# RinceWND/extPOM

Hardware: AMD Instinct MI355X
Metric: 3D cell-updates/sec on internal mode (one internal step = the 3-D baroclinic step and its isplit 2-D external substeps; whole-step wall time) (higher is better)
Workload: dtype f64

## Files before the change

### extpom_amd/csrc/k_adv.hip

```cpp
#include "pomgpu_internal.hpp"

#define dt_(i, j) F2(dt, i, j)
#define dx_(i, j) F2(dx, i, j)
#define dy_(i, j) F2(dy, i, j)
#define h_(i, j) F2(h, i, j)
#define u_(i, j, k) F3(u, i, j, k)
#define v_(i, j, k) F3(v, i, j, k)
#define ub_(i, j, k) F3(ub, i, j, k)
#define vb_(i, j, k) F3(vb, i, j, k)
#define w_(i, j, k) F3(w, i, j, k)
#define aam_(i, j, k) F3(aam, i, j, k)

#define MARCH3(call)                                                                  \
  const int g_ = (int)(blockIdx.x * blockDim.x + threadIdx.x);    \
  const int L_ = g_ >> 6, xcd_ = L_ & 7, m_ = L_ >> 3;                                \
  const int bpl_ = P.g_bpl, nbx_ = P.g_nbx;                                           \
  const int p_ = m_ % bpl_, t_ = m_ / bpl_;                                           \
  const int k = t_ % P.kb + 1;                                                        \
  const int band_ = (t_ / P.kb) * 8 + xcd_;                                           \
  const int i = (p_ % nbx_) * 64 + (g_ & 63) + 1;                                     \
  const int j = band_ * P.g_rb + (p_ / nbx_) * 4 + (int)threadIdx.y + 1;              \
  if (i > P.iml || j > P.jml) return;                                                 \
  call;
__device__ __forceinline__ void c_advct_a(const KP &P, const int i, const int j, const int k);
// ... 290 lines not shown
  MARCH3(c_smol(P, i, j, k, ff))
}
__device__ __forceinline__ void c_smol(const KP &P, const int i, const int j, const int k, const double *ff) {
  if (i > P.im || j > P.jm) return;
  const double value_min = 1.e-9, epsilon = 1.0e-14;
  double *xm = P.s3[0], *ym = P.s3[1], *zw = P.s3[2];
  const double fc = G3(ff, i, j, k);
  if (k <= P.kbm1 && j >= 2 && j <= P.jmm1 && i >= 2) {
    const double fw = G3(ff, i - 1, j, k);
    double r = 0.;
    if (!(fc < value_min || fw < value_min)) {
      const double m = G3(xm, i, j, k);
      const double udx = fabs(m);
      const double u2dt = P.dti2 * m * m * 2. / (F2(aru, i, j) * (dt_(i - 1, j) + dt_(i, j)));
      const double mol = (fc - fw) / (fw + fc + epsilon);
      r = (udx - u2dt) * mol * P.sw;
      if (fabs(udx) < fabs(u2dt)) r = 0.;
    }
    G3(xm, i, j, k) = r;
  }
  if (k <= P.kbm1 && j >= 2 && i >= 2 && i <= P.imm1) {
    const double fs = G3(ff, i, j - 1, k);
    double r = 0.;
    if (!(fc < value_min || fs < value_min)) {
      const double m = G3(ym, i, j, k);
      const double vdy = fabs(m);
      const double v2dt = P.dti2 * m * m * 2. / (F2(arv, i, j) * (dt_(i, j - 1) + dt_(i, j)));
      const double mol = (fc - fs) / (fs + fc + epsilon);
      r = (vdy - v2dt) * mol * P.sw;
      if (fabs(vdy) < fabs(v2dt)) r = 0.;
    }
    G3(ym, i, j, k) = r;
  }
  if (k >= 2 && k <= P.kbm1 && i >= 2 && i <= P.imm1 && j >= 2 && j <= P.jmm1) {
    const double fu = G3(ff, i, j, k - 1);
    double r = 0.;
    if (!(fc < value_min || fu < value_min)) {
      const double m = G3(zw, i, j, k);
      const double wdz = fabs(m);
      const double w2dt = P.dti2 * m * m / (F1(dzz, k - 1) * dt_(i, j));
      const double mol = (fu - fc) / (fc + fu + epsilon);
      r = (wdz - w2dt) * mol * P.sw;
      if (fabs(wdz) < fabs(w2dt)) r = 0.;
    }
    G3(zw, i, j, k) = r;
  }
}
__device__ __forceinline__ void c_copy3(const KP &P, const int i, const int j, const int k, double *dst, const double *src);
__global__ void k_copy3(KP P, double *dst, const double *src) {
  MARCH3(c_copy3(P, i, j, k, dst, src))
}
__device__ __forceinline__ void c_copy3(const KP &P, const int i, const int j, const int k, double *dst, const double *src) {
  G3(dst, i, j, k) = G3(src, i, j, k);
}
__device__ __forceinline__ double advt2_xdiff(const KP &P, const double *fb, const double *fc, int i, int j, int k) {
  const double am = 0.5 * (aam_(i, j, k) + aam_(i - 1, j, k));
  return -am * (h_(i, j) + h_(i - 1, j)) * P.tprni *
         ((G3(fb, i, j, k) - G3(fc, i, j, k)) - (G3(fb, i - 1, j, k) - G3(fc, i - 1, j, k))) * F2(dum, i, j) *
         (dy_(i, j) + dy_(i - 1, j)) * 0.5 / (dx_(i, j) + dx_(i - 1, j));
}
__device__ __forceinline__ double advt2_ydiff(const KP &P, const double *fb, const double *fc, int i, int j, int k) {
  const double am = 0.5 * (aam_(i, j, k) + aam_(i, j - 1, k));
  return -am * (h_(i, j) + h_(i, j - 1)) * P.tprni *
         ((G3(fb, i, j, k) - G3(fc, i, j, k)) - (G3(fb, i, j - 1, k) - G3(fc, i, j - 1, k))) * F2(dvm, i, j) *
         (dx_(i, j) + dx_(i, j - 1)) * 0.5 / (dy_(i, j) + dy_(i, j - 1));
}
__device__ __forceinline__ void c_advt2_diff(const KP &P, const int i, const int j, const int k, const double *fb, const double *fc, double *ff);
__global__ void k_advt2_diff(KP P, const double *fb, const double *fc, double *ff) {
  MARCH3(c_advt2_diff(P, i, j, k, fb, fc, ff))
}
__device__ __forceinline__ void c_advt2_diff(const KP &P, const int i, const int j, const int k, const double *fb, const double *fc, double *ff) {
  if (k > P.kbm1 || i < 2 || i > P.imm1 || j < 2 || j > P.jmm1) return;
  G3(ff, i, j, k) = G3(ff, i, j, k) -
                    P.dti2 * (advt2_xdiff(P, fb, fc, i + 1, j, k) - advt2_xdiff(P, fb, fc, i, j, k) +
                              advt2_ydiff(P, fb, fc, i, j + 1, k) - advt2_ydiff(P, fb, fc, i, j, k)) /
                        ((h_(i, j) + F2(etf, i, j)) * F2(art, i, j));
}

__device__ __forceinline__ double dens_point(const KP &P, double si, double ti, int i, int j, int k);
template <int TAU> __device__ __forceinline__ void c_ts_update(const KP &P, const int i, const int j, const int k, double fold, double fnew, int rt, int store_rst, double tau_b, double tau_f, const unsigned long long *rtf);
template <int TAU> __global__ void k_ts_update(KP P, double fold, double fnew, int rt, int store_rst, double tau_b, double tau_f, const unsigned long long *rtf) {
  MARCH3(c_ts_update<TAU>(P, i, j, k, fold, fnew, rt, store_rst, tau_b, tau_f, rtf))
}
__global__ void k_ts_update_same(KP P, double fold, double fnew, int rt, int store_rst, const unsigned long long *rtf) {
  MARCH3(c_ts_update<2>(P, i, j, k, fold, fnew, rt, store_rst, 0., 0., rtf))
}
template <int TAU> __device__ __forceinline__ void c_ts_update(const KP &P, const int i, const int j, const int k, double fold, double fnew, int rt, int store_rst, double tau_b, double tau_f, const unsigned long long *rtf) {
  const bool act = (i <= P.im && j <= P.jm), lev = (k <= P.kbm1);
  const pomgpu_ct m = F2(fsm, i, j);
  pomgpu_ct uf = F3(uf, i, j, k), vf = F3(vf, i, j, k);
  if (lev && act) {
    uf = uf * m;
    vf = vf * m;
  }
  pomgpu_ct tb = F3(tb, i, j, k), sb = F3(sb, i, j, k);
  bool rtc = rt != 0;
  if (rtc && rtf && lev) rtc = ((rtf[RT_WORD(P, i, j, k)] >> RT_BIT(i)) & 1ull) != 0;
  if (rtc) {
    const pomgpu_ct tc = F3(tclim, i, j, k), sc = F3(sclim, i, j, k);
    tb = (tb - tc) + tc;
    sb = (sb - sc) + sc;
  }
  const pomgpu_ct t0 = F3(t, i, j, k), s0 = F3(s, i, j, k);
  pomgpu_ct tbn = t0 + CT(.5) * CT(P.smoth) * (uf + tb - CT(2.) * t0);
  pomgpu_ct sbn = s0 + CT(.5) * CT(P.smoth) * (vf + sb - CT(2.) * s0);
  pomgpu_ct tn = uf, sn = vf;
// ... 297 lines not shown
  }
  F3(wr, i, j, k) = v;
}

struct LevR { double w_n, u_c, u_e, v_c, v_n; };
__device__ __forceinline__ LevR realvertvl_load(const KP &P, int a, int b, int k) {
  LevR L;
  L.w_n = w_(a, b, k + 1); L.u_c = u_(a, b, k); L.u_e = u_(a + 1, b, k); L.v_c = v_(a, b, k); L.v_n = v_(a, b + 1, k);
  return L;
}
__global__ void __launch_bounds__(256) k_realvertvl_col(KP P, int etf_is_et) {
  const int i = TID_I, j = TID_J;
  if (i > P.iml || j > P.jml) return;
  const bool act = (i <= P.im && j <= P.jm);
  const int a = (P.W && i == 1) ? 2 : ((P.E && i == P.im) ? P.imm1 : i);
  const int b = (P.S && j == 1) ? 2 : ((P.N && j == P.jm) ? P.jmm1 : j);
  const int kb = P.kb, kbm1 = P.kbm1;
  if (!(act && a >= 2 && a <= P.imm1 && b >= 2 && b <= P.jmm1)) {
    for (int k = 1; k <= kb; k++) F3(wr, i, j, k) = 0.;
    return;
  }
  const double dt_c = dt_(a, b), dt_e = dt_(a + 1, b), dt_w = dt_(a - 1, b), dt_n = dt_(a, b + 1), dt_s = dt_(a, b - 1);
  const double et_c = F2(et, a, b), et_e = F2(et, a + 1, b), et_w = F2(et, a - 1, b), et_n = F2(et, a, b + 1), et_s = F2(et, a, b - 1);
  const double dxr = K2(R2DXSX, a + 1, b), dxl = K2(R2DXSX, a, b), dyt = K2(R2DYSY, a, b + 1), dyb = K2(R2DYSY, a, b);
  const double detf = (etf_is_et ? et_c : F2(etf, a, b)) - F2(etb, a, b);
  const double m = F2(fsm, i, j);
  double w_k = w_(a, b, 1);
  LevR c = realvertvl_load(P, a, b, 1), nxt = c;
  for (int k = 1; k <= kbm1; k++) {
    PACE_BARRIER();
    if (k + 1 <= kbm1) nxt = realvertvl_load(P, a, b, k + 1);
    const double zzk = F1(zz, k);
#define TPS(dtv, etv) (zzk * (dtv) + (etv))
    const double tc = TPS(dt_c, et_c);
    double v = 0.5 * (w_k + c.w_n) +
               0.5 * (c.u_e * (TPS(dt_e, et_e) - tc) * dxr + c.u_c * (tc - TPS(dt_w, et_w)) * dxl +
                      c.v_n * (TPS(dt_n, et_n) - tc) * dyt + c.v_c * (tc - TPS(dt_s, et_s)) * dyb) +
               (1.0 + zzk) * detf / P.dti2;
#undef TPS
    F3(wr, i, j, k) = m * v;
    w_k = c.w_n;
    c = nxt;
  }
  F3(wr, i, j, kb) = 0.;
}

#define LD2(ptr, ii, jj, kk) (*(const double2 *)&(ptr)[IX3(ii, jj, kk)])
#define A3(name) (P.b3 + (size_t)P3_##name * P.a3)
__device__ __forceinline__ double aam_point(const KP &P, double dx, double dy, double u_c, double u_e, double u_n, double u_ne, double u_s,
                                            double u_se, double v_c, double v_n, double v_e, double v_ne, double v_w, double v_nw) {
  return P.horcon * dx * dy *
         sqrt(sq((u_e - u_c) / dx) + sq((v_n - v_c) / dy) +
              .5 * sq(.25 * (u_n + u_ne - u_s - u_se) / dy + .25 * (v_e + v_ne - v_w - v_nw) / dx));
}
__device__ __forceinline__ double aam_point_r(const KP &P, const InvD &dx, const InvD &dy, double u_c, double u_e, double u_n, double u_ne, double u_s,
                                              double u_se, double v_c, double v_n, double v_e, double v_ne, double v_w, double v_nw) {
  return P.horcon * dx.b * dy.b *
         sqrt(sq(divi(u_e - u_c, dx)) + sq(divi(v_n - v_c, dy)) +
              .5 * sq(divi(.25 * (u_n + u_ne - u_s - u_se), dy) + divi(.25 * (v_e + v_ne - v_w - v_nw), dx)));
}
#ifndef AAM_KCH
#define AAM_KCH 7
#endif
struct AamLev { double2 u_s, u_0, u_n, v_0, v_n; };
__global__ void __launch_bounds__(256) k_aam_pair(KP P) {
  const int g_ = (int)(blockIdx.x * blockDim.x + threadIdx.x);
  const int L_ = g_ >> 6, xcd_ = L_ & 7, m_ = L_ >> 3;
  const int nbx_ = (P.iml / 2 + 61) / 62, bpl_ = nbx_ * (P.g_rb / 4);
  const int nch_ = (P.kbm1 + AAM_KCH - 1) / AAM_KCH;
  const int p_ = m_ % bpl_, t_ = m_ / bpl_;
  const int k0 = (t_ % nch_) * AAM_KCH + 1;
  const int band_ = (t_ / nch_) * 8 + xcd_;
  const int lane = g_ & 63;
  const int ia0 = 2 * ((p_ % nbx_) * 62 + lane - 1) + 1;
  const int j = band_ * P.g_rb + (p_ / nbx_) * 4 + (int)threadIdx.y + 1;
  if (k0 > P.kbm1 || j < 2 || j > P.jmm1) return;
  const int k1 = k0 + AAM_KCH - 1 < P.kbm1 ? k0 + AAM_KCH - 1 : P.kbm1;
  const bool out = (lane >= 1 && lane <= 62 && ia0 <= P.iml);
#ifdef POMGPU_EMU
  if (!out) return;
#endif
  const int ia = ia0 < 1 ? 1 : (ia0 > P.iml - 1 ? P.iml - 1 : ia0), ib = ia + 1;
  const int iw = ia > 1 ? ia - 1 : 1, ie = ib < P.iml ? ib + 1 : P.iml;
  const double2 dx = *(const double2 *)&F2(dx, ia, j), dy = *(const double2 *)&F2(dy, ia, j);
#ifndef AAM_PLAIN_DIV
  const double2 rdx = *(const double2 *)&K2(RDX, ia, j), rdy = *(const double2 *)&K2(RDY, ia, j);
  const InvD dxa = {dx.x, rdx.x}, dya = {dy.x, rdy.x}, dxb = {dx.y, rdx.y}, dyb = {dy.y, rdy.y};
#endif
  auto lev = [&](int k) {
    AamLev L;
    L.u_s = LD2(A3(u), ia, j - 1, k); L.u_0 = LD2(A3(u), ia, j, k); L.u_n = LD2(A3(u), ia, j + 1, k);
    L.v_0 = LD2(A3(v), ia, j, k); L.v_n = LD2(A3(v), ia, j + 1, k);
    return L;
  };
  AamLev cur = lev(k0);
  for (int k = k0; k <= k1; k++) {
    const AamLev nxt = lev(k < k1 ? k + 1 : k1);
    const double2 u_s = cur.u_s, u_0 = cur.u_0, u_n = cur.u_n, v_0 = cur.v_0, v_n = cur.v_n;
    const double uE_s = halo_e(u_s.x, [&] { return u_(ie, j - 1, k); }), uE_0 = halo_e(u_0.x, [&] { return u_(ie, j, k); }),
                 uE_n = halo_e(u_n.x, [&] { return u_(ie, j + 1, k); });
    const double vE_0 = halo_e(v_0.x, [&] { return v_(ie, j, k); }), vE_n = halo_e(v_n.x, [&] { return v_(ie, j + 1, k); });
    const double vW_0 = halo_w(v_0.y, [&] { return v_(iw, j, k); }), vW_n = halo_w(v_n.y, [&] { return v_(iw, j + 1, k); });
#ifndef AAM_PLAIN_DIV
    const double aa = aam_point_r(P, dxa, dya, u_0.x, u_0.y, u_n.x, u_n.y, u_s.x, u_s.y, v_0.x, v_n.x, v_0.y, v_n.y, vW_0, vW_n);
    const double ab = aam_point_r(P, dxb, dyb, u_0.y, uE_0, u_n.y, uE_n, u_s.y, uE_s, v_0.y, v_n.y, vE_0, vE_n, v_0.x, v_n.x);
#else
    const double aa = aam_point(P, dx.x, dy.x, u_0.x, u_0.y, u_n.x, u_n.y, u_s.x, u_s.y, v_0.x, v_n.x, v_0.y, v_n.y, vW_0, vW_n);
    const double ab = aam_point(P, dx.y, dy.y, u_0.y, uE_0, u_n.y, uE_n, u_s.y, uE_s, v_0.y, v_n.y, vE_0, vE_n, v_0.x, v_n.x);
#endif
    if (out && ia0 >= 2 && ia0 <= P.imm1) F3(aam, ia0, j, k) = aa;
    if (out && ia0 + 1 <= P.imm1) F3(aam, ia0 + 1, j, k) = ab;
    cur = nxt;
  }
}
#undef LD2
#undef A3


void launch_advct_a(pomgpu_ctx *c) { LAUNCH(c, k_advct_a, gridm(c->P), blk2(), c->P); }
void launch_advct_b(pomgpu_ctx *c) { LAUNCH(c, k_advct_b, gridm(c->P), blk2(), c->P); }
void launch_advct_c(pomgpu_ctx *c) { LAUNCH(c, k_advct_c, gridm(c->P), blk2(), c->P); }
void launch_aam(pomgpu_ctx *c) {
  const KP &P = c->P;
#ifdef POMGPU_STORE_F32
  const bool pair_ok = false;
#else
  const bool pair_ok = true;
#endif
  if (pair_ok && P.iml % 2 == 0 && !SW(c, NO_PAIR)) {
    const long nbands = (P.jml + P.g_rb - 1) / P.g_rb, rounds = (nbands + 7) / 8;
    const long bpl = (long)((P.iml / 2 + 61) / 62) * (P.g_rb / 4);
    const long nch = (P.kbm1 + AAM_KCH - 1) / AAM_KCH;
    LAUNCHN(c, "k_aam_pair", k_aam_pair, dim3((unsigned)(8 * rounds * nch * bpl), 1, 1), blk2(), c->P);
  } else {
    LAUNCH(c, k_aam, gridm(c->P), blk2(), c->P);
  }
}
void launch_roundtrip(pomgpu_ctx *c, double *a, const double *b, int fix_kb) { LAUNCH(c, k_roundtrip, gridm(c->P), blk2(), c->P, a, b, fix_kb); }
void launch_roundtrip_level(pomgpu_ctx *c, double *a, const double *b, int k) { LAUNCH(c, k_roundtrip_level, grid2(c->P), blk2(), c->P, a, b, k); }
void launch_advq_flux(pomgpu_ctx *c, const double *q, const double *qb, double *xf, double *yf) {
  LAUNCH(c, k_advq_flux, gridm(c->P), blk2(), c->P, q, qb, xf, yf);
}
void launch_advq_step(pomgpu_ctx *c, const double *q, const double *qb, double *qf, const double *xf, const double *yf, int zero_else) {
  LAUNCH(c, k_advq_step, gridm(c->P), blk2(), c->P, q, qb, qf, xf, yf, zero_else);
}
void launch_q_filter(pomgpu_ctx *c, int mask) { LAUNCH(c, k_q_filter, gridm(c->P), blk2(), c->P, mask); }
void launch_q_filter_rim(pomgpu_ctx *c) {
  const KP &P = c->P;
  const int len = P.im > P.jm ? P.im : P.jm;
  LAUNCH(c, k_q_filter_rim, dim3((len + 63) / 64, 8, P.kb), dim3(64, 1, 1), c->P);
}
void launch_mask_q(pomgpu_ctx *c) { LAUNCH(c, k_mask_q, gridm(c->P), blk2(), c->P); }
void launch_advt1(pomgpu_ctx *c, double *fb, double *f, const double *fclim, double *ff) {
  LAUNCH(c, k_advt1, gridm(c->P), blk2(), c->P, (const double *)fb, (const double *)f, fclim, ff);
  LAUNCH(c, k_copy_kb, grid2(c->P), blk2(), c->P, f, (double *)NULL);
}
void launch_copy_kb(pomgpu_ctx *c, double *f, double *g) { LAUNCH(c, k_copy_kb, grid2(c->P), blk2(), c->P, f, g); }
void launch_advt2_mass(pomgpu_ctx *c) { LAUNCH(c, k_advt2_mass, gridm(c->P), blk2(), c->P); }
void launch_advt2_step(pomgpu_ctx *c, const double *fbmem, const double *f, const double *eta, double *ff, int itera) {
  LAUNCH(c, k_advt2_step, gridm(c->P), blk2(), c->P, fbmem, f, eta, ff, itera);
}
void launch_mask3(pomgpu_ctx *c, double *a, const double *m2) { LAUNCH(c, k_mask3, gridm(c->P), blk2(), c->P, a, m2); }
void launch_smol(pomgpu_ctx *c, const double *ff) { LAUNCH(c, k_smol, gridm(c->P), blk2(), c->P, ff); }
void launch_copy3(pomgpu_ctx *c, double *dst, const double *src) { LAUNCH(c, k_copy3, gridm(c->P), blk2(), c->P, dst, src); }
void launch_advt2_diff(pomgpu_ctx *c, const double *fb, const double *fc, double *ff) { LAUNCH(c, k_advt2_diff, gridm(c->P), blk2(), c->P, fb, fc, ff); }
void launch_ts_update(pomgpu_ctx *c, double fold, double fnew, int rt, int store_rst, int rt_flags) {
  const unsigned long long *rtf = (rt && rt_flags) ? c->rt_words : NULL;
  if (rtf && c->prof_on) {
    const int s = pomgpu_prof_slot(c, "ts_rt_flags");
    if (s >= 0) (c->parent ? c->parent : c)->prof[s].launches++;
  }
  if (c->tau_known[0] && c->tau_known[1] && !c->tau_handed && !SW(c, TAU_ARRAYS))
    LAUNCHN(c, "k_ts_update", (k_ts_update<1>), gridm(c->P), blk2(), c->P, fold, fnew, rt, store_rst, c->tau_val[0], c->tau_val[1], rtf);
  else if (c->tau_same && !c->tau_handed && !SW(c, TAU_ARRAYS))
    LAUNCH(c, k_ts_update_same, gridm(c->P), blk2(), c->P, fold, fnew, rt, store_rst, rtf);
  else
    LAUNCHN(c, "k_ts_update", (k_ts_update<0>), gridm(c->P), blk2(), c->P, fold, fnew, rt, store_rst, 0., 0., rtf);
}
void launch_restore_fields(pomgpu_ctx *c, double fold, double fnew) { LAUNCH(c, k_restore_fields, gridm(c->P), blk2(), c->P, fold, fnew); }
void launch_mask_ts(pomgpu_ctx *c) { LAUNCH(c, k_mask_ts, gridm(c->P), blk2(), c->P); }
void launch_tr_update(pomgpu_ctx *c, const TrUpd *u, int nf, int rt) {
  if (nf == 2) {
    TrUpds<2> A; A.u[0] = u[0]; A.u[1] = u[1];
    LAUNCHN(c, "k_tr_update2", (k_tr_update<2>), gridm(c->P), blk2(), c->P, A, rt);
  } else {
    TrUpds<1> A; A.u[0] = u[0];
    LAUNCHN(c, "k_tr_update", (k_tr_update<1>), gridm(c->P), blk2(), c->P, A, rt);
  }
}
void launch_tr_source(pomgpu_ctx *c, double *ff, const double *fb, const double *fc, const double *q, double lam) {
  LAUNCH(c, k_tr_source, gridm(c->P), blk2(), c->P, ff, fb, fc, q, lam);
}
void launch_mask_uv(pomgpu_ctx *c) { LAUNCH(c, k_mask_uv, gridm(c->P), blk2(), c->P); }
void launch_mask_w(pomgpu_ctx *c) { LAUNCH(c, k_mask_w, gridm(c->P), blk2(), c->P); }
void launch_restore(pomgpu_ctx *c, double fold, double fnew) { LAUNCH(c, k_restore, gridm(c->P), blk2(), c->P, fold, fnew); }
void launch_restore_shift(pomgpu_ctx *c) { LAUNCH(c, k_restore_shift, gridm(c->P), blk2(), c->P); }
void launch_restore_load(pomgpu_ctx *c, const double *tr, const double *sr, double tau, const double *taur, int fill_tau) { LAUNCH(c, k_restore_load, gridm(c->P), blk2(), c->P, tr, sr, tau, taur, fill_tau); }
void launch_probe_gpow15(pomgpu_ctx *c, long n, const double *x, double *out) { LAUNCH(c, k_probe_gpow15, dim3((unsigned)((n + 255) / 256), 1, 1), dim3(256, 1, 1), n, x, out); }
void launch_dens(pomgpu_ctx *c, const double *si, const double *ti, double *rhoo) { LAUNCH(c, k_dens, gridm(c->P), blk2(), c->P, si, ti, rhoo); }
void launch_realvertvl(pomgpu_ctx *c, int etf_is_et) {
  if (SW(c, REALVERTVL_CELLS)) LAUNCH(c, k_realvertvl, gridm(c->P), blk2(), c->P, etf_is_et);
  else LAUNCHN(c, "k_realvertvl_col", k_realvertvl_col, grid2(c->P), blk2(), c->P, etf_is_et);
}
```

### extpom_amd/csrc/k_tile.hip

```cpp
#include "pomgpu_internal.hpp"


__global__ void k_coef_static(KP P) {
  const int i = TID_I, j = TID_J;
  if (i > P.iml || j > P.jml) return;
  const int iw = i > 1 ? i - 1 : 1, js = j > 1 ? j - 1 : 1;
  P.m8[IX2(i, j)] = (unsigned char)((F2(fsm, i, j) != 0. ? 1 : 0) | (F2(dum, i, j) != 0. ? 2 : 0) | (F2(dvm, i, j) != 0. ? 4 : 0));
  K2(HSX, i, j) = F2(h, i, j) + F2(h, iw, j);
  K2(HSY, i, j) = F2(h, i, j) + F2(h, i, js);
  K2(DYSX, i, j) = F2(dy, i, j) + F2(dy, iw, j);
  K2(DXSX, i, j) = F2(dx, i, j) + F2(dx, iw, j);
  K2(DXSY, i, j) = F2(dx, i, j) + F2(dx, i, js);
  K2(DYSY, i, j) = F2(dy, i, j) + F2(dy, i, js);
  K2(DX4, i, j) = F2(dx, i, j) + F2(dx, iw, j) + F2(dx, i, js) + F2(dx, iw, js);
  K2(DY4, i, j) = F2(dy, i, j) + F2(dy, iw, j) + F2(dy, i, js) + F2(dy, iw, js);
  const int ie = i < P.iml ? i + 1 : P.iml, jn = j < P.jml ? j + 1 : P.jml;
  K2(CVA, i, j) = F2(dy, ie, j) - F2(dy, iw, j);
  K2(CVB, i, j) = F2(dx, i, jn) - F2(dx, i, js);
  K2(R2DXSX, i, j) = 2.0 / (F2(dx, i, j) + F2(dx, iw, j));
  K2(R2DYSY, i, j) = 2.0 / (F2(dy, i, j) + F2(dy, i, js));
  K2(RDX, i, j) = 1.0 / F2(dx, i, j);
  K2(RDY, i, j) = 1.0 / F2(dy, i, j);
  if (j == 1)
    for (int n = i - 1; n < POM_NBLK1D * P.kb; n += P.iml) P.r1[n] = 1.0 / P.b1[n];
// ... 24 lines not shown
    K2(VCOR, i, j) = (j >= 2 && j <= P.jm && i <= P.im) ? cv : mark;
  }
}

__device__ __forceinline__ pomgpu_ct upw_(pomgpu_ct m, pomgpu_ct lo, pomgpu_ct hi) {
  return CT(0.5) * ((m + fabs(m)) * lo + (m - fabs(m)) * hi);
}
struct FaceT { pomgpu_ct adv, dif; };
struct TFields { const double *fb[2], *f[2], *fcl[2]; double *ff[2]; unsigned long long *rtf; };
template <int NF> struct LevT { pomgpu_ct c[2 * NF + 2], o[2], h[ROWSHARE_SLOTS(2 * NF + 2)]; };
template <int NS> struct NbrT { pomgpu_ct s[NS], n[NS]; };
struct CoefT { pomgpu_ct cm, hs, msk, ds_num; InvDc den; };
__device__ __forceinline__ CoefT coef_x(const KP &P, int i, int j) {
  CoefT c; c.cm = K2(CMX, i, j); c.hs = K2(HSX, i, j); c.msk = F2(dum, i, j); c.ds_num = K2(DYSX, i, j); c.den = inv_of(CT(K2(DXSX, i, j))); return c;
}
__device__ __forceinline__ CoefT coef_y(const KP &P, int i, int j) {
  CoefT c; c.cm = K2(CMY, i, j); c.hs = K2(HSY, i, j); c.msk = F2(dvm, i, j); c.ds_num = K2(DXSY, i, j); c.den = inv_of(CT(K2(DYSY, i, j))); return c;
}
__device__ __forceinline__ FaceT advt2_face(const pomgpu_ct tprni, const CoefT &c, pomgpu_ct vel, pomgpu_ct fb_hi, pomgpu_ct fb_lo, pomgpu_ct fc_hi,
                                            pomgpu_ct fc_lo, pomgpu_ct am_hi, pomgpu_ct am_lo) {
  FaceT f;
  f.adv = upw_(c.cm * vel, fb_lo, fb_hi);
  const pomgpu_ct am = CT(0.5) * (am_hi + am_lo);
  f.dif = divi(-am * c.hs * tprni * ((fb_hi - fc_hi) - (fb_lo - fc_lo)) * c.msk * c.ds_num * CT(0.5), c.den);
  return f;
}
#if COL_WX != 1
#error "the row-sharing column kernels keep one wavefront per workgroup row (COL_WX == 1)"
#endif
template <int NF, bool UM = false, bool RTF = false>
__global__ void __launch_bounds__(64 * LDS_ROWS) k_advt2_col(KP P, TFields A) {
  constexpr int NS = 2 * NF + 2, NH = ROWSHARE_SLOTS(NS), AM = 2 * NF, VV = 2 * NF + 1;
  HALO_XCD_DECODE_R(LDS_ROWS)
  const int r = WAVE_UNIFORM((int)threadIdx.y), j0w = j - r;
  const bool jrow = j <= P.jml;
  const int jc = jrow ? j : P.jml;
  const bool icol = jrow && (lane >= 1 && lane <= 62 && i0 <= P.iml);
#ifdef POMGPU_EMU
  if (!icol) return;
#endif
  const int i = i0 < 1 ? 1 : (i0 > P.iml ? P.iml : i0);
  const int iw = i > 1 ? i - 1 : 1, ie = i < P.iml ? i + 1 : P.iml;
  const int js = jc > 1 ? jc - 1 : 1, jn = jc < P.jml ? jc + 1 : P.jml;
  const bool in = icol && (i >= 2 && i <= P.imm1 && jc >= 2 && jc <= P.jmm1);
  const pomgpu_ct fsm = F2(fsm, i, jc);
  const CoefT cw = coef_x(P, i, jc), cs = coef_y(P, i, jc), cn = coef_y(P, i, jn);
  const pomgpu_ct art = F2(art, i, jc), hea = K2(HEA, i, jc);
  const InvDc hfa = inv_of(CT(K2(HFA, i, jc)));
  const pomgpu_ct tprni = P.tprni, dti2 = P.dti2;
  BufA bs[NS], bo[2], bff[NF], bh[NH];
  const double *ps[NS];
#pragma unroll
  for (int f = 0; f < NF; f++) { ps[f] = A.fb[f]; ps[NF + f] = A.fcl[f]; bff[f] = BUF3(A.ff[f]); }
  ps[AM] = A3(aam); ps[VV] = A3(v); bo[0] = BUF3(A3(u)); bo[1] = BUF3(A3(w));
#pragma unroll
  for (int x = 0; x < NS; x++) bs[x] = BUF3(ps[x]);
  const RowShare<NS> S = rowshare_setup<NS>(P, r, j, j0w, i);
#pragma unroll
  for (int q = 0; q < NH; q++) bh[q] = BUF3(rowshare_pick<NS>(ps, S.hop[q]));
  const UvmC mu = UM ? uvm_of<0>(P, i, jc) : uvm_none(), mv = UM ? uvm_of<1>(P, i, jc) : uvm_none();
  UvmC mh[NH];
#pragma unroll
  for (int q = 0; q < NH; q++) mh[q] = UM ? rowshare_uvm<1, NS, LDS_ROWS>(P, S, q, VV, j0w, i) : uvm_none();
  const unsigned oc = BOFF2(i, jc), lvb = LVB;
  const unsigned ost = in ? oc : BOFF_NONE;
  const int rt_nbx = RT_NBX(P);
  const BufA brtf = buf2_of((const double *)A.rtf, RTF ? (size_t)P.kbm1 * P.jml * rt_nbx : 0);
  const unsigned ortf = (RTF && jrow && lane == 0) ? (unsigned)((jc - 1) * rt_nbx + (i0 - lane) / 62) * 8u : BOFF_NONE, lvrtf = (unsigned)(P.jml * rt_nbx) * 8u;
#ifndef POMGPU_EMU
  __shared__ pomgpu_ct slab[2][NS][ROWSHARE_ROWS][64];
#else
  const unsigned os = BOFF2(i, js), on = BOFF2(i, jn);
#endif
  auto load = [&](LevT<NF> &L, unsigned lv) {
#pragma unroll
    for (int x = 0; x < NS; x++) L.c[x] = bldc(bs[x], oc, lv);
    L.o[0] = bldc(bo[0], oc, lv); L.o[1] = bldc(bo[1], oc, lv);
#pragma unroll
    for (int q = 0; q < NH; q++) L.h[q] = bldc(bh[q], S.hoff[q], lv);
  };
  pomgpu_ct f1[NF];
#pragma unroll
  for (int f = 0; f < NF; f++) f1[f] = G3(A.f[f], i, jc, 1);
  const int kbm1 = P.kbm1;
  pomgpu_ct p_adv[NF], p_dif[NF], p_fb[NF], p_zu[NF];
#pragma unroll
  for (int f = 0; f < NF; f++) p_adv[f] = p_dif[f] = p_fb[f] = p_zu[f] = 0.;
  auto step = [&](const int L, const int par, const LevT<NF> &cur, LevT<NF> &nxt) {
    load(nxt, (unsigned)(L < kbm1 ? L : kbm1 - 1) * lvb);
    NbrT<NS> nb;
    const pomgpu_ct v_c = uvm_fix(cur.c[VV], mv);
#ifndef POMGPU_EMU
#pragma unroll
    for (int x = 0; x < NS; x++) slab[par][x][r + 1][lane] = x == VV ? v_c : cur.c[x];
#pragma unroll
    for (int q = 0; q < NH; q++) slab[par][S.hop[q]][S.hrow[q]][lane] = uvm_fix(cur.h[q], mh[q]);
    __syncthreads();
#pragma unroll
    for (int x = 0; x < NS; x++) { nb.s[x] = slab[par][x][S.ss][lane]; nb.n[x] = slab[par][x][S.sn][lane]; }
#else
    const unsigned lvc = (unsigned)((L <= kbm1 ? L : kbm1) - 1) * lvb;
#pragma unroll
    for (int x = 0; x < NS; x++) { nb.s[x] = bldc(bs[x], os, lvc); nb.n[x] = bldc(bs[x], on, lvc); }
    nb.s[VV] = uvm_fix(nb.s[VV], uvm_of<1>(P, i, js)); nb.n[VV] = uvm_fix(nb.n[VV], uvm_of<1>(P, i, jn));
#endif
    const pomgpu_ct am_c = cur.c[AM], u_c = uvm_fix(cur.o[0], mu), w_c = cur.o[1];
    const pomgpu_ct am_w = halo_w(am_c, [&] { return F3(aam, iw, jc, L); });
    InvDc dzk; dzk.b = dzk.y = 0.;
    if (L >= 2) { dzk.b = F1(dz, L - 1); dzk.y = R1(dz, L - 1); }
    if constexpr (RTF) {
      bool ch = false;
#pragma unroll
      for (int f = 0; f < NF; f++) ch = ch || rt_changes(cur.c[f], cur.c[NF + f]);
      const unsigned lvw = (unsigned)WAVE_UNIFORM(L - 1) * lvrtf;
#ifndef POMGPU_EMU
      bst2u(brtf, L <= kbm1 ? ortf : BOFF_NONE, lvw, __ballot(icol && ch));
#else
      if (L <= kbm1) {
        unsigned long long &wd = A.rtf[RT_WORD(P, i, jc, L)];
        wd = (lane == 1 ? 0ull : wd) | ((unsigned long long)ch << lane);
      }
      (void)brtf; (void)ortf; (void)lvw;
#endif
    }
#pragma unroll
    for (int f = 0; f < NF; f++) {
      const pomgpu_ct fb_c = cur.c[f], fc_c = cur.c[NF + f];
      pomgpu_ct zu = 0.;
      pomgpu_ct s_adv = 0., s_dif = 0.;
      if (L <= kbm1) {
        const pomgpu_ct fb_w = halo_w(fb_c, [&] { return G3(A.fb[f], iw, jc, L); });
        const pomgpu_ct fc_w = halo_w(fc_c, [&] { return G3(A.fcl[f], iw, jc, L); });
        const FaceT xw = advt2_face(tprni, cw, u_c, fb_c, fb_w, fc_c, fc_w, am_c, am_w);
        auto east = [&] {
          return advt2_face(tprni, coef_x(P, ie, jc), uvm_ld<0>(P, ie, jc, L), G3(A.fb[f], ie, jc, L), fb_c, G3(A.fcl[f], ie, jc, L), fc_c,
                            F3(aam, ie, jc, L), am_c);
        };
        FaceT xe;
        xe.adv = halo_e(xw.adv, [&] { return east().adv; });
        xe.dif = halo_e(xw.dif, [&] { return east().dif; });
        const FaceT ys = advt2_face(tprni, cs, v_c, fb_c, nb.s[f], fc_c, nb.s[NF + f], am_c, nb.s[AM]);
        const FaceT yn = advt2_face(tprni, cn, nb.n[VV], nb.n[f], fb_c, nb.n[NF + f], fc_c, nb.n[AM], am_c);
        s_adv = xe.adv - xw.adv + yn.adv - ys.adv;
        s_dif = xe.dif - xw.dif + yn.dif - ys.dif;
        zu = (L == 1) ? w_c * f1[f] * art : upw_(w_c, fb_c, p_fb[f]) * art;
      }
      {
        pomgpu_ct rr = p_adv[f] + divi(p_zu[f] - zu, dzk);
        rr = divi(p_fb[f] * hea - dti2 * rr, hfa);
        rr = rr * fsm;
        rr = rr - divi(dti2 * p_dif[f], hfa);
        bstc(bff[f], (L >= 2 && L <= kbm1 + 1) ? ost : BOFF_NONE, (unsigned)(L >= 2 ? L - 2 : 0) * lvb, rr);
      }
      p_adv[f] = s_adv; p_dif[f] = s_dif; p_fb[f] = fb_c; p_zu[f] = zu;
    }
  };
  LevT<NF> ra, rb;
  load(ra, 0u);
  rb = ra;
  for (int L = 1; L <= kbm1 + 1; L += 2) {
    step(L, 1, ra, rb);
    step(L + 1, 0, rb, ra);
  }
  if (icol) {
    for (int k = in ? P.kb : 1; k <= P.kb; k++) {
#pragma unroll
      for (int f = 0; f < NF; f++) G3(A.ff[f], i, jc, k) = CT(G3(A.ff[f], i, jc, k)) * fsm;
    }
  }
}

struct QFields { const double *q[2], *qb[2]; double *qf[2]; };
template <int NF, int NO = 2> struct LevQa { pomgpu_ct c[2 * NF + 2], o[NO], h[ROWSHARE_SLOTS(2 * NF + 2)]; };
struct CoefQ { pomgpu_ct dts, hs, msk, ds_num; InvDc den; };
__device__ __forceinline__ CoefQ coefq_x(const KP &P, int i, int j) {
  CoefQ c; c.dts = K2(DTSX, i, j); c.hs = K2(HSX, i, j); c.msk = F2(dum, i, j); c.den = inv_of(CT(K2(DXSX, i, j))); c.ds_num = K2(DYSX, i, j); return c;
}
__device__ __forceinline__ CoefQ coefq_y(const KP &P, int i, int j) {
  CoefQ c; c.dts = K2(DTSY, i, j); c.hs = K2(HSY, i, j); c.msk = F2(dvm, i, j); c.den = inv_of(CT(K2(DYSY, i, j))); c.ds_num = K2(DXSY, i, j); return c;
}
__device__ __forceinline__ pomgpu_ct advq_face(const CoefQ &c, pomgpu_ct q_hi, pomgpu_ct q_lo, pomgpu_ct vel_k, pomgpu_ct vel_km1, pomgpu_ct am_hi_k,
                                               pomgpu_ct am_lo_k, pomgpu_ct am_hi_m, pomgpu_ct am_lo_m, pomgpu_ct qb_hi, pomgpu_ct qb_lo) {
  pomgpu_ct x = CT(.125) * (q_hi + q_lo) * c.dts * (vel_k + vel_km1);
  x = x - divi(CT(.25) * (am_hi_k + am_lo_k + am_hi_m + am_lo_m) * c.hs * (qb_hi - qb_lo) * c.msk, c.den);
  return CT(.5) * c.ds_num * x;
}
template <int NF, bool WF = false, bool UM = false>
__global__ void __launch_bounds__(64 * LDS_ROWS) k_advq_col(KP P, QFields A, int zero_else) {
  constexpr int NS = 2 * NF + 2, NH = ROWSHARE_SLOTS(NS), AM = 2 * NF, VV = 2 * NF + 1;
  typedef LevQa<NF, WF ? 1 : 2> Lev;
  HALO_XCD_DECODE_R(LDS_ROWS)
  const int r = WAVE_UNIFORM((int)threadIdx.y), j0w = j - r;
  const bool jrow = j <= P.jml;
  const int jc = jrow ? j : P.jml;
  const bool icol = jrow && (lane >= 1 && lane <= 62 && i0 <= P.iml);
#ifdef POMGPU_EMU
  if (!icol) return;
#endif
  const int i = i0 < 1 ? 1 : (i0 > P.iml ? P.iml : i0);
  const int iw = i > 1 ? i - 1 : 1, ie = i < P.iml ? i + 1 : P.iml;
  const int js = jc > 1 ? jc - 1 : 1, jn = jc < P.jml ? jc + 1 : P.jml;
  const bool in = icol && (i >= 2 && i <= P.imm1 && jc >= 2 && jc <= P.jmm1);
  const CoefQ cw = coefq_x(P, i, jc), cs = coefq_y(P, i, jc), cn = coefq_y(P, i, jn);
  const pomgpu_ct art = F2(art, i, jc), hea = K2(HEA, i, jc);
  const InvDc hfa = inv_of(CT(K2(HFA, i, jc)));
  const int kb = P.kb, kbm1 = P.kbm1;
  BufA bs[NS], bo[2], bqf[NF], bh[NH];
  const double *ps[NS];
#pragma unroll
  for (int f = 0; f < NF; f++) { ps[f] = A.q[f]; ps[NF + f] = A.qb[f]; bqf[f] = BUF3(A.qf[f]); }
  ps[AM] = A3(aam); ps[VV] = A3(v); bo[0] = BUF3(A3(u)); bo[1] = BUF3(A3(w));
#pragma unroll
  for (int x = 0; x < NS; x++) bs[x] = BUF3(ps[x]);
  const RowShare<NS> S = rowshare_setup<NS>(P, r, j, j0w, i);
#pragma unroll
  for (int q = 0; q < NH; q++) bh[q] = BUF3(rowshare_pick<NS>(ps, S.hop[q]));
  const UvmC mu = UM ? uvm_of<0>(P, i, jc) : uvm_none(), mv = UM ? uvm_of<1>(P, i, jc) : uvm_none();
  UvmC mh[NH];
#pragma unroll
  for (int q = 0; q < NH; q++) mh[q] = UM ? rowshare_uvm<1, NS, LDS_ROWS>(P, S, q, VV, j0w, i) : uvm_none();
  const unsigned oc = BOFF2(i, jc), lvb = LVB;
  const unsigned ost = in ? oc : ((zero_else && icol) ? oc : BOFF_NONE);
  const unsigned ostw = in ? oc : BOFF_NONE;
#ifndef POMGPU_EMU
  __shared__ pomgpu_ct slab[2][NS][ROWSHARE_ROWS][64];
#else
  const unsigned os = BOFF2(i, js), on = BOFF2(i, jn);
#endif
  double vv_cw = 0., vv_ce = 0., vv_cs = 0., vv_cn = 0., vv_det = 0., vv_m = 0., wk = 0.;
  InvD vv_area; vv_area.b = vv_area.y = 0.;
  if constexpr (WF) {
    vv_m = F2(fsm, i, jc);
    const double dyc = F2(dy, i, jc), dtc = F2(dt, i, jc), dxc = F2(dx, i, jc);
    const double dyw = halo_w(dyc, [&] { return F2(dy, iw, jc); }), dtw = halo_w(dtc, [&] { return F2(dt, iw, jc); });
    const double dye = halo_e(dyc, [&] { return F2(dy, ie, jc); }), dte = halo_e(dtc, [&] { return F2(dt, ie, jc); });
    vv_cw = .25 * (dyc + dyw) * (dtc + dtw);
    vv_ce = .25 * (dye + dyc) * (dte + dtc);
    vv_cs = .25 * (dxc + F2(dx, i, js)) * (dtc + F2(dt, i, js));
    vv_cn = .25 * (F2(dx, i, jn) + dxc) * (F2(dt, i, jn) + dtc);
    vv_area = inv_of(dxc * dyc);
    vv_det = (F2(etf, i, jc) - F2(etb, i, jc)) / P.dti2;
    wk = 0.5 * (F2(vfluxb, i, jc) + F2(vfluxf, i, jc));
  }
  auto load = [&](Lev &L, int k) {
    const unsigned lv = (unsigned)WAVE_UNIFORM(k - 1) * lvb;
#pragma unroll
    for (int x = 0; x < NS; x++) L.c[x] = bldc(bs[x], oc, lv);
    L.o[0] = bldc(bo[0], oc, lv);
    if constexpr (!WF) L.o[1] = bldc(bo[1], oc, lv);
#pragma unroll
    for (int q = 0; q < NH; q++) L.h[q] = bldc(bh[q], S.hoff[q], lv);
  };
  pomgpu_ct u_m = 0., v_m = 0., vn_m = 0., am_m = 0., ams_m = 0., amn_m = 0.;
  pomgpu_ct am_w_prv = 0.;
  pomgpu_ct ue_m = 0.;
  pomgpu_ct wq_pp[NF], wq_p[NF];
  pomgpu_ct xe_p[NF], xw_p[NF], yn_p[NF], ys_p[NF], qb_p[NF];
#pragma unroll
  for (int f = 0; f < NF; f++) wq_pp[f] = wq_p[f] = xe_p[f] = xw_p[f] = yn_p[f] = ys_p[f] = qb_p[f] = 0.;
  auto step = [&](const int L, const int par, const Lev &cur, Lev &nxt) {
    load(nxt, L + 1 <= kb ? L + 1 : kb);
    NbrT<NS> nb;
    const bool lcor = L <= kbm1;
    const pomgpu_ct v_c = uvm_fix(cur.c[VV], mv, lcor), u_c = uvm_fix(cur.o[0], mu, lcor);
#ifndef POMGPU_EMU
#pragma unroll
    for (int x = 0; x < NS; x++) slab[par][x][r + 1][lane] = x == VV ? v_c : cur.c[x];
#pragma unroll
    for (int q = 0; q < NH; q++) slab[par][S.hop[q]][S.hrow[q]][lane] = uvm_fix(cur.h[q], mh[q], lcor);
    __syncthreads();
#pragma unroll
    for (int x = 0; x < NS; x++) { nb.s[x] = slab[par][x][S.ss][lane]; nb.n[x] = slab[par][x][S.sn][lane]; }
#else
    const unsigned lvc = (unsigned)((L <= kb ? L : kb) - 1) * lvb;
#pragma unroll
    for (int x = 0; x < NS; x++) { nb.s[x] = bldc(bs[x], os, lvc); nb.n[x] = bldc(bs[x], on, lvc); }
    nb.s[VV] = uvm_fix(nb.s[VV], uvm_of<1>(P, i, js), lcor); nb.n[VV] = uvm_fix(nb.n[VV], uvm_of<1>(P, i, jn), lcor);
#endif
    const pomgpu_ct am_c = cur.c[AM];
    const pomgpu_ct am_s = nb.s[AM], am_n = nb.n[AM], v_n = nb.n[VV];
    const pomgpu_ct am_w = halo_w(am_c, [&] { return F3(aam, iw, jc, L); });
    pomgpu_ct w_c, ue_c = 0.;
    if constexpr (WF) {
      ue_c = halo_e(u_c, [&] { return uvm_ld<0>(P, ie, jc, L); });
      const double wn = wk + F1(dz, L >= 2 ? L - 1 : 1) *
                             (divi(vv_ce * (double)ue_m - vv_cw * (double)u_m + vv_cn * (double)vn_m - vv_cs * (double)v_m, vv_area) + vv_det);
      wk = L >= 2 ? wn : wk;
      const double wst = L <= kbm1 ? wk * vv_m : wk;
      bst(bo[1], ostw, (unsigned)WAVE_UNIFORM(L - 1) * lvb, wst);
      w_c = CT((pomgpu_st)wst);
    } else {
      w_c = cur.o[1];
    }
    const int k = L - 1;
    InvDc dz2; dz2.b = dz2.y = 0.;
    if (k >= 2 && k <= kbm1) { dz2.b = CT(F1(dz, k)) + CT(F1(dz, k - 1)); dz2.y = CT(1.0) / dz2.b; }
#pragma unroll
    for (int f = 0; f < NF; f++) {
      const pomgpu_ct q_c = cur.c[f], qb_c = cur.c[NF + f];
      pomgpu_ct xe_c = 0., xw_c = 0., yn_c = 0., ys_c = 0.;
      if (L >= 2 && L <= kbm1) {
        const pomgpu_ct q_w = halo_w(q_c, [&] { return G3(A.q[f], iw, jc, L); });
        const pomgpu_ct qb_w = halo_w(qb_c, [&] { return G3(A.qb[f], iw, jc, L); });
        const pomgpu_ct xw = advq_face(cw, q_c, q_w, u_c, u_m, am_c, am_w, am_m, am_w_prv, qb_c, qb_w);
        xw_c = xw;
        xe_c = halo_e(xw, [&] {
          return advq_face(coefq_x(P, ie, jc), G3(A.q[f], ie, jc, L), q_c, uvm_ld<0>(P, ie, jc, L), uvm_ld<0>(P, ie, jc, L - 1), F3(aam, ie, jc, L), am_c,
                           F3(aam, ie, jc, L - 1), am_m, G3(A.qb[f], ie, jc, L), qb_c);
        });
        ys_c = advq_face(cs, q_c, nb.s[f], v_c, v_m, am_c, am_s, am_m, ams_m, qb_c, nb.s[NF + f]);
        yn_c = advq_face(cn, nb.n[f], q_c, v_n, vn_m, am_n, am_c, amn_m, am_m, nb.n[NF + f], qb_c);
      }
      const pomgpu_ct wq_c = w_c * q_c;
      {
        pomgpu_ct rr = 0.;
        if (in && k >= 2 && k <= kbm1) {
          rr = divi((wq_pp[f] - wq_c) * art, dz2) + xe_p[f] - xw_p[f] + yn_p[f] - ys_p[f];
          rr = divi(hea * qb_p[f] - CT(P.dti2) * rr, hfa);
        }
        const bool lev_in = (k >= 2 && k <= kbm1);
        const unsigned o = (k >= 1) ? (lev_in ? ost : ((zero_else && icol) ? oc : BOFF_NONE)) : BOFF_NONE;
        bstc(bqf[f], o, (unsigned)WAVE_UNIFORM(k >= 1 ? k - 1 : 0) * lvb, rr);
      }
      wq_pp[f] = wq_p[f]; wq_p[f] = wq_c; qb_p[f] = qb_c;
      xe_p[f] = xe_c; xw_p[f] = xw_c; yn_p[f] = yn_c; ys_p[f] = ys_c;
    }
    am_w_prv = am_w;
    if constexpr (WF) ue_m = ue_c;
    u_m = u_c; v_m = v_c; vn_m = v_n; am_m = am_c; ams_m = am_s; amn_m = am_n;
  };
  Lev ra, rb;
  load(ra, 1);
  rb = ra;
  for (int L = 1; L <= kb; L += 2) {
    step(L, 1, ra, rb);
    if (L + 1 <= kb) step(L + 1, 0, rb, ra);
  }
  if (icol && zero_else) {
#pragma unroll
    for (int f = 0; f < NF; f++) G3(A.qf[f], i, jc, kb) = 0.;
  }
  if constexpr (WF) {
    if (icol && !in && i0 <= P.im && jc <= P.jm)
      for (int k = 1; k <= kbm1; k++) F3(w, i, jc, k) = F3(w, i, jc, k) * vv_m;
  }
}

__device__ double advct_xf_mem(const KP &P, int i, int j, int k) {
  if (i < 2 || i > P.imm1) return 0.;
  double xf = .125 * (K2(DTSX, i + 1, j) * F3(u, i + 1, j, k) + K2(DTSX, i, j) * F3(u, i, j, k)) * (F3(u, i + 1, j, k) + F3(u, i, j, k));
  xf = xf - F2(dt, i, j) * F3(aam, i, j, k) * 2. * (F3(ub, i + 1, j, k) - F3(ub, i, j, k)) / F2(dx, i, j);
  return F2(dy, i, j) * xf;
}
__device__ double advct_curv_mem(const KP &P, int i, int j, int k) {
  if (i < 2 || i > P.imm1 || j < 2 || j > P.jmm1) return 0.;
  return .25 * ((F3(v, i, j + 1, k) + F3(v, i, j, k)) * K2(CVA, i, j) - (F3(u, i + 1, j, k) + F3(u, i, j, k)) * K2(CVB, i, j)) / F2(art, i, j);
}
__device__ double advct_xg_mem(const KP &P, int i, int j, int k) {
  double xg = .125 * (K2(DTSX, i, j) * F3(u, i, j, k) + K2(DTSX, i, j - 1) * F3(u, i, j - 1, k)) * (F3(v, i, j, k) + F3(v, i - 1, j, k));
  const double dtaam = .25 * K2(DT4, i, j) * (F3(aam, i, j, k) + F3(aam, i - 1, j, k) + F3(aam, i, j - 1, k) + F3(aam, i - 1, j - 1, k));
  const double dy4 = K2(DY4, i, j);
  xg = xg - dtaam * ((F3(ub, i, j, k) - F3(ub, i, j - 1, k)) / dy4 + (F3(vb, i, j, k) - F3(vb, i - 1, j, k)) / K2(DX4, i, j));
  return .25 * dy4 * xg;
}
__device__ double advct_yf_mem(const KP &P, int i, int j, int k) {
  double yf = .125 * (K2(DTSY, i, j) * F3(v, i, j, k) + K2(DTSY, i - 1, j) * F3(v, i - 1, j, k)) * (F3(u, i, j, k) + F3(u, i, j - 1, k));
  const double dtaam = .25 * K2(DT4, i, j) * (F3(aam, i, j, k) + F3(aam, i - 1, j, k) + F3(aam, i, j - 1, k) + F3(aam, i - 1, j - 1, k));
  const double dx4 = K2(DX4, i, j);
  yf = yf - dtaam * ((F3(ub, i, j, k) - F3(ub, i, j - 1, k)) / K2(DY4, i, j) + (F3(vb, i, j, k) - F3(vb, i - 1, j, k)) / dx4);
  return .25 * dx4 * yf;
}
__device__ double advct_yg_mem(const KP &P, int i, int j, int k) {
  double yg = .125 * (K2(DTSY, i, j + 1) * F3(v, i, j + 1, k) + K2(DTSY, i, j) * F3(v, i, j, k)) * (F3(v, i, j + 1, k) + F3(v, i, j, k));
  yg = yg - F2(dt, i, j) * F3(aam, i, j, k) * 2. * (F3(vb, i, j + 1, k) - F3(vb, i, j, k)) / F2(dy, i, j);
  return F2(dx, i, j) * yg;
}
__global__ void k_advct_edge(KP P, double *to_e, double *to_n) {
  const int t = TID_I, k = (int)blockIdx.y + 1;
  if (k > P.kbm1) return;
  if (to_e && t <= P.jm) {
    const size_t o = (size_t)(k - 1) * P.jm + (size_t)(t - 1);
    to_e[o] = advct_curv_mem(P, P.imm1, t, k);
    to_e[(size_t)P.kbm1 * P.jm + o] = t >= 2 ? advct_xf_mem(P, P.imm1, t, k) : 0.;
  }
  if (to_n && t <= P.im) {
    const size_t o = (size_t)(k - 1) * P.im + (size_t)(t - 1);
    to_n[o] = advct_curv_mem(P, t, P.jmm1, k);
    to_n[(size_t)P.kbm1 * P.im + o] = t >= 2 ? advct_yg_mem(P, t, P.jmm1, k) : 0.;
  }
}
__global__ void k_advct_fix(KP P, const double *from_w, const double *from_s) {
  const int t = TID_I, k = (int)blockIdx.y + 1;
  if (k > P.kbm1) return;
  if (from_w && t >= 2 && t <= P.jmm1) {
    const int j = t;
    const size_t o = (size_t)(k - 1) * P.jm + (size_t)(j - 1);
    const double cv_w = from_w[o], xf_w = from_w[(size_t)P.kbm1 * P.jm + o];
    const double xf = advct_xf_mem(P, 2, j, k), yf_n = advct_yf_mem(P, 2, j + 1, k), yf_c = advct_yf_mem(P, 2, j, k);
    const double cv = advct_curv_mem(P, 2, j, k);
    const double ctx = cv * F2(dt, 2, j) * (F3(v, 2, j + 1, k) + F3(v, 2, j, k));
    const double ctx_w = cv_w * F2(dt, 1, j) * (F3(v, 1, j + 1, k) + F3(v, 1, j, k));
    double ax = xf - xf_w + yf_n - yf_c;
    ax = ax - F2(aru, 2, j) * .25 * (ctx + ctx_w);
    F3(advx, 2, j, k) = ax;
  }
  if (from_s && t >= 2 && t <= P.imm1) {
    const int i = t;
    const size_t o = (size_t)(k - 1) * P.im + (size_t)(i - 1);
    const double cv_s = from_s[o], yg_s = from_s[(size_t)P.kbm1 * P.im + o];
    const double xg_e = advct_xg_mem(P, i + 1, 2, k), xg = advct_xg_mem(P, i, 2, k), yg_c = advct_yg_mem(P, i, 2, k);
    const double cv = advct_curv_mem(P, i, 2, k);
    double ay = xg_e - xg + yg_c - yg_s;
    ay = ay + F2(arv, i, 2) * .25 * (cv * F2(dt, i, 2) * (F3(u, i + 1, 2, k) + F3(u, i, 2, k)) +
                                     cv_s * F2(dt, i, 1) * (F3(u, i + 1, 1, k) + F3(u, i, 1, k)));
    F3(advy, i, 2, k) = ay;
  }
}
template <int ROWS> struct LevCaT { pomgpu_ct c[5], h[(2 * 5 + ROWS - 1) / ROWS]; };
template <int ROWS>
__global__ void __launch_bounds__(64 * ROWS) k_advct_col(KP P, int sum2d) {
  constexpr int NS = 5, NH = (2 * NS + ROWS - 1) / ROWS, U = 0, V = 1, UB = 2, VB = 3, AM = 4;
  typedef LevCaT<ROWS> LevCa;
  HALO_XCD_DECODE_R(ROWS)
#ifdef POMGPU_WGTIME
  const unsigned long long wgt0 = wall_clock64();
#endif
  const int r = WAVE_UNIFORM((int)threadIdx.y), j0w = j - r;
  const bool jvalid = j <= P.jml;
  const int jc = jvalid ? j : P.jml;
  const bool out = jvalid && (lane >= 1 && lane <= 62 && i0 <= P.iml);
#ifdef POMGPU_EMU
  if (!out) return;
#endif
  const int i = i0 < 1 ? 1 : (i0 > P.iml ? P.iml : i0);
  const int iw = i > 1 ? i - 1 : 1, ie = i < P.iml ? i + 1 : P.iml;
  const int js = jc > 1 ? jc - 1 : 1, jn = jc < P.jml ? jc + 1 : P.jml;
  const bool jrow = (jc >= 2 && jc <= P.jmm1);
  const bool iin = (i0 >= 2 && i0 <= P.imm1);
  const bool in = out && iin && jrow;
  const int kb = P.kb, kbm1 = P.kbm1;
  double ax2 = 0., ay2 = 0.;
#if POMGPU_UVM_ONLOAD
  double su2 = 0., sv2 = 0.;
#endif
  const pomgpu_ct dtsx_c = K2(DTSX, i, jc), dtsx_s = K2(DTSX, i, js);
  const pomgpu_ct dtsx_e = halo_e(dtsx_c, [&] { return K2(DTSX, ie, jc); });
  const pomgpu_ct dtsy_c = K2(DTSY, i, jc), dtsy_n = K2(DTSY, i, jn), dtsy_s = K2(DTSY, i, js);
  const pomgpu_ct dtsy_w = halo_w(dtsy_c, [&] { return K2(DTSY, iw, jc); });
  const pomgpu_ct dtsy_nw = halo_w(dtsy_n, [&] { return K2(DTSY, iw, jn); });
  const pomgpu_ct dt4_c = K2(DT4, i, jc), dt4_n = K2(DT4, i, jn);
  const pomgpu_ct dx4_c = K2(DX4, i, jc), dx4_n = K2(DX4, i, jn);
  const InvDc dy4_c = inv_of(CT(K2(DY4, i, jc))), dy4_n = inv_of(CT(K2(DY4, i, jn))), idx4_c = inv_of(dx4_c), idx4_n = inv_of(dx4_n);
  const pomgpu_ct dt_c = F2(dt, i, jc), dy_c = F2(dy, i, jc), dx_c = F2(dx, i, jc);
  const pomgpu_ct dt_s = F2(dt, i, js), dx_s = F2(dx, i, js);
  const InvDc idx_c = inv_of(dx_c), idy_c = inv_of(dy_c), idy_s = inv_of(CT(F2(dy, i, js)));
  const pomgpu_ct cva_c = K2(CVA, i, jc), cvb_c = K2(CVB, i, jc);
  const pomgpu_ct cva_s = K2(CVA, i, js), cvb_s = K2(CVB, i, js);
  const InvDc art_c = inv_of(CT(F2(art, i, jc))), art_s = inv_of(CT(F2(art, i, js)));
  const pomgpu_ct aru = F2(aru, i, jc), arv = F2(arv, i, jc);
  const bool srow = (jc - 1 >= 2);
  const bool curvx = (i0 >= (P.W ? 3 : 2)), curvy = (jc >= (P.S ? 3 : 2));
  BufA bs[NS], bh[NH];
  const double *ps[NS] = {A3(u), A3(v), A3(ub), A3(vb), A3(aam)};
#pragma unroll
  for (int x = 0; x < NS; x++) bs[x] = BUF3(ps[x]);
  const BufA bax = BUF3(A3(advx)), bay = BUF3(A3(advy));
  const RowShare<NS, ROWS> S = rowshare_setup<NS, ROWS>(P, r, j, j0w, i);
#pragma unroll
  for (int q = 0; q < NH; q++) bh[q] = BUF3(rowshare_pick<NS>(ps, S.hop[q]));
  const unsigned oc = BOFF2(i, jc), lvb = LVB;
  const unsigned ost = (out && jrow) ? oc : BOFF_NONE;
#ifndef POMGPU_EMU
  __shared__ pomgpu_ct slab[2][NS][ROWS + 3][64];
#else
  const unsigned os = BOFF2(i, js), on = BOFF2(i, jn);
#endif
  auto load = [&](LevCa &L, int k) {
    const unsigned lv = (unsigned)WAVE_UNIFORM(k - 1) * lvb;
#pragma unroll
    for (int x = 0; x < NS; x++) L.c[x] = bldc(bs[x], oc, lv);
#pragma unroll
    for (int q = 0; q < NH; q++) L.h[q] = bldc(bh[q], S.hoff[q], lv);
  };
  auto step = [&](const int k, const int par, const LevCa &cur, LevCa &nxt) {
    load(nxt, k + 1 <= kbm1 ? k + 1 : kbm1);
    NbrT<NS> nb;
#ifndef POMGPU_EMU
#pragma unroll
    for (int x = 0; x < NS; x++) slab[par][x][r + 1][lane] = cur.c[x];
#pragma unroll
    for (int q = 0; q < NH; q++) slab[par][S.hop[q]][S.hrow[q]][lane] = cur.h[q];
    __syncthreads();
#pragma unroll
    for (int x = 0; x < NS; x++) { nb.s[x] = slab[par][x][S.ss][lane]; nb.n[x] = slab[par][x][S.sn][lane]; }
#else
    const unsigned lvc = (unsigned)(k - 1) * lvb;
#pragma unroll
    for (int x = 0; x < NS; x++) { nb.s[x] = bldc(bs[x], os, lvc); nb.n[x] = bldc(bs[x], on, lvc); }
#endif
    const pomgpu_ct u_c = cur.c[U], v_c = cur.c[V], ub_c = cur.c[UB], vb_c = cur.c[VB], am_c = cur.c[AM];
    const pomgpu_ct u_s = nb.s[U], v_s = nb.s[V], ub_s = nb.s[UB], vb_s = nb.s[VB], am_s = nb.s[AM];
    const pomgpu_ct u_n = nb.n[U], v_n = nb.n[V], ub_n = nb.n[UB], vb_n = nb.n[VB], am_n = nb.n[AM];
    const pomgpu_ct u_e = halo_e(u_c, [&] { return F3(u, ie, jc, k); });
    const pomgpu_ct u_se = halo_e(u_s, [&] { return F3(u, ie, js, k); });
    const pomgpu_ct ub_e = halo_e(ub_c, [&] { return F3(ub, ie, jc, k); });
    const pomgpu_ct v_w = halo_w(v_c, [&] { return F3(v, iw, jc, k); });
    const pomgpu_ct v_nw = halo_w(v_n, [&] { return F3(v, iw, jn, k); });
    const pomgpu_ct vb_w = halo_w(vb_c, [&] { return F3(vb, iw, jc, k); });
    const pomgpu_ct vb_nw = halo_w(vb_n, [&] { return F3(vb, iw, jn, k); });
    const pomgpu_ct am_w = halo_w(am_c, [&] { return F3(aam, iw, jc, k); });
    const pomgpu_ct am_sw = halo_w(am_s, [&] { return F3(aam, iw, js, k); });
    const pomgpu_ct am_nw = halo_w(am_n, [&] { return F3(aam, iw, jn, k); });
    pomgpu_ct xf = 0., cv = 0.;
    if (iin) {
      xf = CT(.125) * (dtsx_e * u_e + dtsx_c * u_c) * (u_e + u_c);
      xf = xf - divi(dt_c * am_c * CT(2.) * (ub_e - ub_c), idx_c);
      xf = dy_c * xf;
      cv = divi(CT(.25) * ((v_n + v_c) * cva_c - (u_e + u_c) * cvb_c), art_c);
    }
    const pomgpu_ct ctx = cv * dt_c * (v_n + v_c);
    const pomgpu_ct xf_w = halo_w(xf, [&] { return advct_xf_mem(P, i - 1, jc, k); });
    const pomgpu_ct ctx_w = halo_w(ctx, [&] {
      return advct_curv_mem(P, i - 1, jc, k) * F2(dt, i - 1, jc) * (F3(v, i - 1, jc + 1, k) + F3(v, i - 1, jc, k));
    });
    const pomgpu_ct dtaam = CT(.25) * dt4_c * (am_c + am_w + am_s + am_sw);
    const pomgpu_ct br = divi(ub_c - ub_s, dy4_c) + divi(vb_c - vb_w, idx4_c);
    pomgpu_ct yf_c = CT(.125) * (dtsy_c * v_c + dtsy_w * v_w) * (u_c + u_s);
    yf_c = yf_c - dtaam * br;
    yf_c = CT(.25) * dx4_c * yf_c;
    pomgpu_ct xg = CT(.125) * (dtsx_c * u_c + dtsx_s * u_s) * (v_c + v_w);
    xg = xg - dtaam * br;
    xg = CT(.25) * dy4_c.b * xg;
    const pomgpu_ct xg_e = halo_e(xg, [&] { return advct_xg_mem(P, i + 1, jc, k); });
    const pomgpu_ct dtaam_n = CT(.25) * dt4_n * (am_n + am_nw + am_c + am_w);
    pomgpu_ct yf_n = CT(.125) * (dtsy_n * v_n + dtsy_nw * v_nw) * (u_n + u_c);
    yf_n = yf_n - dtaam_n * (divi(ub_n - ub_c, dy4_n) + divi(vb_n - vb_nw, idx4_n));
    yf_n = CT(.25) * dx4_n * yf_n;
    pomgpu_ct yg_c = CT(.125) * (dtsy_n * v_n + dtsy_c * v_c) * (v_n + v_c);
    yg_c = yg_c - divi(dt_c * am_c * CT(2.) * (vb_n - vb_c), idy_c);
    yg_c = dx_c * yg_c;
    pomgpu_ct yg_s = 0., cv_s = 0.;
    if (srow) {
      yg_s = CT(.125) * (dtsy_c * v_c + dtsy_s * v_s) * (v_c + v_s);
      yg_s = yg_s - divi(dt_s * am_s * CT(2.) * (vb_c - vb_s), idy_s);
      yg_s = dx_s * yg_s;
      if (iin) cv_s = divi(CT(.25) * ((v_c + v_s) * cva_s - (u_se + u_s) * cvb_s), art_s);
    }
    pomgpu_ct ax = 0., ay = 0.;
    if (in) {
      ax = xf - xf_w + yf_n - yf_c;
      if (curvx) ax = ax - aru * CT(.25) * (ctx + ctx_w);
      ay = xg_e - xg + yg_c - yg_s;
      if (curvy) ay = ay + arv * CT(.25) * (cv * dt_c * (u_e + u_c) + cv_s * dt_s * (u_se + u_s));
    }
    const unsigned lv = (unsigned)WAVE_UNIFORM(k - 1) * lvb;
    bstc(bax, ost, lv, ax);
    bstc(bay, ost, lv, ay);
    const double dzk = F1(dz, k);
    ax2 = ax2 + ax * dzk;
    ay2 = ay2 + ay * dzk;
#if POMGPU_UVM_ONLOAD
    su2 = su2 + (double)u_c * dzk;
    sv2 = sv2 + (double)v_c * dzk;
#endif
  };
  LevCa ra, rb;
#ifdef POMGPU_EMU
  if (jrow) {
#endif
  load(ra, 1);
  rb = ra;
  for (int k = 1; k <= kbm1; k += 2) {
    step(k, 1, ra, rb);
    if (k + 1 <= kbm1) step(k + 1, 0, rb, ra);
  }
#ifdef POMGPU_EMU
  }
#if POMGPU_UVM_ONLOAD
  else {
    for (int k = 1; k <= kbm1; k++) { su2 = su2 + (double)F3(u, i, jc, k) * F1(dz, k); sv2 = sv2 + (double)F3(v, i, jc, k) * F1(dz, k); }
  }
#endif
#endif
#if POMGPU_UVM_ONLOAD
  if (out && (sum2d & 2)) { K2(USUM, i, jc) = su2; K2(VSUM, i, jc) = sv2; }
#endif
  if (out) {
    if (jrow) {
      F3(advx, i, jc, kb) = 0.; F3(advy, i, jc, kb) = 0.;
    } else {
      for (int k = 1; k <= kb; k++) { F3(advx, i, jc, k) = 0.; F3(advy, i, jc, k) = 0.; }
    }
    if (sum2d & 1) { F2(adx2d, i, jc) = jrow ? ax2 : 0.; F2(ady2d, i, jc) = jrow ? ay2 : 0.; }
  }
#ifdef POMGPU_WGTIME
  __syncthreads();
  if (threadIdx.y == 0 && lane == 0) {
    double *rec = (double *)(P.b3 + (size_t)P3_wr * P.a3) + 4 * (size_t)L__;
    rec[0] = (double)wgt0; rec[1] = (double)wall_clock64();
    rec[2] = (double)__builtin_amdgcn_s_getreg((31 << 11) | 4);
    rec[3] = (double)__builtin_amdgcn_s_getreg((31 << 11) | 20);
  }
#endif
}

struct LevUV { pomgpu_ct c[3], h[ROWSHARE_SLOTS(3)], ub, vb, advx, advy, drhox, drhoy; };
template <bool UM>
__global__ void __launch_bounds__(64 * LDS_ROWS) k_advuv_col(KP P) {
  constexpr int NS = 3, NH = ROWSHARE_SLOTS(NS), W = 0, U = 1, V = 2;
  HALO_XCD_DECODE_R(LDS_ROWS)
  const int r = WAVE_UNIFORM((int)threadIdx.y), j0w = j - r;
  const bool jvalid = j <= P.jm;
  const int jc = j <= P.jml ? j : P.jml;
  const bool out = jvalid && (lane >= 1 && lane <= 62 && i0 <= P.im);
#ifdef POMGPU_EMU
  if (!out) return;
#endif
  const int i = i0 < 1 ? 1 : (i0 > P.iml ? P.iml : i0);
  const int iw = i > 1 ? i - 1 : 1, ie = i < P.iml ? i + 1 : P.iml;
  const int js = jc > 1 ? jc - 1 : 1, jn = jc < P.jml ? jc + 1 : P.jml;
  const bool in = out && (i >= 2 && i <= P.imm1 && jc >= 2 && jc <= P.jmm1);
  const int kb = P.kb, kbm1 = P.kbm1;
#define C2_(name, i, j) CT(F2(name, i, j))
  const pomgpu_ct aru = F2(aru, i, jc), arv = F2(arv, i, jc), dti2 = P.dti2;
  const pomgpu_ct dt_c = F2(dt, i, jc), dt_w = F2(dt, iw, jc), dt_s = F2(dt, i, js);
  const pomgpu_ct cd_c = C2_(cor, i, jc) * dt_c, cd_s = C2_(cor, i, js) * dt_s;
  const pomgpu_ct hcu = CT(P.grav) * CT(.125) * (dt_c + dt_w) *
                        (C2_(egf, i, jc) - C2_(egf, iw, jc) + C2_(egb, i, jc) - C2_(egb, iw, jc) + (C2_(e_atmos, i, jc) - C2_(e_atmos, iw, jc)) * CT(2.)) *
                        (C2_(dy, i, jc) + C2_(dy, iw, jc));
  const pomgpu_ct hcv = CT(P.grav) * CT(.125) * (dt_c + dt_s) *
                        (C2_(egf, i, jc) - C2_(egf, i, js) + C2_(egb, i, jc) - C2_(egb, i, js) + (C2_(e_atmos, i, jc) - C2_(e_atmos, i, js)) * CT(2.)) *
                        (C2_(dx, i, jc) + C2_(dx, i, js));
  const pomgpu_ct hb = C2_(h, i, jc) + C2_(etb, i, jc), hf = C2_(h, i, jc) + C2_(etf, i, jc);
  const pomgpu_ct sau = (hb + C2_(h, iw, jc) + C2_(etb, iw, jc)) * aru;
  const pomgpu_ct sav = (hb + C2_(h, i, js) + C2_(etb, i, js)) * arv;
  const InvDc sdu = inv_of((hf + C2_(h, iw, jc) + C2_(etf, iw, jc)) * aru), sdv = inv_of((hf + C2_(h, i, js) + C2_(etf, i, js)) * arv);
#undef C2_
  BufA bs[NS], bh[NH];
  const double *ps[NS] = {A3(w), A3(u), A3(v)};
#pragma unroll
  for (int x = 0; x < NS; x++) bs[x] = BUF3(ps[x]);
  const BufA bub = BUF3(A3(ub)), bvb = BUF3(A3(vb)), bax = BUF3(A3(advx)), bay = BUF3(A3(advy)), bdx = BUF3(A3(drhox)), bdy = BUF3(A3(drhoy)),
             buf = BUF3(A3(uf)), bvf = BUF3(A3(vf));
  const RowShare<NS> S = rowshare_setup<NS>(P, r, j, j0w, i);
#pragma unroll
  for (int q = 0; q < NH; q++) bh[q] = BUF3(rowshare_pick<NS>(ps, S.hop[q]));
// ... 57 lines not shown
    pomgpu_ct fu_n = 0., fv_n = 0.;
    if (k + 1 <= kbm1) {
      if (i >= 2) fu_n = CT(.25) * (w_c + w_w) * (u_c + u_k);
      if (jc >= 2) fv_n = CT(.25) * (w_c + w_s) * (v_c + v_k);
    }
    pomgpu_ct ru = fu_k, rv = fv_k;
    if (in) {
      InvDc dzk; dzk.b = F1(dz, k); dzk.y = R1(dz, k);
      ru = divi(sau * c.ub - CT(2.) * dti2 * (c.advx + divi((fu_k - fu_n) * aru, dzk) - aru * CT(.25) * (tc + tw) + hcu + c.drhox), sdu);
      rv = divi(sav * c.vb -
                    CT(2.) * dti2 * (c.advy + divi((fv_k - fv_n) * arv, dzk) + arv * CT(.25) * (cd_c * (u_e + u_k) + cd_s * (u_se + u_s)) + hcv + c.drhoy),
                sdv);
    }
    const unsigned lv = (unsigned)WAVE_UNIFORM(k - 1) * lvb;
    bstc(buf, ost, lv, ru);
    bstc(bvf, ost, lv, rv);
    fu_k = fu_n; fv_k = fv_n;
    u_k = u_c; v_k = v_c;
  };
  LevUV ra, rb;
  load(ra, 1);
  rb = ra;
  for (int k = 1; k <= kbm1; k += 6) {
    step(k, 1, ra, rb);
    if (k + 1 <= kbm1) step(k + 1, 2, rb, ra);
    if (k + 2 <= kbm1) step(k + 2, 0, ra, rb);
    if (k + 3 <= kbm1) step(k + 3, 1, rb, ra);
    if (k + 4 <= kbm1) step(k + 4, 2, ra, rb);
    if (k + 5 <= kbm1) step(k + 5, 0, rb, ra);
  }
  if (out) { F3(uf, i, jc, kb) = 0.; F3(vf, i, jc, kb) = 0.; }
}

void launch_coef_static(pomgpu_ctx *c) { LAUNCH(c, k_coef_static, grid2(c->P), blk2(), c->P); }
void launch_coef_dt(pomgpu_ctx *c) { LAUNCH(c, k_coef_dt, grid2(c->P), blk2(), c->P); }
void launch_coef_eta(pomgpu_ctx *c, int uvm) { LAUNCH(c, k_coef_eta, grid2(c->P), blk2(), c->P, uvm); }
void launch_advq_col(pomgpu_ctx *c, const double *q, const double *qb, double *qf, int zero_else) {
  QFields A; A.q[0] = A.q[1] = q; A.qb[0] = A.qb[1] = qb; A.qf[0] = A.qf[1] = qf;
  LAUNCHN(c, "k_advq_col", (k_advq_col<1>), grid1_halo_r(c->P, LDS_ROWS), blk_col_r(LDS_ROWS), c->P, A, zero_else);
}
void launch_advq2_col(pomgpu_ctx *c, const double *q, const double *qb, double *qf, const double *ql, const double *qlb, double *qlf, int zero_else) {
  QFields A; A.q[0] = q; A.qb[0] = qb; A.qf[0] = qf; A.q[1] = ql; A.qb[1] = qlb; A.qf[1] = qlf;
  LAUNCHN(c, "k_advq2_col", (k_advq_col<2>), grid1_halo_r(c->P, LDS_ROWS), blk_col_r(LDS_ROWS), c->P, A, zero_else);
}
#if POMGPU_W_FUSE
void launch_advq2w_col(pomgpu_ctx *c, const double *q, const double *qb, double *qf, const double *ql, const double *qlb, double *qlf, int zero_else) {
  QFields A; A.q[0] = q; A.qb[0] = qb; A.qf[0] = qf; A.q[1] = ql; A.qb[1] = qlb; A.qf[1] = qlf;
#if POMGPU_UVM_ONLOAD
  if (c->P.uvm) { LAUNCHN(c, "k_advq2_col", (k_advq_col<2, true, true>), grid1_halo_r(c->P, LDS_ROWS), blk_col_r(LDS_ROWS), c->P, A, zero_else); return; }
#endif
  LAUNCHN(c, "k_advq2_col", (k_advq_col<2, true>), grid1_halo_r(c->P, LDS_ROWS), blk_col_r(LDS_ROWS), c->P, A, zero_else);
}
#endif
void launch_advct_col(pomgpu_ctx *c, int sum2d) {
  const bool rows4 = SW(c, ADVCT_ROWS4) || (!SW(c, ADVCT_ROWS8) && c->P.jml <= 400 && c->exch);
  sum2d = (sum2d ? 1 : 0) | (POMGPU_UVM_ONLOAD && !c->exch && !c->tp.on && !c->wide.on && !(c->flags & POMGPU_CTX_2D) ? 2 : 0);
  if (rows4) LAUNCHN(c, "k_advct_col", (k_advct_col<4>), grid1_halo_r(c->P, 4), blk_col_r(4), c->P, sum2d);
  else LAUNCHN(c, "k_advct_col", (k_advct_col<LDS_ROWS>), grid1_halo_r(c->P, LDS_ROWS), blk_col_r(LDS_ROWS), c->P, sum2d);
}
__global__ void k_advct_fix2d(KP P, int west, int south) {
  const int t = TID_I;
  if (west && t >= 2 && t <= P.jmm1) {
    double a = 0.;
#pragma unroll 8
    for (int k = 1; k <= P.kbm1; k++) a = a + F3(advx, 2, t, k) * F1(dz, k);
    F2(adx2d, 2, t) = a;
  }
  if (south && t >= 2 && t <= P.imm1) {
    double a = 0.;
#pragma unroll 8
    for (int k = 1; k <= P.kbm1; k++) a = a + F3(advy, t, 2, k) * F1(dz, k);
    F2(ady2d, t, 2) = a;
  }
}
void launch_advct_fix2d(pomgpu_ctx *c, int west, int south) {
  const KP &P = c->P;
  const int len = P.im > P.jm ? P.im : P.jm;
  LAUNCH(c, k_advct_fix2d, dim3((len + 63) / 64, 1, 1), dim3(64, 1, 1), c->P, west, south);
}
void launch_advct_edge(pomgpu_ctx *c, double *to_e, double *to_n) {
  const KP &P = c->P;
  const int len = P.im > P.jm ? P.im : P.jm;
  LAUNCH(c, k_advct_edge, dim3((len + 63) / 64, P.kbm1, 1), dim3(64, 1, 1), c->P, to_e, to_n);
}
void launch_advct_fix(pomgpu_ctx *c, const double *from_w, const double *from_s) {
  const KP &P = c->P;
  const int len = P.im > P.jm ? P.im : P.jm;
  LAUNCH(c, k_advct_fix, dim3((len + 63) / 64, P.kbm1, 1), dim3(64, 1, 1), c->P, from_w, from_s);
}
void launch_advuv_col(pomgpu_ctx *c) {
#if POMGPU_UVM_ONLOAD
  if (c->P.uvm) { LAUNCHN(c, "k_advuv_col", (k_advuv_col<true>), grid1_halo_r(c->P, LDS_ROWS), blk_col_r(LDS_ROWS), c->P); return; }
#endif
  LAUNCHN(c, "k_advuv_col", (k_advuv_col<false>), grid1_halo_r(c->P, LDS_ROWS), blk_col_r(LDS_ROWS), c->P);
}
void launch_advt2_rows(pomgpu_ctx *c, const double *fb, const double *f, const double *fc, double *ff) {
  {
    TFields A; A.fb[0] = A.fb[1] = fb; A.f[0] = A.f[1] = f; A.fcl[0] = A.fcl[1] = fc; A.ff[0] = A.ff[1] = ff; A.rtf = NULL;
#if POMGPU_UVM_ONLOAD
    if (c->P.uvm) { LAUNCHN(c, "k_advt2_col", (k_advt2_col<1, true>), grid1_halo_r(c->P, LDS_ROWS), blk_col_r(LDS_ROWS), c->P, A); return; }
#endif
    LAUNCHN(c, "k_advt2_col", (k_advt2_col<1>), grid1_halo_r(c->P, LDS_ROWS), blk_col_r(LDS_ROWS), c->P, A);
  }
}
void launch_advt2x2_col(pomgpu_ctx *c, const double *tb, const double *t, const double *tc, double *tf, const double *sb, const double *s_,
                        const double *sc, double *sf, unsigned long long *rtf) {
  TFields A; A.fb[0] = tb; A.f[0] = t; A.fcl[0] = tc; A.ff[0] = tf; A.fb[1] = sb; A.f[1] = s_; A.fcl[1] = sc; A.ff[1] = sf; A.rtf = rtf;
  if (rtf) {
#if POMGPU_UVM_ONLOAD
    if (c->P.uvm) { LAUNCHN(c, "k_advt2x2_col", (k_advt2_col<2, true, true>), grid1_halo_r(c->P, LDS_ROWS), blk_col_r(LDS_ROWS), c->P, A); return; }
#endif
// ... 9 lines not shown
```

### extpom_amd/csrc/pomgpu_api.hip

```cpp
#include <math.h>
#include <stdarg.h>
#include <stdio.h>
#include <stdlib.h>
#include <string.h>
#include <vector>
#include "pomgpu.h"
#include "pomgpu_internal.hpp"

struct ProfPair { int slot; hipEvent_t a, b; };
struct ProfState { std::vector<ProfPair> pending; std::vector<ProfPair> free_; char filter[64]; };
static ProfState *PS(pomgpu_ctx *c) { return (ProfState *)c->prof_state; }

#define SLOT2(c, n) ((c)->P.b2 + (size_t)(n) * (c)->P.n2)
#define SLOT3(c, n) ((c)->P.b3 + (size_t)(n) * (c)->P.a3)
#define D2(c, name) SLOT2(c, P2_##name)
#define D3(c, name) SLOT3(c, P3_##name)
#define LEV3(c, p, lev) ((double *)((pomgpu_st *)(p) + (size_t)(lev) * (c)->P.n2))

int pomgpu_fail(pomgpu_ctx *c, int code, const char *fmt, ...) {
  if (c && c->parent) c = c->parent;
  if (c) {
    va_list ap;
    va_start(ap, fmt);
    vsnprintf(c->err, sizeof c->err, fmt, ap);
// ... 175 lines not shown
}

static const int X2_SLOT[POMGPU_NGEN] = {P2_ua, P2_va, P2_d, P2_el, P2_elb, P2_uab, P2_vab};
static void ext_buffers(pomgpu_ctx *c) {
  KP &P = c->P;
  for (int n = 0; n < POMGPU_NGEN; n++) P.x2[n] = P.y2[n] = c->ext_parity ? c->alt2[n] : P.b2 + (size_t)X2_SLOT[n] * P.n2;
}
static void rho_materialize(pomgpu_ctx *c) {
  if (!c->rho_rt_pending || (c->flags & POMGPU_CTX_2D)) return;
  c->rho_rt_pending = c->rho_rt_cols = 0;
  launch_roundtrip(c, SLOT3(c, P3_rho), SLOT3(c, P3_rmean), 2);
}
static void side_join(pomgpu_ctx *c);
static void side_begin(pomgpu_ctx *c);
static void side_end(pomgpu_ctx *c, hipEvent_t ev);
static int rim_side(pomgpu_ctx *c);
static void early_invalidate(pomgpu_ctx *c);
void pomgpu_wr_materialize(pomgpu_ctx *c) {
  if (!c->wr_pending) return;
  c->wr_pending = 0;
  (void)hipSetDevice(c->device);
  if (!(c->flags & POMGPU_CTX_2D)) launch_realvertvl(c, 1);
}
static bool wr_on_demand(const pomgpu_ctx *c) {
  return !c->exch && !c->tp.on && !c->wide.on && !c->parent && !(c->flags & POMGPU_CTX_2D) && !c->wr_eager && !SW(c, WR_NODEFER);
}
static bool uv_fused(const pomgpu_ctx *c) {
  const KP &P = c->P;
  return !c->exch && !c->tp.on && !c->wide.on && !c->parent && !(c->flags & POMGPU_CTX_2D) && !c->wr_eager && pomgpu_reg_kb(c) &&
         P.im >= 8 && P.jm >= 8 && !SW(c, UV_NOFUSE);
}
static bool w_fused(const pomgpu_ctx *c) {
  return POMGPU_W_FUSE && !c->exch && !c->tp.on && !c->wide.on && !(c->flags & POMGPU_CTX_2D) && !SW(c, ADVQ_SINGLE) && !SW(c, ADVQ_EXCHANGE) &&
         !SW(c, VERTVL_CELLS) && !SW(c, W_NOFUSE);
}
static bool uvm_onload(const pomgpu_ctx *c) {
  const pom_blkcon &k = c->con;
  return POMGPU_UVM_ONLOAD && w_fused(c) && uv_fused(c) && c->uvm_valid && !SW(c, UVMEAN_PASS) &&
         (k.mode == 4 || (k.nadv == 2 && c->P.nitera == 1 && !SW(c, ADVT2_SINGLE))) &&
         (!c->ntr || (k.nadv == 2 && c->P.nitera == 1));
}
static bool rt_one_tile(const pomgpu_ctx *c) { return !c->exch && !c->tp.on && !c->wide.on && !c->parent && !(c->flags & POMGPU_CTX_2D) && !c->wr_eager; }
static bool ld_on_demand(const pomgpu_ctx *c) {
  return !c->exch && !c->tp.on && !c->wide.on && !c->parent && !(c->flags & POMGPU_CTX_2D) && !c->wr_eager && !SW(c, LD_EAGER);
}
static bool next_step_fetches_record(const pomgpu_ctx *c) {
  if (!c->frc_on && !c->lat_on && !c->wat_on) return false;
  const pom_blkcon &k = c->con;
  const int isrf = (int)(.125 * 86400. / k.dti), ibc = (int)((double)(1.f / 24.f) * 86400. / k.dti), iwater = (int)(86400. / k.dti);
  const int next = k.iint + 1 + k.cont_bry;
  return (c->frc_on && (isrf < 1 || next % isrf == 0)) || (c->lat_on && (ibc < 1 || next % ibc == 0)) ||
         (c->wat_on && (iwater < 1 || (k.iint + 1) % iwater == 0));
}
static void uvf_materialize(pomgpu_ctx *c) {
  if (!c->uvf_pending) return;
  c->uvf_pending = 0;
  launch_uvf_copy(c);
}
static void restore_materialize(pomgpu_ctx *c) {
  c->uvm_valid = 0;
  side_join(c);
  rho_materialize(c);
  pomgpu_wr_materialize(c);
  uvf_materialize(c);
  if (!c->rst_pending) return;
  c->rst_pending = 0;
  launch_restore_fields(c, c->rst_fold, c->rst_fnew);
}
static void ext_flush_deferred(pomgpu_ctx *c);
static void ext_canonical(pomgpu_ctx *c) {
  ext_flush_deferred(c);
  if (!c->ext_parity) return;
  KP &P = c->P;
  for (int n = 0; n < POMGPU_NGEN; n++) launch_copy2(c, P.b2 + (size_t)X2_SLOT[n] * P.n2, c->alt2[n]);
  c->ext_parity = 0;
  ext_buffers(c);
}
static int ctx_create(pomgpu_ctx **out, const pomgpu_dims *d, int device, void *stream, int flags);
extern "C" int pomgpu_create(pomgpu_ctx **out, const pomgpu_dims *d, int device, void *stream) {
  return ctx_create(out, d, device, stream, 0);
}
static int ctx_create(pomgpu_ctx **out, const pomgpu_dims *d, int device, void *stream, int flags) {
  if (!out || !d) return POMGPU_EINVAL;
  *out = NULL;
  if (d->kb < 4 || d->kb > POMGPU_KBMAX || d->im < 5 || d->jm < 5 || d->im > d->im_local || d->jm > d->jm_local) {
    fprintf(stderr, "pomgpu_create: unsupported extents im=%d jm=%d kb=%d (need im,jm>=5, 4<=kb<=%d)\n", d->im, d->jm,
            d->kb, POMGPU_KBMAX);
    return POMGPU_EINVAL;
  }
  if ((size_t)d->im_local * d->jm_local * d->kb * sizeof(double) >= ((size_t)1 << 32)) {
    fprintf(stderr, "pomgpu_create: a 3-D array of this tile has %zu bytes; the column kernels address a level with 32-bit offsets "
                    "(< 4 GiB per array): split the domain into more tiles\n", (size_t)d->im_local * d->jm_local * d->kb * sizeof(double));
    return POMGPU_EINVAL;
  }
  int ndev = 0;
  if (hipGetDeviceCount(&ndev) != hipSuccess || ndev <= 0 || device < 0 || device >= ndev) {
    fprintf(stderr, "pomgpu_create: no usable HIP device (count=%d, asked %d); the hot path has no CPU fallback\n", ndev,
            device);
    return POMGPU_ENODEV;
  }
  pomgpu_ctx *c = (pomgpu_ctx *)calloc(1, sizeof(pomgpu_ctx));
  if (!c) return POMGPU_ENOMEM;
  c->device = device;
  c->flags = flags;
  c->lbry_sides = POMGPU_SIDE_EAST | POMGPU_SIDE_SOUTH;
  if (hipSetDevice(device) != hipSuccess) { free(c); return POMGPU_EHIP; }
  KP &P = c->P;
  P.im = d->im; P.jm = d->jm; P.kb = d->kb; P.imm1 = d->im - 1; P.jmm1 = d->jm - 1; P.kbm1 = d->kb - 1; P.kbm2 = d->kb - 2;
  P.iml = d->im_local; P.jml = d->jm_local;
  P.W = d->n_west == -1; P.E = d->n_east == -1; P.S = d->n_south == -1; P.N = d->n_north == -1;
  P.n2 = (size_t)P.iml * P.jml; P.n3 = P.n2 * P.kb;
  pomgpu_switches_read(c->sw);
  {
    const long pages = SW(c, PAD3) ? SWV(c, PAD3) : 0;
    P.a3 = P.n3 + (pages > 0 ? (size_t)pages * 512 : 0);
  }
  set_band_geometry(P, c->sw);
// ... 11 lines not shown
  else {
    if (hipStreamCreateWithFlags(&c->stream, hipStreamNonBlocking) != hipSuccess) { free(c); return POMGPU_EHIP; }
    c->own_stream = true;
  }
  c->cur = c->stream;
  c->prof_state = new ProfState();
  PS(c)->filter[0] = 0;
  bool ok = true;
  auto alloc = [&](double **p, size_t n) {
    if (!ok) return;
    if (hipMalloc((void **)p, n * sizeof(double)) != hipSuccess) { ok = false; *p = NULL; return; }
    if (hipMemsetAsync(*p, 0, n * sizeof(double), c->stream) != hipSuccess) ok = false;
  };
  alloc(&P.b1, (size_t)POM_NBLK1D * P.kb);
  alloc(&P.r1, (size_t)POM_NBLK1D * P.kb);
  alloc(&P.b2, (size_t)POM_NBLK2D * P.n2);
  const bool only2d = (flags & POMGPU_CTX_2D) != 0;
  if (!only2d) alloc(&P.b3, (size_t)POM_NBLK3D * P.a3);
  alloc(&P.bd, nbd);
  for (int n = 0; n < POMGPU_NSCR3 && !only2d; n++) alloc(&P.s3[n], P.n3);
  for (int n = 0; n < POMGPU_NSCR2; n++) alloc(&P.s2[n], P.n2);
  for (int n = 0; n < 2 && !only2d; n++) alloc(&c->uvb_bot[n], P.n2);
  if (!only2d) {
    double *m = NULL; alloc(&m, (size_t)(P.kb > 1 ? P.kb - 1 : 1) * P.jml * RT_NBX(P)); c->rt_words = (unsigned long long *)m;
    m = NULL; alloc(&m, (P.n2 + 1) / 2); c->rt_cols = (unsigned *)m;
  }
  for (int n = 0; n < POMGPU_NCOEF2; n++) alloc(&P.c2[n], P.n2);
  alloc(&c->alt2[0], (size_t)POMGPU_NGEN * P.n2);
  for (int n = 1; n < POMGPU_NGEN && ok; n++) c->alt2[n] = c->alt2[0] + (size_t)n * P.n2;
  { double *m = NULL; alloc(&m, (P.n2 + 7) / 8 + 1); P.m8 = (unsigned char *)m; }
  for (int n = 0; n < 2; n++) {
    const size_t len = (size_t)(P.kb + 1) * (n == 0 ? P.jml : P.iml);
    alloc(&c->ord_send[n], len);
    alloc(&c->ord_recv[n], len);
  }
  if (ok) { P.g4[2] = c->ord_recv[0]; P.g4[0] = c->ord_recv[0] + P.jml; P.g4[3] = c->ord_recv[1]; P.g4[1] = c->ord_recv[1] + P.iml; }
  alloc(&c->d_vel, 4);
  alloc(&c->d_stats, 8);
  if (ok && hipMalloc((void **)&c->d_err, sizeof(int)) != hipSuccess) ok = false;
  if (ok && hipMalloc((void **)&c->d_areas, sizeof(int)) != hipSuccess) ok = false;
  if (ok && hipMemsetAsync(c->d_areas, 0, sizeof(int), c->stream) != hipSuccess) ok = false;
  if (ok && hipMemsetAsync(c->d_err, 0, sizeof(int), c->stream) != hipSuccess) ok = false;
  if (SW(c, DEBUG_ALLOC))
    fprintf(stderr, "pomgpu_create: b1 %p r1 %p b2 %p b3 %p bd %p s3[0] %p s3[4] %p s2[0] %p c2[0] %p\n", (void *)P.b1, (void *)P.r1, (void *)P.b2,
            (void *)P.b3, (void *)P.bd, (void *)P.s3[0], (void *)P.s3[4], (void *)P.s2[0], (void *)P.c2[0]);
  if (!ok) {
    fprintf(stderr, "pomgpu_create: device allocation failed (%zu MB per 3-D array)\n", P.n3 * 8 >> 20);
    pomgpu_destroy(c);
    return POMGPU_ENOMEM;
  }
  c->ext_parity = 0;
  c->rst_pending = 0;
  ext_buffers(c);
  (void)hipStreamSynchronize(c->stream);
  *out = c;
  return POMGPU_OK;
}

static void wide_free(pomgpu_ctx *c);
extern "C" void pomgpu_destroy(pomgpu_ctx *c) {
  if (!c) return;
  (void)hipSetDevice(c->device);
  if (c->stream) (void)hipStreamSynchronize(c->stream);
  if (c->side) (void)hipStreamSynchronize(c->side);
  if (pomgpu_io_wait(c) != POMGPU_OK)
    fprintf(stderr, "pomgpu_destroy: the output / restart file still being written could not be completed -- call pomgpu_io_wait (or pomgpu_sync) "
                    "before pomgpu_destroy to get its status\n");
  wide_free(c);
  pomgpu_tp_free(c);
  pomgpu_ff_free(c);
  KP &P = c->P;
  (void)hipFree(P.r1);
  if (c->tune_block) {
    (void)hipFree(c->tune_block);
    c->tune_block = NULL; P.b3 = NULL;
    for (int n = 0; n < POMGPU_NSCR3; n++) P.s3[n] = NULL;
  }
  (void)hipFree(P.b1); (void)hipFree(P.b2); (void)hipFree(P.b3); (void)hipFree(P.bd);
  for (int n = 0; n < POMGPU_NSCR3; n++) (void)hipFree(P.s3[n]);
  for (int n = 0; n < POMGPU_NSCR2; n++) (void)hipFree(P.s2[n]);
  (void)hipFree(c->uvb_bot[0]); (void)hipFree(c->uvb_bot[1]);
  (void)hipFree(c->rt_words); (void)hipFree(c->rt_cols);
  for (int n = 0; n < POMGPU_NCOEF2; n++) (void)hipFree(P.c2[n]);
  (void)hipFree(c->alt2[0]); (void)hipFree(c->alt3[0]);
  (void)hipFree(P.m8);
  for (int n = 0; n < 2; n++) { (void)hipFree(c->ord_send[n]); (void)hipFree(c->ord_recv[n]); }
  for (int n = 0; n <= POMGPU_MAXREC; n++) { (void)hipFree(c->rec_t[n]); (void)hipFree(c->rec_s[n]); (void)hipFree(c->rec_tau[n]); }
  (void)hipFree(c->d_vel); (void)hipFree(c->d_err); (void)hipFree(c->d_areas); (void)hipFree(c->d_stats); (void)hipFree(c->ext_bar);
  for (int k = 0; k < 3; k++) for (int sl = 0; sl < 4; sl++) { (void)hipFree(c->frc_dev[k][sl][0]); (void)hipFree(c->frc_dev[k][sl][1]); }
  for (int sl = 0; sl < 4; sl++) { (void)hipFree(c->lat_dev[sl]); (void)hipFree(c->wat_dev[sl]); }
  (void)hipFree(c->mean_acc);
  tracers_free(c);
  ProfState *ps = PS(c);
  if (ps) {
    for (auto &p : ps->pending) { (void)hipEventDestroy(p.a); (void)hipEventDestroy(p.b); }
    for (auto &p : ps->free_) { (void)hipEventDestroy(p.a); (void)hipEventDestroy(p.b); }
    delete ps;
  }
  if (c->side) {
    (void)hipEventDestroy(c->ev_fork); (void)hipEventDestroy(c->ev_early);
    for (auto &e : c->side_ev) (void)hipEventDestroy(e.ev);
    (void)hipStreamDestroy(c->side);
  }
  if (c->own_stream && c->stream) (void)hipStreamDestroy(c->stream);
  free(c);
}

extern "C" int pomgpu_debug_switch(pomgpu_ctx *c, const char *name, const char *value) {
  if (!c || !name) return POMGPU_EINVAL;
  if (strncmp(name, "POMGPU_", 7) == 0) name += 7;
  for (int n = 0; n < SW__count; n++)
    if (strcmp(POMGPU_SW_NAMES[n], name) == 0) {
      pomgpu_ctx *two[2] = {c, c->wide.x};
      for (pomgpu_ctx *t : two)
        if (t) { t->sw.on[n] = value ? 1 : 0; t->sw.val[n] = value ? atol(value) : 0; }
      return POMGPU_OK;
    }
  return fail(c, POMGPU_EINVAL, "debug_switch: no switch named %s", name);
}
extern "C" const char *pomgpu_last_error(const pomgpu_ctx *c) { return c ? c->err : "null context"; }
extern "C" void *pomgpu_stream(pomgpu_ctx *c) { return c ? (void *)c->stream : NULL; }
extern "C" void *pomgpu_current_stream(pomgpu_ctx *c) { return c ? (void *)c->cur : NULL; }

static int pull_err(pomgpu_ctx *c) {
  if (c->launch_err) return POMGPU_EHIP;
  int e = 0;
  HIPCHK(c, hipMemcpyAsync(&e, c->d_err, sizeof(int), hipMemcpyDeviceToHost, c->stream));
  HIPCHK(c, hipStreamSynchronize(c->stream));
  if (e) c->con.error_status = 1;
  if (e & POMGPU_DERR_BARRIER) {
    pomgpu_ctx *two[2] = {c, c->wide.x};
    for (pomgpu_ctx *t : two)
      if (t && t->ext_bar) {
        (void)hipMemsetAsync(t->ext_bar, 0, 2 * sizeof(unsigned), c->stream);
        t->ext_bar_base = 0;
        t->ext_loop_off = 1;
      }
  }
  return POMGPU_OK;
}
extern "C" int pomgpu_sync(pomgpu_ctx *c) {
  if (!c) return POMGPU_EINVAL;
  side_join(c);
  HIPCHK(c, hipStreamSynchronize(c->stream));
  { const int rio = pomgpu_io_wait(c); if (rio) return rio; }
  return c->launch_err ? POMGPU_EHIP : POMGPU_OK;
}

extern "C" int pomgpu_set_con(pomgpu_ctx *c, const pom_blkcon *con, int lramp) {
  if (!c || !con) return POMGPU_EINVAL;
  if (c->wr_pending && con->dti2 != c->P.dti2) pomgpu_wr_materialize(c);
  c->con = *con;
  c->lramp = lramp;
  sync_scalars(c);
  return POMGPU_OK;
}
extern "C" int pomgpu_get_con(pomgpu_ctx *c, pom_blkcon *con) {
  if (!c || !con) return POMGPU_EINVAL;
  int rc = pull_err(c);
  if (rc) return rc;
  *con = c->con;
  return POMGPU_OK;
}
static int check_masks(pomgpu_ctx *c, const double *blk2d) {
  const int slots[3] = {P2_fsm, P2_dum, P2_dvm};
  for (int s = 0; s < 3; s++) {
    const double *m = blk2d + (size_t)slots[s] * c->P.n2;
    for (size_t n = 0; n < c->P.n2; n++)
// ... 178 lines not shown
  if (!c || !dev || !nz || (dir != 0 && dir != 1)) return POMGPU_EINVAL;
  return launch_halo_unpack(c, dev, nz, count, dir, from_lo, from_hi) ? fail(c, POMGPU_EINVAL, "halo_unpack: bad array list") : POMGPU_OK;
}
extern "C" int pomgpu_halo_pack8(pomgpu_ctx *c, double *const *dev, const int *nz, int count, double *const *to) {
  if (!c || !dev || !nz || !to) return POMGPU_EINVAL;
  return launch_halo_pack8(c, dev, nz, count, to) ? fail(c, POMGPU_EINVAL, "halo_pack8: bad array list") : POMGPU_OK;
}
extern "C" int pomgpu_halo_unpack8(pomgpu_ctx *c, double *const *dev, const int *nz, int count, const double *const *from) {
  if (!c || !dev || !nz || !from) return POMGPU_EINVAL;
  return launch_halo_unpack8(c, dev, nz, count, from) ? fail(c, POMGPU_EINVAL, "halo_unpack8: bad array list") : POMGPU_OK;
}

static double *dev3(pomgpu_ctx *c, const double *host) {
  if (!c->host3 || !host) return NULL;
  const ptrdiff_t off = host - c->host3;
  if (off < 0 || (size_t)off >= (size_t)POM_NBLK3D * c->P.n3 || (size_t)off % c->P.n3) return NULL;
  if ((size_t)off / c->P.n3 == P3_taurstrb) pomgpu_tau_touched(c, 0);
  if ((size_t)off / c->P.n3 == P3_taurstrf) pomgpu_tau_touched(c, 1);
  return SLOT3(c, (size_t)off / c->P.n3);
}
static double *dev2(pomgpu_ctx *c, const double *host) {
  if (!c->host2 || !host) return NULL;
  const ptrdiff_t off = host - c->host2;
  if (off < 0 || (size_t)off >= (size_t)POM_NBLK2D * c->P.n2 || (size_t)off % c->P.n2) return NULL;
  return c->P.b2 + off;
}

static void xch(pomgpu_ctx *c, int count, ...) {
  if (!c->exch) return;
  double *ptr[8];
  int nz[8];
  va_list ap;
  va_start(ap, count);
  for (int n = 0; n < count; n++) { ptr[n] = va_arg(ap, double *); nz[n] = va_arg(ap, int); }
  va_end(ap);
  c->exch(c->exch_user, ptr, nz, count);
}

static void seq_advave(pomgpu_ctx *c) {
  KP &P = c->P;
  if (!c->exch && P.mode != 2) { launch_advave_fused(c); return; }
  launch_advave_a(c);
  xch(c, 2, P.s2[0], 1, P.s2[1], 1);
  launch_advave_b(c);
  xch(c, 3, D2(c, advua), 1, D2(c, fluxua), 1, D2(c, fluxva), 1);
  launch_advave_c(c);
  xch(c, 1, D2(c, advva), 1);
  if (P.mode == 2) {
    launch_advave_m2a(c);
    xch(c, 1, P.s2[2], 1);
    launch_advave_m2b(c);
  }
}
static void seq_advct(pomgpu_ctx *c, int sum2d = 0, int defer_xch = 0) {
  KP &P = c->P;
  if (!c->exch) {
    launch_advct_col(c, sum2d);
    c->uvm_valid = POMGPU_UVM_ONLOAD && !c->tp.on && !c->wide.on && !(c->flags & POMGPU_CTX_2D);
    return;
  }
  if (c->tp.on && !SW(c, ADVCT_SPLIT)) {
    pomgpu_transport &T = c->tp;
    const size_t ne = 2 * (size_t)P.kbm1 * P.jm, nn = 2 * (size_t)P.kbm1 * P.im;
    const size_t sc[8] = {0, T.nbr[1] >= 0 ? ne : 0, 0, T.nbr[3] >= 0 ? nn : 0, 0, 0, 0, 0};
    const size_t rc[8] = {T.nbr[0] >= 0 ? ne : 0, 0, T.nbr[2] >= 0 ? nn : 0, 0, 0, 0, 0, 0};
    const bool side = rim_side(c);
    double *const *snd = side ? T.send2 : T.send, *const *rcv = side ? T.recv2 : T.recv;
    if (side) side_begin(c);
    launch_advct_edge(c, T.nbr[1] >= 0 ? snd[1] : NULL, T.nbr[3] >= 0 ? snd[3] : NULL);
    const int rcm = side ? pomgpu_tp_move_side(c, sc, rc) : pomgpu_tp_move(c, sc, rc);
    if (side) side_end(c, c->side_ev[SIDE_R1].ev);
    if (rcm) return;
    launch_advct_col(c, sum2d);
    if (side) (void)hipStreamWaitEvent(c->stream, c->side_ev[SIDE_R1].ev, 0);
    launch_advct_fix(c, T.nbr[0] >= 0 ? rcv[0] : NULL, T.nbr[2] >= 0 ? rcv[2] : NULL);
    if (sum2d) launch_advct_fix2d(c, T.nbr[0] >= 0, T.nbr[2] >= 0);
    if (!defer_xch) xch(c, 2, D3(c, advx), P.kb, D3(c, advy), P.kb);
    return;
  }
  launch_advct_a(c);
  xch(c, 2, P.s3[0], P.kbm1, P.s3[1], P.kbm1);
  launch_advct_b(c);
  xch(c, 2, D3(c, advx), P.kb, P.s3[4], P.kbm1);
  launch_advct_c(c);
  xch(c, 1, D3(c, advy), P.kb);
}
static void seq_rho_roundtrip(pomgpu_ctx *c, int defer_rt, int cols = 0) {
  if (defer_rt) {
    launch_roundtrip_level(c, D3(c, rho), D3(c, rmean), c->P.kb);
    c->rho_rt_pending = 1;
    c->rho_rt_cols = cols;
  } else {
    launch_roundtrip(c, D3(c, rho), D3(c, rmean), 0);
  }
}
static void seq_baropg(pomgpu_ctx *c, int sum2d = 0, int defer_rt = 0) {
  const int cols = launch_baropg(c, sum2d, (defer_rt && rt_one_tile(c)) ? c->rt_cols : NULL);
  seq_rho_roundtrip(c, defer_rt, cols);
}
static void seq_baropg_mcc(pomgpu_ctx *c, int sum2d = 0, int defer_rt = 0) {
  KP &P = c->P;
  if (c->order) {
    launch_order_pack(c, c->ord_send[0], c->ord_send[1]);
    c->order(c->order_user, c->ord_send[0], (P.kb + 1) * P.jml, c->ord_send[1], (P.kb + 1) * P.iml, c->ord_recv[0], c->ord_recv[1]);
  }
  launch_baropg_mcc(c, sum2d);
  seq_rho_roundtrip(c, defer_rt);
}
static void seq_advq(pomgpu_ctx *c, double *qb, double *q, double *qf, int pair, int zero_else) {
  KP &P = c->P;
// ... 173 lines not shown
  if (hipStreamCreateWithFlags(&c->side, hipStreamNonBlocking) != hipSuccess) { c->side = NULL; return 0; }
  bool ok = hipEventCreateWithFlags(&c->ev_fork, hipEventDisableTiming) == hipSuccess && hipEventCreateWithFlags(&c->ev_early, hipEventDisableTiming) == hipSuccess;
  for (auto &e : c->side_ev) ok = ok && hipEventCreateWithFlags(&e.ev, hipEventDisableTiming) == hipSuccess;
  if (!ok) {
    (void)hipStreamDestroy(c->side);
    c->side = NULL;
    return 0;
  }
#ifdef POMGPU_EMU
  emu_stream_defer(c->side);
#endif
  return 1;
}
#define NEED_RAW(c) if (!(c)) return POMGPU_EINVAL; if ((c)->broken) return POMGPU_EHIP; (void)hipSetDevice((c)->device)
static void wide_flush(pomgpu_ctx *c);
#define NEED_HOT(c) NEED_RAW(c); ext_canonical(c); wide_flush(c)
#define NEED(c) NEED_HOT(c); side_join(c); restore_materialize(c)

int pomgpu_materialize(pomgpu_ctx *c) {
  NEED(c);
  return POMGPU_OK;
}
void pomgpu_mirrors_written(pomgpu_ctx *c) {
  c->uvm_valid = 0;
  c->rho_rt_cols = 0;
  c->wide.static_done = 0;
  early_invalidate(c);
  refresh_coefs(c);
}
void pomgpu_cold_tail(pomgpu_ctx *c, void (*update_initial)(pomgpu_ctx *), void (*sums)(pomgpu_ctx *)) {
  launch_dens(c, D3(c, sclim), D3(c, tclim), D3(c, rmean));
  launch_dens(c, D3(c, sb), D3(c, tb), D3(c, rho));
  update_initial(c);
  if (c->con.npg == 2) seq_baropg_mcc(c); else seq_baropg(c);
  sums(c);
  pomgpu_tau_touched(c, 0); pomgpu_tau_touched(c, 1);
  pomgpu_mirrors_written(c);
}
extern "C" int pomgpu_get_time(pomgpu_ctx *c) {
  NEED_HOT(c);
  pom_blkcon &k = c->con;
  k.time = k.dti * (double)(float)k.iint / 86400. + k.time0;
  if (k.iint >= k.iswtch) k.iprint = (int)lround(k.prtd2 * 24. * 3600. / k.dti);
  if (c->lramp) { k.ramp = k.time / k.period; if (k.ramp > 1.) k.ramp = 1.; }
  else k.ramp = 1.;
  sync_scalars(c);
  return POMGPU_OK;
}
static int lateral_viscosity(pomgpu_ctx *c, int sum2d, int defer_rt = 0) {
  NEED_HOT(c);
  side_wait(c, SIDE_RTS);
  rho_materialize(c);
  KP &P = c->P;
  if (P.mode != 2) {
    const bool lib_x = c->tp.on && c->exch && !SW(c, ADVCT_SPLIT);
    auto pressure_gradient = [&]() {
      if (P.npg == 1) seq_baropg(c, sum2d, defer_rt);
      else if (P.npg == 2) seq_baropg_mcc(c, sum2d, defer_rt);
      else {
        fprintf(stderr, "\nError: invalid value for npg\n");
        c->con.error_status = 1;
      }
    };
    const bool pg_first = c->side_ev[SIDE_R8].pending != 0;
    if (pg_first) pressure_gradient();
    side_wait(c, SIDE_R8);
    seq_advct(c, sum2d, lib_x);
    if (!pg_first) pressure_gradient();
    launch_aam(c);
    if (lib_x && sum2d && rim_side(c)) {
      double *arr[3] = {D3(c, advx), D3(c, advy), D3(c, aam)};
      const int nz[3] = {P.kb, P.kb, P.kbm1};
      side_begin(c);
      const int rc2 = round8(c, 1, arr, nz, 3);
      if (!rc2) launch_vint(c, 1, -1);
      side_post(c, SIDE_R2);
      if (rc2) return rc2;
    }
    else if (lib_x) xch(c, 3, D3(c, advx), P.kb, D3(c, advy), P.kb, D3(c, aam), P.kbm1);
    else xch(c, 1, D3(c, aam), P.kbm1);
  }
  return POMGPU_OK;
}
static int wide_early_start(pomgpu_ctx *c);
extern "C" int pomgpu_lateral_viscosity(pomgpu_ctx *c) {
  NEED_HOT(c);
  const int rc = wide_early_start(c);
  const pom_blkcon &k0 = c->con;
  const int defer_rt = k0.mode == 3 && (k0.iint != 1 || k0.time0 != 0.) && !SW(c, RHO_ROUNDTRIP);
  return rc ? rc : lateral_viscosity(c, 0, defer_rt);
}
static int wide_begin(pomgpu_ctx *c);
static int mode_interaction(pomgpu_ctx *c, int sums_done) {
  NEED_HOT(c);
  if (c->wide.on) {
    if (c->P.mode != 2) launch_vint(c, sums_done, sums_done && c->side_ev[SIDE_R2].pending ? 1 : 0);
    return wide_begin(c);
  }
  if (c->P.mode != 2) {
    launch_vint(c, sums_done);
    seq_advave(c);
  }
  launch_modeint_tail(c);
  xch(c, 2, D2(c, utf), 1, D2(c, vtf), 1);
  return POMGPU_OK;
}
static KP row_window(const KP &P, int lo, int hi) {
  KP Q = P;
  const size_t sh = (size_t)lo * P.iml;
  Q.b2 += sh;
  for (int n = 0; n < POMGPU_NSCR2; n++) if (Q.s2[n]) Q.s2[n] += sh;
  for (int n = 0; n < POMGPU_NCOEF2; n++) if (Q.c2[n]) Q.c2[n] += sh;
  for (int n = 0; n < POMGPU_NGEN; n++) { Q.x2[n] += sh; Q.y2[n] += sh; }
  if (Q.m8) Q.m8 += sh;
  int s = 0;
#define BD_(name, shape) Q.bdoff[s++] += BDW_##shape;
#define BDW_J ((size_t)lo)
#define BDW_I 0
#define BDW_JK 0
#define BDW_IK 0
  POM_BDRY(BD_)
#undef BD_
  Q.jm = P.jm - lo - hi; Q.jmm1 = Q.jm - 1; Q.jml = Q.jm;
  return Q;
}
static int mode_external(pomgpu_ctx *c, int store_f) {
  NEED_RAW(c);
  if (c->wide.on && c->wide.pending) {
    pomgpu_ctx *x = c->wide.x;
    x->con.iext = c->con.iext;
    const int last = c->con.iext == c->con.isplit;
    const int rc = mode_external(x, store_f || last);
    if (last) wide_flush(c);
    return rc;
  }
  KP &P = c->P;
  P.iext = c->con.iext;
  if (!c->exch && !SW(c, EXT_SPLIT)) {
    const int fuse_adv = c->con.ispadv == 1 && P.mode != 2 && !SW(c, ADVAVE_SEPARATE);
    if (!fuse_adv && c->con.ispadv > 0 && c->con.iext % c->con.ispadv == 0) seq_advave(c);
    KP Q = P;
    for (int n = 0; n < POMGPU_NGEN; n++) Q.y2[n] = c->ext_parity ? P.b2 + (size_t)X2_SLOT[n] * P.n2 : c->alt2[n];
    if (fuse_adv && !c->areas_checked) { launch_check_areas(c); c->areas_checked = 1; }
    if (c->parent && !SW(c, WIDE_FULL)) {
      const pomgpu_wide &Wd = c->parent->wide;
      int cut = P.iext - 1 < Wd.w - 5 ? P.iext - 1 : Wd.w - 5;
      if (cut < 0) cut = 0;
      const int lo = Wd.oy > 0 ? cut : 0, hi = P.jm - c->parent->P.jm - Wd.oy > 0 ? cut : 0;
      if (lo + hi > 0 && P.jm - lo - hi >= 16) Q = row_window(Q, lo, hi);
    }
    launch_ext_step(c, Q, store_f || P.iext == P.isplit, fuse_adv);
    c->ext_parity ^= 1;
    ext_buffers(c);
    return POMGPU_OK;
  }
// ... 416 lines not shown
    else if (one_pass) {
      launch_advt2_rows(c, a.trb, a.tr, a.clim, a.trf);
      if (!lib_x) xch(c, 1, a.trf, P.kbm1);
      launch_copy_kb(c, a.trb);
    } else seq_advt2(c, a.trb, a.tr, a.clim, a.trf, true);
    n += 1;
  }
  for (int n = 0; n < ntr; n++) {
    const pomgpu_ctx::pomgpu_tracer &a = c->trc[n];
    if (a.q || a.lam != 0.) launch_tr_source(c, a.trf, a.trb, rt ? a.clim : NULL, a.q, a.lam);
  }
  {
    double *ptr[POMGPU_TRMAX];
    int nz[POMGPU_TRMAX];
    for (int n = 0; n < ntr; n++) { ptr[n] = c->trc[n].trf; nz[n] = P.kbm1; }
    xchv(c, ptr, nz, ntr);
  }
  side_wait(c, SIDE_RQ);
  for (int n = 0; n < ntr;) {
    const pomgpu_ctx::pomgpu_tracer &a = c->trc[n];
    const int nf = (pairs && n + 1 < ntr) ? 2 : 1;
    const pomgpu_ctx::pomgpu_tracer &b = c->trc[n + nf - 1];
    if (nf == 1 || !launch_proft2(c, a.trf, a.wsurf, a.surf, a.nbc, b.trf, b.wsurf, b.surf, b.nbc)) {
      launch_proft(c, a.trf, a.wsurf, a.surf, a.nbc);
      if (nf == 2) launch_proft(c, b.trf, b.wsurf, b.surf, b.nbc);
    }
    const TrEdge e[2] = {{a.trf, a.tr, a.bd[0], a.bd[1], a.bd[2], a.bd[3]}, {b.trf, b.tr, b.bd[0], b.bd[1], b.bd[2], b.bd[3]}};
    launch_tr_edges(c, e, nf);
    const TrUpd u[2] = {{a.trf, a.clim, a.tr, a.trb}, {b.trf, b.clim, b.tr, b.trb}};
    launch_tr_update(c, u, nf, rt);
    n += nf;
  }
  return POMGPU_OK;
}
static int wr_on_side(pomgpu_ctx *c, int with_kernel) {
  const KP &P = c->P;
  side_wait(c, SIDE_WR);
  side_begin(c);
  if (with_kernel) launch_realvertvl(c);
  double *arr[1] = {D3(c, wr)};
  const int nz[1] = {P.kbm1};
  const int rcw = round8(c, 1, arr, nz, 1);
  side_post(c, SIDE_WR);
  return rcw;
}
static int mode_internal(pomgpu_ctx *c, int defer_wr) {
  NEED_HOT(c);
  KP &P = c->P;
  const pom_blkcon &k = c->con;
  side_wait(c, SIDE_R2);
  side_wait(c, SIDE_R8);
  if ((k.iint != 1 || k.time0 != 0.) && k.mode != 2) {
    c->uvf_pending = 0;
    struct UvmScope { pomgpu_ctx *c; ~UvmScope() { c->P.uvm = 0; c->uvm_valid = 0; } } uvm_scope{c};
    P.uvm = uvm_onload(c) ? 1 : 0;
    if (!P.uvm) launch_int_uvmean(c);
    const bool wf = w_fused(c);
    if (!wf) launch_vertvl(c, 1);
    const bool lib_x = c->tp.on && c->exch;
    const bool rimr = lib_x && rim_side(c) && !SW(c, RIM_RESULTS_MAIN) && !SW(c, ADVQ_EXCHANGE) && !SW(c, PROD_FULL);
    if (rimr) {
      double *aw[1] = {D3(c, w)};
      const int nw[1] = {P.kb};
      const int rcw = rim_round(c, SIDE_RW, aw, nw, 1);
      if (rcw) return rcw;
    }
    else if (!lib_x) xch(c, 1, D3(c, w), P.kb);
    launch_coef_eta(c, P.uvm);
    if (!c->exch || !SW(c, ADVQ_EXCHANGE)) {
      if (SW(c, ADVQ_SINGLE)) {
        launch_advq_col(c, D3(c, q2), D3(c, q2b), D3(c, uf), 1);
        launch_advq_col(c, D3(c, q2l), D3(c, q2lb), D3(c, vf), 1);
#if POMGPU_W_FUSE
      } else if (wf) {
        launch_advq2w_col(c, D3(c, q2), D3(c, q2b), D3(c, uf), D3(c, q2l), D3(c, q2lb), D3(c, vf), 1);
#endif
      } else {
        launch_advq2_col(c, D3(c, q2), D3(c, q2b), D3(c, uf), D3(c, q2l), D3(c, q2lb), D3(c, vf), 1);
      }
    } else {
      double *x0 = P.s3[0], *y0 = P.s3[1], *x1 = P.s3[2], *y1 = P.s3[3];
      launch_advq_flux(c, D3(c, q2), D3(c, q2b), x0, y0);
      launch_advq_flux(c, D3(c, q2l), D3(c, q2lb), x1, y1);
      xch(c, 4, x0, P.kbm1, y0, P.kbm1, x1, P.kbm1, y1, P.kbm1);
      launch_advq_step(c, D3(c, q2), D3(c, q2b), D3(c, uf), x0, y0, 1);
      launch_advq_step(c, D3(c, q2l), D3(c, q2lb), D3(c, vf), x1, y1, 1);
    }
    const int qfuse = !SW(c, QFILTER_SPLIT);
    if (rimr) {
      launch_profq_bc(c);
      launch_profq(c, 1, qfuse, c->rho_rt_pending, P.S ? 1 : 2, P.N ? P.jm : P.jmm1);
    } else {
      seq_profq(c, qfuse, lib_x, !(defer_wr && ld_on_demand(c) && !next_step_fetches_record(c)));
      xch(c, 2, LEV3(c, D3(c, uf), 1), P.kbm2, LEV3(c, D3(c, vf), 1), P.kbm2);
    }
    launch_bcond6_edges(c);
    if (qfuse) launch_q_filter_rim(c);
    else launch_q_filter(c, 1);
    if (rimr) {
      double *aq[9] = {D3(c, q2), D3(c, q2b), D3(c, q2l), D3(c, q2lb), D3(c, km), D3(c, kh), D3(c, kq), D3(c, l), D3(c, dtef)};
      const int nq[9] = {P.kb, P.kb, P.kb, P.kb, P.kb, P.kb, P.kb, P.kb, P.kb};
      const int rcq = rim_round(c, SIDE_RQ, aq, nq, 9);
      if (rcq) return rcq;
    }
    side_wait(c, SIDE_RW);
    if (k.mode != 4) {
// ... 561 lines not shown
  }
  const int ph_ext = prof_phase_open(c);
  if (!ext_loop_all(c))
  for (int iext = 1; iext <= c->con.isplit; iext++) {
    if (ext_pair(c, iext)) { iext++; continue; }
    c->con.iext = iext;
    if ((rc = mode_external(c, 0))) return rc;
  }
  prof_phase_close(c, ph_ext, "phase_external");
  c->con.iext = c->con.isplit + 1;
  if ((rc = mode_internal(c, more_steps_follow))) return rc;
  if (c->mean_acc && (rc = mean_accumulate(c))) return rc;
  launch_check_velocity(c);
  prof_phase_close(c, ph_step, "phase_step");
  return POMGPU_OK;
}
extern "C" int pomgpu_run(pomgpu_ctx *c, int nsteps) {
  NEED_HOT(c);
  c->wr_deferred = 0;
  for (int n = 0; n < nsteps; n++) {
    c->con.iint += 1;
    int rc = advance(c, n + 1 < nsteps);
    if (rc) return rc;
  }
  return POMGPU_OK;
}

static int piece_move(pomgpu_ctx *c, double *dst, const double *src, size_t n) {
  if (dst == src || !n) return POMGPU_OK;
  const size_t shift = dst > src ? (size_t)(dst - src) : (size_t)(src - dst), chunk = shift < n ? shift : n;
  const size_t nch = (n + chunk - 1) / chunk;
  for (size_t q = 0; q < nch; q++) {
    const size_t m = dst > src ? nch - 1 - q : q;
    const size_t o = m * chunk, len = (o + chunk <= n ? chunk : n - o);
    HIPCHK(c, hipMemcpyAsync(dst + o, src + o, len * sizeof(double), hipMemcpyDeviceToDevice, c->stream));
  }
  return POMGPU_OK;
}
struct TuneLay { size_t f, a; };
static double *tune_piece(const pomgpu_ctx *c, const TuneLay &L, int i) {
  return c->tune_block + L.f + (i < POM_NBLK3D ? (size_t)i * L.a : (size_t)POM_NBLK3D * L.a + (size_t)(i - POM_NBLK3D) * c->P.n3);
}
static int tune_relayout(pomgpu_ctx *c, TuneLay to) {
  const int np = POM_NBLK3D + POMGPU_NSCR3;
  auto one_way = [&](const TuneLay &from, const TuneLay &dst_) -> int {
    const bool up = dst_.f >= from.f && dst_.a >= from.a;
    for (int q = 0; q < np; q++) {
      const int i = up ? np - 1 - q : q;
      const int rc = piece_move(c, tune_piece(c, dst_, i), tune_piece(c, from, i), c->P.n3);
      if (rc) return rc;
    }
    return POMGPU_OK;
  };
  const TuneLay cur = {c->tune_front, c->P.a3};
  int rc = POMGPU_OK;
  if ((to.f >= cur.f && to.a >= cur.a) || (to.f <= cur.f && to.a <= cur.a)) rc = one_way(cur, to);
  else {
    const TuneLay mid = {to.f > cur.f ? to.f : cur.f, to.a > cur.a ? to.a : cur.a};
    rc = one_way(cur, mid);
    if (!rc) rc = one_way(mid, to);
  }
  if (rc) return rc;
  KP &P = c->P;
  c->tune_front = to.f;
  P.a3 = to.a;
  P.b3 = c->tune_block + to.f;
  for (int n = 0; n < POMGPU_NSCR3; n++) P.s3[n] = P.b3 + (size_t)POM_NBLK3D * P.a3 + (size_t)n * P.n3;
  return POMGPU_OK;
}
extern "C" int pomgpu_tune_placement(pomgpu_ctx *c, int steps, int max_try, double *ms_out, long *front_mib_out, long *pad_mib_out, int *ntried, int *kept) {
  NEED(c);
  if (ntried) *ntried = 0;
  if (kept) *kept = 0;
  if (c->mean_acc)
    return fail(c, POMGPU_EINVAL, "tune_placement: the time-mean output is on and the trial steps would count -- tune first, switch the mean on afterwards");
  if (c->ntr)
    return fail(c, POMGPU_EINVAL, "tune_placement: passive tracers are registered and the trial steps would move them -- tune first, register tracers afterwards");
#ifdef POMGPU_EMU
  (void)steps; (void)max_try; (void)ms_out; (void)front_mib_out; (void)pad_mib_out;
  return POMGPU_OK;
#else
  KP &P = c->P;
  if ((c->flags & POMGPU_CTX_2D) || !P.b3 || steps < 1 || max_try < 1) return fail(c, POMGPU_EINVAL, "tune_placement: a context with 3-D arrays, steps >= 1, max_try >= 1");
  if (c->dev3_handed)
    return fail(c, POMGPU_EINVAL, "tune_placement: pomgpu_device_3d has handed out addresses of the 3-D arrays, which this call would leave dangling -- tune first, take addresses afterwards");
  if (P.n3 * sizeof(double) < ((size_t)64 << 20) && !SW(c, TUNE_FORCE)) return POMGPU_OK;
  const size_t unit = 2 * P.n3;
  size_t pad1 = P.n3 * sizeof(double) >= ((size_t)512 << 20) ? ((size_t)256 << 20) / sizeof(double) : (P.n3 / 4 + 8191) / 8192 * 8192;
  HIPCHK(c, hipStreamSynchronize(c->stream));
  if (c->side) HIPCHK(c, hipStreamSynchronize(c->side));
  if (!c->tune_block) {
    size_t fre = 0, tot = 0;
    HIPCHK(c, hipMemGetInfo(&fre, &tot));
    const size_t a0 = P.a3;
    size_t amax = a0 + pad1;
    auto need = [&](int kmax, size_t am) { return ((size_t)kmax * unit + (size_t)POM_NBLK3D * am + (size_t)POMGPU_NSCR3 * P.n3) * sizeof(double) + ((size_t)2 << 30); };
    int kmax = max_try > 12 ? 30 : 10;
    while (kmax > 0 && need(kmax, amax) > fre) kmax--;
    if (kmax < 1) { amax = a0; kmax = 10; while (kmax > 0 && need(kmax, amax) > fre) kmax--; }
    if (kmax < 1) return POMGPU_OK;
    double *blk = NULL;
    if (hipMalloc((void **)&blk, need(kmax, amax) - ((size_t)2 << 30)) != hipSuccess) { (void)hipGetLastError(); return POMGPU_OK; }
    for (int n = 0; n < POM_NBLK3D; n++)
      HIPCHK(c, hipMemcpyAsync(blk + (size_t)n * a0, P.b3 + (size_t)n * a0, P.n3 * sizeof(double), hipMemcpyDeviceToDevice, c->stream));
    for (int n = 0; n < POMGPU_NSCR3; n++)
      HIPCHK(c, hipMemcpyAsync(blk + (size_t)POM_NBLK3D * a0 + (size_t)n * P.n3, P.s3[n], P.n3 * sizeof(double), hipMemcpyDeviceToDevice, c->stream));
    HIPCHK(c, hipStreamSynchronize(c->stream));
    (void)hipFree(P.b3);
    for (int n = 0; n < POMGPU_NSCR3; n++) (void)hipFree(P.s3[n]);
    c->tune_block = blk;
    c->tune_front = 0;
    c->tune_kmax = kmax;
    c->tune_a0 = a0;
    c->tune_amax = amax;
    P.b3 = blk;
    for (int n = 0; n < POMGPU_NSCR3; n++) P.s3[n] = blk + (size_t)POM_NBLK3D * a0 + (size_t)n * P.n3;
  }
  static const int KS[20][2] = {{0, 0}, {3, 0}, {10, 0}, {0, 1}, {3, 1}, {10, 1}, {5, 0}, {5, 1}, {2, 0}, {1, 0}, {7, 0}, {4, 0}, {7, 1}, {2, 1}, {15, 0}, {20, 0}, {25, 0}, {30, 0}, {15, 1}, {20, 1}};
  hipEvent_t e0 = NULL, e1 = NULL;
  if (hipEventCreate(&e0) != hipSuccess || hipEventCreate(&e1) != hipSuccess) {
    if (e0) (void)hipEventDestroy(e0);
    return fail(c, POMGPU_EHIP, "tune_placement: hipEventCreate failed");
  }
  int n = 0, best = 0, rc = POMGPU_OK;
  TuneLay lay[20];
  double ms[20];
  for (int q = 0; q < 20 && n < max_try && !rc; q++) {
    if (KS[q][0] > c->tune_kmax || (KS[q][1] && c->tune_amax == c->tune_a0)) continue;
    lay[n].f = (size_t)KS[q][0] * unit;
    lay[n].a = KS[q][1] ? c->tune_amax : c->tune_a0;
    if ((rc = tune_relayout(c, lay[n]))) break;
    if ((rc = pomgpu_run(c, 1))) break;
    (void)hipEventRecord(e0, c->stream);
    if ((rc = pomgpu_run(c, steps))) break;
    side_join(c);
    (void)hipEventRecord(e1, c->stream);
    (void)hipEventSynchronize(e1);
    float t = 0.f;
    (void)hipEventElapsedTime(&t, e0, e1);
    ms[n] = (double)t / steps;
    if (ms[n] < ms[best]) best = n;
    n++;
  }
  (void)hipEventDestroy(e0); (void)hipEventDestroy(e1);
  if (!rc && n) rc = tune_relayout(c, lay[best]);
  if (!rc && hipStreamSynchronize(c->stream) != hipSuccess) rc = fail(c, POMGPU_EHIP, "tune_placement: hipStreamSynchronize failed");
  if (rc) {
    c->broken = 1;
    c->con.error_status = 1;
    return rc;
  }
  for (int q = 0; q < n; q++) {
    if (ms_out) ms_out[q] = ms[q];
    if (front_mib_out) front_mib_out[q] = (long)(lay[q].f * sizeof(double) >> 20);
    if (pad_mib_out) pad_mib_out[q] = (long)((lay[q].a - P.n3) * sizeof(double) >> 20);
  }
  if (ntried) *ntried = n;
  if (kept) *kept = best;
  return POMGPU_OK;
#endif
}

extern "C" int pomgpu_advave(pomgpu_ctx *c) { NEED(c); seq_advave(c); return POMGPU_OK; }
extern "C" int pomgpu_advct(pomgpu_ctx *c) { NEED(c); seq_advct(c); return POMGPU_OK; }
extern "C" int pomgpu_baropg(pomgpu_ctx *c) { NEED(c); seq_baropg(c); return POMGPU_OK; }
extern "C" int pomgpu_baropg_mcc(pomgpu_ctx *c) { NEED(c); seq_baropg_mcc(c); return POMGPU_OK; }
extern "C" int pomgpu_advq(pomgpu_ctx *c, const double *qb, const double *q, const double *qf) {
  NEED(c);
  double *a = dev3(c, qb), *b = dev3(c, q), *d = dev3(c, qf);
// ... 144 lines not shown
```

### extpom_amd/csrc/pomgpu_internal.hpp

```cpp
#pragma once
#include <hip/hip_runtime.h>
#include <stddef.h>
#include <stdlib.h>
#include "pom_layout.h"

#ifndef COL_ROWS
#define COL_ROWS 4
#endif
#ifndef COL_WX
#define COL_WX 1
#endif
#define POMGPU_NSCR3 8
#define POMGPU_NSCR2 8
#define POMGPU_NCOEF2 25
#define POMGPU_MAXREC 8
#define POMGPU_TRMAX 8
#define POMGPU_KBMAX 128
#define POMGPU_CTX_2D 1
#define POMGPU_DERR_VELOCITY 1
#define POMGPU_DERR_BARRIER 2
#define POMGPU_NGEN 7

struct KP {
  int im, jm, kb, imm1, jmm1, kbm1, kbm2, iml, jml;
  int W, E, S, N;
  size_t n2, n3;
  size_t a3;
  double *b1, *b2, *b3, *bd;
  double *r1;
  double *s3[POMGPU_NSCR3];
  double *s2[POMGPU_NSCR2];
  double *c2[POMGPU_NCOEF2];
  size_t bdoff[80];
  double alpha, dte, dti, dti2, dte2, grav, kappa, ramp, rfe, rfn, rfs, rfw, rhoref, sbias, small_,
         tbias, tprni, umol, horcon, ispi, isp2i, smoth, sw, time, vmaxl;
  int mode, ntp, nadv, nbct, nbcs, nitera, npg, isplit, iext, iint, iend;
  int g_rb, g_nbx, g_bpl;
  int g_lin;
  int g_strip;
  double const1_profq, cb_profq;
  double *x2[POMGPU_NGEN], *y2[POMGPU_NGEN];
  double *g4[4];
  unsigned char *m8;
  int uvm;
};
enum pomgpu_x2 { X2_ua, X2_va, X2_d, X2_el, X2_elb, X2_uab, X2_vab };

#ifdef POMGPU_STORE_F32
typedef float pomgpu_st;
#else
typedef double pomgpu_st;
#endif
#define POMGPU_ST_BYTES ((unsigned)sizeof(pomgpu_st))
#if defined(POMGPU_COMPUTE_F32) && !defined(POMGPU_STORE_F32)
#error "POMGPU_COMPUTE_F32 is the fp32-arithmetic variant of the fp32-storage build: it needs POMGPU_STORE_F32"
#endif
#ifdef POMGPU_COMPUTE_F32
typedef float pomgpu_ct;
#else
typedef double pomgpu_ct;
#endif
#define CT(x) ((pomgpu_ct)(x))
#ifdef POMGPU_COMPUTE_F32
#define POMGPU_W_FUSE 0
#else
#define POMGPU_W_FUSE 1
#endif
#ifdef POMGPU_COMPUTE_F32
#define POMGPU_UVM_ONLOAD 0
#else
#define POMGPU_UVM_ONLOAD 1
#endif
#ifdef POMGPU_STORE_F32
struct Ref3 {
  pomgpu_st *p;
  __device__ __forceinline__ operator double() const { return (double)*p; }
  __device__ __forceinline__ const Ref3 &operator=(double v) const { *p = (pomgpu_st)v; return *this; }
  __device__ __forceinline__ const Ref3 &operator=(const Ref3 &o) const { *p = *o.p; return *this; }
};
#define REF3(ptr, idx) (Ref3{(pomgpu_st *)(ptr) + (idx)})
#else
#define REF3(ptr, idx) ((ptr)[(idx)])
#endif

#define IX2(i, j) ((size_t)((j)-1) * (size_t)P.iml + (size_t)((i)-1))
#define IX3(i, j, k) ((size_t)((k)-1) * P.n2 + IX2(i, j))
#if !defined(POMGPU_EMU) && !defined(POMGPU_F1_GLOBAL)
typedef const double __attribute__((address_space(4))) *pomgpu_cptr;
#define F1(name, k) ((pomgpu_cptr)(size_t)P.b1)[(size_t)P1_##name * P.kb + ((k)-1)]
#define R1(name, k) ((pomgpu_cptr)(size_t)P.r1)[(size_t)P1_##name * P.kb + ((k)-1)]
#else
#define F1(name, k) P.b1[(size_t)P1_##name * P.kb + ((k)-1)]
#define R1(name, k) P.r1[(size_t)P1_##name * P.kb + ((k)-1)]
#endif
#define F2(name, i, j) P.b2[(size_t)P2_##name * P.n2 + IX2(i, j)]
#define F3(name, i, j, k) REF3(P.b3 + (size_t)P3_##name * P.a3, IX3(i, j, k))
#define A2(name) (P.b2 + (size_t)P2_##name * P.n2)
#define A3(name) (P.b3 + (size_t)P3_##name * P.a3)
#define G3(p, i, j, k) REF3(p, IX3(i, j, k))
#define G2(p, i, j) (p)[IX2(i, j)]

enum pom_bdry_slot_dev {
#define POMGPU_BD_(name, shape) PB_##name,
  POM_BDRY(POMGPU_BD_)
#undef POMGPU_BD_
  PB__count
};
#define BD1(name, a) P.bd[P.bdoff[PB_##name] + (size_t)((a)-1)]
#define BDJ(name, a, k) P.bd[P.bdoff[PB_##name] + (size_t)((k)-1) * P.jml + (size_t)((a)-1)]
#define BDI(name, a, k) P.bd[P.bdoff[PB_##name] + (size_t)((k)-1) * P.iml + (size_t)((a)-1)]

__device__ __forceinline__ double sq(double x) { return x * x; }

enum pomgpu_coef2 {
  C2_HSX, C2_HSY,
  C2_DYSX, C2_DXSX,
  C2_DXSY, C2_DYSY,
  C2_CMX, C2_CMY,
  C2_HEA, C2_HFA,
  C2_DTSX, C2_DTSY,
  C2_DT4,
  C2_DX4, C2_DY4,
  C2_CVA, C2_CVB,
  C2_R2DXSX, C2_R2DYSY,
// ... 224 lines not shown
    const int job = q * ROWS + r;
    const bool valid = job < 2 * NS;
    const int side = valid ? job / NS : 0;
    S.hop[q] = valid ? job % NS : 0;
    S.hrow[q] = valid ? (side ? ROWS + 1 : 0) : ROWS + 2;
    S.hoff[q] = valid ? BOFF2(i, side ? jnorth : jsouth) : BOFF_NONE;
  }
  return S;
}
template <int V, int NS, int ROWS> __device__ __forceinline__ UvmC rowshare_uvm(const KP &P, const RowShare<NS, ROWS> &S, int q, int op, int j0w, int i) {
  if (S.hop[q] != op || S.hrow[q] == ROWS + 2) return uvm_none();
  const int jsouth = j0w > 1 ? j0w - 1 : 1, jnorth = j0w + ROWS <= P.jml ? j0w + ROWS : P.jml;
  return uvm_of<V>(P, i, S.hrow[q] == 0 ? jsouth : jnorth);
}
template <int NS> __device__ __forceinline__ const double *rowshare_pick(const double *const (&b)[NS], int op) {
  const double *x = b[0];
#pragma unroll
  for (int o = 1; o < NS; o++)
    if (op == o) x = b[o];
#ifndef POMGPU_EMU
  const unsigned long long v = (unsigned long long)x;
  const unsigned lo = (unsigned)__builtin_amdgcn_readfirstlane((int)(unsigned)v), hi = (unsigned)__builtin_amdgcn_readfirstlane((int)(unsigned)(v >> 32));
  x = (const double *)(((unsigned long long)hi << 32) | lo);
#endif
  return x;
}

template <class T> struct InvDT { T b, y; };
typedef InvDT<double> InvD;
typedef InvDT<pomgpu_ct> InvDc;
__device__ __forceinline__ InvD inv_of(double b) { InvD d; d.b = b; d.y = 1.0 / b; return d; }
__device__ __forceinline__ InvDT<float> inv_of(float b) { InvDT<float> d; d.b = b; d.y = 1.0f / b; return d; }
#ifndef POMGPU_EMU
__device__ __forceinline__ double divi(double a, const InvD &d) {
  const double q0 = a * d.y;
  double r = __builtin_fma(-d.b, q0, a);
  double q = __builtin_fma(r, d.y, q0);
  r = __builtin_fma(-d.b, q, a);
  q = __builtin_fma(r, d.y, q);
  return a == 0. ? q0 : q;
}
__device__ __forceinline__ float divi(float a, const InvDT<float> &d) {
  const float q0 = a * d.y;
  float r = __builtin_fmaf(-d.b, q0, a);
  float q = __builtin_fmaf(r, d.y, q0);
  r = __builtin_fmaf(-d.b, q, a);
  q = __builtin_fmaf(r, d.y, q);
  return a == 0.f ? q0 : q;
}
#else
static inline double divi(double a, const InvD &d) { return a / d.b; }
static inline float divi(float a, const InvDT<float> &d) { return a / d.b; }
#endif
#define HALO_XCD_ORDER                                                                    \
  if (P.g_strip > 0) {                                                                    \
    const int st__ = P.g_strip, nfull__ = nbx__ / st__, wlast__ = nbx__ - nfull__ * st__; \
    int s__ = m__ / (rpx__ * st__);                                                       \
    if (s__ > nfull__) s__ = nfull__;                                                     \
    const int rem__ = m__ - s__ * rpx__ * st__, w__ = s__ < nfull__ ? st__ : (wlast__ > 0 ? wlast__ : 1); \
    byl__ = rem__ / w__; bxg__ = s__ * st__ + rem__ % w__;                                \
    if (bxg__ >= nbx__ || byl__ >= rpx__) return;                                         \
  } else {                                                                                \
    byl__ = m__ / nbx__; bxg__ = m__ % nbx__;                                             \
    if (byl__ >= rpx__) return;                                                           \
  }
#define HALO_XCD_DECODE HALO_XCD_DECODE_R(COL_ROWS)
#define HALO_XCD_DECODE_R(ROWS__)                                                         \
  const int g__ = (int)(blockIdx.x * blockDim.x + threadIdx.x);                           \
  const int L__ = g__ >> 6, nwx__ = (P.iml + 61) / 62, nbx__ = (nwx__ + COL_WX - 1) / COL_WX; \
  const int nby__ = (P.jml + ROWS__ - 1) / ROWS__;                                        \
  const int rpx__ = (nby__ + 7) / 8, m__ = L__ >> 3;                                      \
  int by__, bxg__;                                                                        \
  if (P.g_lin && 10 * nby__ < 72 * rpx__) {                                               \
    const int x__ = L__ & 7, T__ = nby__ * nbx__;                                         \
    const int c0__ = (int)(((long)x__ * T__) >> 3), c1__ = (int)(((long)(x__ + 1) * T__) >> 3); \
    const int t__ = c0__ + m__;                                                           \
    if (t__ >= c1__) return;                                                              \
    const int st__ = P.g_strip > 0 ? P.g_strip : nbx__, per__ = st__ * nby__, s__ = t__ / per__; \
    const int rem__ = t__ - s__ * per__, w__ = (s__ + 1) * st__ <= nbx__ ? st__ : nbx__ - s__ * st__; \
    by__ = rem__ / w__; bxg__ = s__ * st__ + rem__ % w__;                                 \
  } else {                                                                                \
    int byl__;                                                                            \
    HALO_XCD_ORDER                                                                        \
    by__ = (L__ & 7) * rpx__ + byl__;                                                     \
    if (by__ >= nby__) return;                                                            \
  }                                                                                       \
  const int lane = g__ & 63;                                                              \
  const int i0 = (bxg__ * COL_WX + (int)threadIdx.y % COL_WX) * 62 + lane;                \
  const int j = by__ * ROWS__ + (int)threadIdx.y / COL_WX + 1;
static inline dim3 grid1_halo_r(const KP &P, int rows) {
  const int nwx = (P.iml + 61) / 62, nbx = (nwx + COL_WX - 1) / COL_WX, nby = (P.jml + rows - 1) / rows, rpx = (nby + 7) / 8;
  if (P.g_lin && 10 * nby < 72 * rpx) return dim3((unsigned)(8 * ((nby * nbx + 7) / 8)), 1, 1);
  return dim3((unsigned)(8 * rpx * nbx), 1, 1);
}
static inline dim3 grid1_halo(const KP &P) { return grid1_halo_r(P, COL_ROWS); }
static inline dim3 blk_col_r(int rows) { return dim3(64, rows * COL_WX, 1); }
static inline dim3 blk_col() { return dim3(64, COL_ROWS * COL_WX, 1); }
#define HALO_COL (int)(((blockIdx.x * blockDim.x + threadIdx.x) >> 6) * 62 + ((blockIdx.x * blockDim.x + threadIdx.x) & 63))
static inline dim3 grid2_halo(const KP &P) { return dim3((P.iml + 61) / 62, (P.jml + 3) / 4, 1); }

#define TID_I (int)(blockIdx.x * blockDim.x + threadIdx.x + 1)
#define TID_J (int)(blockIdx.y * blockDim.y + threadIdx.y + 1)
#define TID_K (int)(blockIdx.z * blockDim.z + threadIdx.z + 1)

#define POMGPU_SWITCHES(X)                                                                                                    \
  X(THOMAS_SCRATCH) X(NO_PAIR) X(EXT_SPLIT) X(ADVAVE_SEPARATE) X(EXT_RIM_KERNEL) X(EXT_LOOP) X(EXT_NOMARCH) X(EXT_MARCH)      \
  X(EXT_ROWS) X(EXT_NOPAIR) X(EXT_PAIR) X(EXT_ROWS2) X(EXT_TWO_SETS) X(EXT_AREAS_LOAD) X(BAROPG_CELLS) X(VERTVL_CELLS)        \
  X(NO_LIN) X(ADVQ_SINGLE) X(ADVT2_SINGLE) X(REALVERTVL_CELLS) X(RHO_ROUNDTRIP) X(TAU_ARRAYS) X(PROFQ_ROWS8) X(PROFQ_ROWS2)    \
  X(PROFQ_NOPACE) X(COL_STRIP) X(BAND_BYTES) X(PAD3) X(IO_SYNC) X(ADVCT_SPLIT) X(ADVQ_EXCHANGE) X(PROD_FULL) X(QFILTER_SPLIT) \
  X(NO_OVERLAP) X(NO_SIDE_COMM) X(WR_MAIN) X(WIDE_W) X(WIDE_FULL) X(DEBUG_ALLOC) X(TEST_SPLIT_FAIL_RANK)  \
  X(WR_NODEFER) X(EXT_RING_FIRST) X(TUNE_FORCE) X(RIM_MAIN) X(RIM_RESULTS_MAIN) X(SUM2D_OFF) X(ADVCT_ROWS4) X(ADVCT_ROWS8) \
  X(IO_CHUNK_KB) X(UV_NOFUSE) X(W_NOFUSE) X(UVMEAN_PASS) X(PROFT_TWIN) X(LD_EAGER) X(TR_NOPAIR) X(RT_LOAD)
enum pomgpu_sw {
#define POMGPU_SW_(name) SW_##name,
  POMGPU_SWITCHES(POMGPU_SW_)
#undef POMGPU_SW_
  SW__count
};
struct pomgpu_switches {
  unsigned char on[SW__count];
  long val[SW__count];
};
static const char *const POMGPU_SW_NAMES[SW__count] = {
#define POMGPU_SW_(name) #name,
  POMGPU_SWITCHES(POMGPU_SW_)
#undef POMGPU_SW_
};
static inline void pomgpu_switches_read(pomgpu_switches &s) {
  for (int n = 0; n < SW__count; n++) {
    char var[64] = "POMGPU_";
    size_t k = 7;
    for (const char *q = POMGPU_SW_NAMES[n]; *q && k + 1 < sizeof var; q++) var[k++] = *q;
    var[k] = 0;
    const char *e = getenv(var);
    s.on[n] = e ? 1 : 0;
    s.val[n] = e ? atol(e) : 0;
  }
}
static inline unsigned pomgpu_switches_collective_digest(const pomgpu_switches &s) {
  static const int coll[] = {SW_ADVCT_SPLIT, SW_ADVQ_EXCHANGE, SW_PROD_FULL, SW_QFILTER_SPLIT, SW_NO_OVERLAP,
                             SW_NO_SIDE_COMM, SW_WR_MAIN, SW_WIDE_W, SW_WIDE_FULL, SW_EXT_SPLIT, SW_ADVAVE_SEPARATE, SW_WR_NODEFER, SW_RIM_MAIN, SW_ADVT2_SINGLE, SW_RIM_RESULTS_MAIN, SW_SUM2D_OFF};
  unsigned h = 2166136261u;
  for (size_t n = 0; n < sizeof coll / sizeof coll[0]; n++) {
    h = (h ^ (unsigned)(s.on[coll[n]] ? 1 + coll[n] : 0)) * 16777619u;
    h = (h ^ (unsigned)s.val[coll[n]]) * 16777619u;
  }
  return h & 0x3fffffffu;
}
#define SW(c, NAME) ((c)->sw.on[SW_##NAME] != 0)
#define SWV(c, NAME) ((c)->sw.val[SW_##NAME])
struct ProfEntry { const char *name; long launches; double ms; };
struct pomgpu_ctx;

static const int POMGPU_OPP[8] = {1, 0, 3, 2, 7, 6, 5, 4};
struct pomgpu_transport {
  int on;
  int nbr[8];
  void (*fn)(void *, const double *const *, const size_t *, double *const *, const size_t *);
  void *user;
  void *rccl;
  double *send[8], *recv[8];
  size_t cap[8];
  double *send2[8], *recv2[8];
  size_t cap2[8];
  int fn_ordered;
// ... 12 lines not shown
  size_t scount[8], rcount[8];
  RectTable early_pack, early_unpack, late_pack, late_unpack;
  size_t e_scount[8], e_rcount[8], l_scount[8], l_rcount[8];
  int split;
  int pending;
  int static_done;
};
enum side_round { SIDE_WR, SIDE_R1, SIDE_R2, SIDE_R8, SIDE_RW, SIDE_RQ, SIDE_RTS, SIDE__count };

struct pomgpu_ctx {
  KP P;
  pomgpu_switches sw;
  int device;
  hipStream_t stream;
  bool own_stream;
  hipStream_t cur, side;
  hipEvent_t ev_fork, ev_early;
  struct { hipEvent_t ev; int pending; } side_ev[SIDE__count];
  int early_started;
  double *tune_block;
  size_t tune_front;
  int tune_kmax;
  size_t tune_a0, tune_amax;
  int dev3_handed;
  int broken;
  int wr_deferred;
  pom_blkcon con;
  int lramp;
  double *rec_t[POMGPU_MAXREC + 1], *rec_s[POMGPU_MAXREC + 1];
  const double *host2, *host3;
  void (*exch)(void *, double *const *, const int *, int);
  void *exch_user;
  void (*order)(void *, const double *, int, const double *, int, double *, double *);
  void *order_user;
  double *ord_send[2], *ord_recv[2];
  double *alt2[POMGPU_NGEN];
  double *alt3[POMGPU_NGEN];
  int ext_parity;
  int ext_deferred;
  int tau_known[2];
  double tau_val[2];
  double *rec_tau[POMGPU_MAXREC + 1];
  long tau_id[2], tau_gen;
  int tau_same, rate_in_f, tau_handed;
  int rho_rt_pending;
  unsigned long long *rt_words;
  unsigned *rt_cols;
  int rho_rt_cols;
  int rst_pending;
  double rst_fold, rst_fnew;
  int wr_pending;
  int uvf_pending;
  int uvm_valid;
  double *uvb_bot[2];
  int wr_eager;
  double *d_vel;
  int *d_err;
  int *d_areas;
  int areas_checked;
  double *d_stats;
  double *frc_dev[3][4][2];
  int frc_n[3][4];
  double *lat_dev[4];
  int lat_n[4];
  int frc_on, lat_on;
  double *wat_dev[4];
  int wat_n[4];
  int wat_on;
  int sss_on;
  bool prof_on;
  ProfEntry prof[96];
  int nprof;
  void *prof_state;
  pomgpu_transport tp;
  pomgpu_wide wide;
  pomgpu_ctx *parent;
  int flags;
  unsigned *ext_bar;
  unsigned ext_bar_base;
  int ext_loop_off;
  void *io_job;
  int z_init, z_clim;
  int z_lbry;
  int lbry_sides;
  void *frc_files;
  int launch_err;
  double *mean_acc;
  size_t mean_off[9];
  int mean_count;
  int ntr;
  struct pomgpu_tracer { double *trb, *tr, *trf, *clim, *q, *wsurf, *surf, *bd[4]; int nbc; double lam; } trc[POMGPU_TRMAX];
  double *tr_zero3;
  double *trmean_acc;
  size_t trmean_stride;
  int trmean_count;
  double *d_trstats;
  char err[512];
};
static inline bool pomgpu_reg_kb(const pomgpu_ctx *c) { return c->P.kb >= 6 && c->P.kb <= 64 && !SW(c, THOMAS_SCRATCH); }

int pomgpu_prof_slot(pomgpu_ctx *c, const char *name);
void pomgpu_prof_pre(pomgpu_ctx *c);
void pomgpu_prof_post(pomgpu_ctx *c, int slot);
int pomgpu_fail(pomgpu_ctx *c, int code, const char *fmt, ...);
void pomgpu_launch_check(pomgpu_ctx *c, const char *name);

// ... 4 lines not shown
    hipLaunchKernelGGL(kern, grid, block, 0, (c)->cur, __VA_ARGS__);             \
    pomgpu_launch_check((c), #kern);                                             \
    if (_s >= 0) pomgpu_prof_post((c), _s);                                      \
  } while (0)

#define LAUNCHN(c, name, kern, grid, block, ...)                                 \
  do {                                                                           \
    int _s = (c)->prof_on ? pomgpu_prof_slot((c), name) : -1;                    \
    if (_s >= 0) pomgpu_prof_pre(c);                                             \
    hipLaunchKernelGGL(kern, grid, block, 0, (c)->cur, __VA_ARGS__);             \
    pomgpu_launch_check((c), name);                                              \
    if (_s >= 0) pomgpu_prof_post((c), _s);                                      \
  } while (0)

static inline dim3 blk2() { return dim3(64, 4, 1); }
static inline dim3 grid2(const KP &P) { return dim3((P.iml + 63) / 64, (P.jml + 3) / 4, 1); }
static inline dim3 grid3(const KP &P, int nz) { return dim3((P.iml + 63) / 64, (P.jml + 3) / 4, nz); }
static inline dim3 gridm(const KP &P) {
  const long nbands = (P.jml + P.g_rb - 1) / P.g_rb;
  const long rounds = (nbands + 7) / 8;
  return dim3((unsigned)(8 * rounds * P.kb * P.g_bpl), 1, 1);
}
static inline void set_band_geometry(KP &P, const pomgpu_switches &sw) {
  long budget = 3L << 20;
  const bool e = sw.on[SW_BAND_BYTES] != 0;
  if (e && sw.val[SW_BAND_BYTES] >= 1024) budget = sw.val[SW_BAND_BYTES];
  long rows = budget / ((long)P.iml * 8 * 24);
  rows = (rows / 4) * 4;
  if (rows < 4) rows = 4;
  if (rows > ((P.jml + 3) / 4) * 4) rows = ((P.jml + 3) / 4) * 4;
  P.g_rb = (int)rows;
  P.g_nbx = (P.iml + 63) / 64;
  P.g_bpl = P.g_nbx * (int)(rows / 4);
  const int nbx = ((P.iml + 61) / 62 + COL_WX - 1) / COL_WX;
  const int nstr = (nbx + 11) / 12;
  P.g_strip = nbx >= 20 ? (nbx + nstr - 1) / nstr : 0;
  if (sw.on[SW_COL_STRIP]) P.g_strip = (int)sw.val[SW_COL_STRIP];
  P.g_lin = sw.on[SW_NO_LIN] ? 0 : 1;
  if (!e) {
    long best = -1, bslots = 0;
    for (long r = 4; r <= rows; r += 4) {
      const long nb = (P.jml + r - 1) / r, slots = (nb + 7) / 8 * 8 * r;
      if (best < 0 || slots < bslots || (slots == bslots && r > best)) { best = r; bslots = slots; }
    }
    P.g_rb = (int)best;
    P.g_bpl = P.g_nbx * (int)(best / 4);
  }
}

void launch_advave_a(pomgpu_ctx *c);
void launch_advave_b(pomgpu_ctx *c);
void launch_advave_c(pomgpu_ctx *c);
void launch_advave_fused(pomgpu_ctx *c);
void launch_advct_col(pomgpu_ctx *c, int sum2d);
void launch_advct_edge(pomgpu_ctx *c, double *to_e, double *to_n);
void launch_advct_fix(pomgpu_ctx *c, const double *from_w, const double *from_s);
void launch_advct_fix2d(pomgpu_ctx *c, int west, int south);
void launch_advt2x2_col(pomgpu_ctx *c, const double *tb, const double *t, const double *tc, double *tf, const double *sb, const double *s_,
                        const double *sc, double *sf, unsigned long long *rtf = NULL);
void launch_advq2_col(pomgpu_ctx *c, const double *q, const double *qb, double *qf, const double *ql, const double *qlb, double *qlf, int zero_else);
#if POMGPU_W_FUSE
void launch_advq2w_col(pomgpu_ctx *c, const double *q, const double *qb, double *qf, const double *ql, const double *qlb, double *qlf, int zero_else);
#endif
void launch_advuv_col(pomgpu_ctx *c);
int launch_profuv_reg(pomgpu_ctx *c);
void launch_profuv_filter_reg(pomgpu_ctx *c, double *ubk, double *vbk);
void launch_uv_filter_rim(pomgpu_ctx *c);
void launch_uvf_copy(pomgpu_ctx *c);
void launch_advave_m2a(pomgpu_ctx *c);
void launch_advave_m2b(pomgpu_ctx *c);
void launch_vint(pomgpu_ctx *c, int only_aam, int ghost = 0);
void launch_modeint_tail(pomgpu_ctx *c);
void launch_ext_elf(pomgpu_ctx *c);
void launch_ext_uvaf(pomgpu_ctx *c, int interior);
void launch_ext_update(pomgpu_ctx *c);
void launch_ext_step(pomgpu_ctx *c, const KP &Q, int store_f, int fuse_adv);
void launch_check_areas(pomgpu_ctx *c);
int launch_ext_loop(pomgpu_ctx *c, const KP &Q, int first, int last);
int launch_ext_pair_ok(const pomgpu_switches &sw, const KP &Q);
int launch_ext_pair(pomgpu_ctx *c, const KP &Q, double *const *T, int store_f2);
void launch_copy2(pomgpu_ctx *c, double *dst, const double *src);
void launch_lat(pomgpu_ctx *c, int phase, const double *rec, double fold, double fnew);
void launch_frc_load(pomgpu_ctx *c, const double *ra, const double *rb, double *xf, double *yf);
void launch_frc_interp(pomgpu_ctx *c, double fold, double fnew, double *x, const double *xb, const double *xf, double *y, const double *yb,
                       const double *yf);
void launch_frc_load1(pomgpu_ctx *c, const double *ra, double *xf, double *xb);
void launch_frc_interp1(pomgpu_ctx *c, double fold, double fnew, double *x, const double *xb, const double *xf);
void launch_int_tail(pomgpu_ctx *c);
void launch_bcond1(pomgpu_ctx *c);
void launch_advct_a(pomgpu_ctx *c);
void launch_advct_b(pomgpu_ctx *c);
void launch_advct_c(pomgpu_ctx *c);
void launch_aam(pomgpu_ctx *c);
void launch_roundtrip(pomgpu_ctx *c, double *a, const double *b, int fix_kb);
void launch_roundtrip_level(pomgpu_ctx *c, double *a, const double *b, int k);
void launch_advq_flux(pomgpu_ctx *c, const double *q, const double *qb, double *xf, double *yf);
void launch_advq_step(pomgpu_ctx *c, const double *q, const double *qb, double *qf, const double *xf, const double *yf, int zero_else);
void launch_q_filter(pomgpu_ctx *c, int mask);
void launch_q_filter_rim(pomgpu_ctx *c);
void launch_mask_q(pomgpu_ctx *c);
void launch_advt1(pomgpu_ctx *c, double *fb, double *f, const double *fclim, double *ff);
void launch_copy_kb(pomgpu_ctx *c, double *f, double *g = NULL);
void launch_advt2_mass(pomgpu_ctx *c);
void launch_advt2_step(pomgpu_ctx *c, const double *fbmem, const double *f, const double *eta, double *ff, int itera);
void launch_mask3(pomgpu_ctx *c, double *a, const double *m2);
void launch_smol(pomgpu_ctx *c, const double *ff);
void launch_copy3(pomgpu_ctx *c, double *dst, const double *src);
void launch_advt2_diff(pomgpu_ctx *c, const double *fb, const double *fc, double *ff);
void launch_ts_update(pomgpu_ctx *c, double fold, double fnew, int rt, int store_rst, int rt_flags = 0);
void launch_restore_fields(pomgpu_ctx *c, double fold, double fnew);
void launch_mask_ts(pomgpu_ctx *c);
struct TrUpd { const double *ff, *fc; double *f, *fb; };
void launch_tr_update(pomgpu_ctx *c, const TrUpd *u, int nf, int rt);
void launch_mask_uv(pomgpu_ctx *c);
void launch_mask_w(pomgpu_ctx *c);
void launch_restore(pomgpu_ctx *c, double fold, double fnew);
void launch_restore_shift(pomgpu_ctx *c);
void launch_restore_load(pomgpu_ctx *c, const double *tr, const double *sr, double tau, const double *taur = NULL, int fill_tau = 1);
void launch_dens(pomgpu_ctx *c, const double *si, const double *ti, double *rhoo);
void launch_realvertvl(pomgpu_ctx *c, int etf_is_et = 0);
int launch_baropg(pomgpu_ctx *c, int sum2d, unsigned *rtcol = NULL);
void launch_baropg_mcc(pomgpu_ctx *c, int sum2d);
void launch_order_pack(pomgpu_ctx *c, double *send_e, double *send_n);
void launch_int_uvmean(pomgpu_ctx *c);
void launch_vertvl(pomgpu_ctx *c, int mask);
void launch_profq_bc(pomgpu_ctx *c);
void launch_profq_prod(pomgpu_ctx *c, int lines_only, int rho_rt = 0);
void launch_profq(pomgpu_ctx *c, int fuse_prod, int fuse_filter, int rho_rt = 0, int jfirst = 0, int jlast = -1, int store_ld = 1);
void launch_proft(pomgpu_ctx *c, double *f, const double *wfsurf, const double *fsurf, int nbc);
int launch_proft2(pomgpu_ctx *c, double *f0, const double *wfsurf0, const double *fsurf0, int nbc0, double *f1, const double *wfsurf1, const double *fsurf1, int nbc1);
void launch_advu_profu(pomgpu_ctx *c, int do_adv, int do_prof);
void launch_advv_profv(pomgpu_ctx *c, int do_adv, int do_prof);
void launch_uv_filter(pomgpu_ctx *c, int own = 0);
void launch_coef_static(pomgpu_ctx *c);
void launch_coef_dt(pomgpu_ctx *c);
void launch_coef_eta(pomgpu_ctx *c, int uvm = 0);
void launch_advt2_rows(pomgpu_ctx *c, const double *fb, const double *f, const double *fc, double *ff);
void launch_advq_col(pomgpu_ctx *c, const double *q, const double *qb, double *qf, int zero_else);
void launch_bcond4_edges(pomgpu_ctx *c);
void launch_bcond6_edges(pomgpu_ctx *c);
void launch_bcondorl3(pomgpu_ctx *c);
struct TrEdge { double *ff; const double *f, *be, *bw, *bn, *bs; };
void launch_tr_edges(pomgpu_ctx *c, const TrEdge *e, int nf);
void launch_tr_source(pomgpu_ctx *c, double *ff, const double *fb, const double *fc, const double *q, double lam);
int launch_halo_pack(pomgpu_ctx *c, double *const *dev, const int *nz, int count, int dir, double *to_lo, double *to_hi);
int launch_halo_pack8(pomgpu_ctx *c, double *const *dev, const int *nz, int count, double *const *to);
int launch_halo_unpack8(pomgpu_ctx *c, double *const *dev, const int *nz, int count, const double *const *from);
int launch_halo_unpack(pomgpu_ctx *c, double *const *dev, const int *nz, int count, int dir, const double *from_lo, const double *from_hi);
void launch_rect_jobs(pomgpu_ctx *c, const RectJob *jobs_dev, int njobs, int max_ni, int max_nj);
int pomgpu_tp_move(pomgpu_ctx *c, const size_t *scount, const size_t *rcount);
int pomgpu_tp_move_ptr(pomgpu_ctx *c, const double *const *send, const size_t *scount, double *const *recv, const size_t *rcount);
int pomgpu_tp_setup(pomgpu_ctx *c, const int *nbr8);
int pomgpu_tp_rccl(pomgpu_ctx *c, const void *id128, int rank, int nranks, const char *librccl_path);
void pomgpu_tp_free(pomgpu_ctx *c);
int pomgpu_tp_reserve(pomgpu_ctx *c, const size_t *need);
int pomgpu_tp_reserve2(pomgpu_ctx *c, const size_t *need);
void pomgpu_wr_materialize(pomgpu_ctx *c);
int pomgpu_materialize(pomgpu_ctx *c);
void pomgpu_mirrors_written(pomgpu_ctx *c);
void pomgpu_cold_tail(pomgpu_ctx *c, void (*update_initial)(pomgpu_ctx *), void (*sums)(pomgpu_ctx *));
// ... 29 lines not shown
```

Baseline: 4.969 billion.

## Fuse Smagorinsky aam computation and its vertical sum into advct column kernel

Computes the new horizontal viscosity aam inside the advct column kernel, which already holds u and v for each level. It also accumulates the depth-integrated aam2d there, which removes the separate launch_aam pass and lets vint skip recomputing the 2D sum. Because advct must keep reading the old aam while writing the new one, the code ping-pongs between the canonical aam slot and a newly allocated spare buffer. Consumers read through a P.aamc pointer, and an aam_canonical copy step restores the canonical layout wherever other paths need it. The cost is an extra full 3D allocation, more parity bookkeeping, and higher register pressure in the advct kernel.

```diff
diff --git a/extpom_amd/csrc/k_adv.hip b/extpom_amd/csrc/k_adv.hip
--- a/extpom_amd/csrc/k_adv.hip
+++ b/extpom_amd/csrc/k_adv.hip
@@ -366,6 +366,12 @@
 }
 __device__ __forceinline__ void c_copy3(const KP &P, const int i, const int j, const int k, double *dst, const double *src) {
   G3(dst, i, j, k) = G3(src, i, j, k);
+}
+__device__ __forceinline__ void c_aam_copy(const KP &P, const int i, const int j, const int k, double *dst, const double *src) {
+  if (k <= P.kbm1) G3(dst, i, j, k) = G3(src, i, j, k);
+}
+__global__ void k_aam_copy(KP P, double *dst, const double *src) {
+  MARCH3(c_aam_copy(P, i, j, k, dst, src))
 }
 __device__ __forceinline__ double advt2_xdiff(const KP &P, const double *fb, const double *fc, int i, int j, int k) {
   const double am = 0.5 * (aam_(i, j, k) + aam_(i - 1, j, k));
@@ -769,12 +775,6 @@
   return P.horcon * dx * dy *
          sqrt(sq((u_e - u_c) / dx) + sq((v_n - v_c) / dy) +
               .5 * sq(.25 * (u_n + u_ne - u_s - u_se) / dy + .25 * (v_e + v_ne - v_w - v_nw) / dx));
-}
-__device__ __forceinline__ double aam_point_r(const KP &P, const InvD &dx, const InvD &dy, double u_c, double u_e, double u_n, double u_ne, double u_s,
-                                              double u_se, double v_c, double v_n, double v_e, double v_ne, double v_w, double v_nw) {
-  return P.horcon * dx.b * dy.b *
-         sqrt(sq(divi(u_e - u_c, dx)) + sq(divi(v_n - v_c, dy)) +
-              .5 * sq(divi(.25 * (u_n + u_ne - u_s - u_se), dy) + divi(.25 * (v_e + v_ne - v_w - v_nw), dx)));
 }
 #ifndef AAM_KCH
 #define AAM_KCH 7
@@ -880,6 +880,7 @@
 void launch_mask3(pomgpu_ctx *c, double *a, const double *m2) { LAUNCH(c, k_mask3, gridm(c->P), blk2(), c->P, a, m2); }
 void launch_smol(pomgpu_ctx *c, const double *ff) { LAUNCH(c, k_smol, gridm(c->P), blk2(), c->P, ff); }
 void launch_copy3(pomgpu_ctx *c, double *dst, const double *src) { LAUNCH(c, k_copy3, gridm(c->P), blk2(), c->P, dst, src); }
+void launch_aam_copy(pomgpu_ctx *c, double *dst, const double *src) { LAUNCH(c, k_aam_copy, gridm(c->P), blk2(), c->P, dst, src); }
 void launch_advt2_diff(pomgpu_ctx *c, const double *fb, const double *fc, double *ff) { LAUNCH(c, k_advt2_diff, gridm(c->P), blk2(), c->P, fb, fc, ff); }
 void launch_ts_update(pomgpu_ctx *c, double fold, double fnew, int rt, int store_rst, int rt_flags) {
   const unsigned long long *rtf = (rt && rt_flags) ? c->rt_words : NULL;
diff --git a/extpom_amd/csrc/k_tile.hip b/extpom_amd/csrc/k_tile.hip
--- a/extpom_amd/csrc/k_tile.hip
+++ b/extpom_amd/csrc/k_tile.hip
@@ -100,7 +100,7 @@
   const double *ps[NS];
 #pragma unroll
   for (int f = 0; f < NF; f++) { ps[f] = A.fb[f]; ps[NF + f] = A.fcl[f]; bff[f] = BUF3(A.ff[f]); }
-  ps[AM] = A3(aam); ps[VV] = A3(v); bo[0] = BUF3(A3(u)); bo[1] = BUF3(A3(w));
+  ps[AM] = P.aamc; ps[VV] = A3(v); bo[0] = BUF3(A3(u)); bo[1] = BUF3(A3(w));
 #pragma unroll
   for (int x = 0; x < NS; x++) bs[x] = BUF3(ps[x]);
   const RowShare<NS> S = rowshare_setup<NS>(P, r, j, j0w, i);
@@ -153,7 +153,7 @@
     nb.s[VV] = uvm_fix(nb.s[VV], uvm_of<1>(P, i, js)); nb.n[VV] = uvm_fix(nb.n[VV], uvm_of<1>(P, i, jn));
 #endif
     const pomgpu_ct am_c = cur.c[AM], u_c = uvm_fix(cur.o[0], mu), w_c = cur.o[1];
-    const pomgpu_ct am_w = halo_w(am_c, [&] { return F3(aam, iw, jc, L); });
+    const pomgpu_ct am_w = halo_w(am_c, [&] { return G3(P.aamc, iw, jc, L); });
     InvDc dzk; dzk.b = dzk.y = 0.;
     if (L >= 2) { dzk.b = F1(dz, L - 1); dzk.y = R1(dz, L - 1); }
     if constexpr (RTF) {
@@ -182,7 +182,7 @@
         const FaceT xw = advt2_face(tprni, cw, u_c, fb_c, fb_w, fc_c, fc_w, am_c, am_w);
         auto east = [&] {
           return advt2_face(tprni, coef_x(P, ie, jc), uvm_ld<0>(P, ie, jc, L), G3(A.fb[f], ie, jc, L), fb_c, G3(A.fcl[f], ie, jc, L), fc_c,
-                            F3(aam, ie, jc, L), am_c);
+                            G3(P.aamc, ie, jc, L), am_c);
         };
         FaceT xe;
         xe.adv = halo_e(xw.adv, [&] { return east().adv; });
@@ -257,7 +257,7 @@
   const double *ps[NS];
 #pragma unroll
   for (int f = 0; f < NF; f++) { ps[f] = A.q[f]; ps[NF + f] = A.qb[f]; bqf[f] = BUF3(A.qf[f]); }
-  ps[AM] = A3(aam); ps[VV] = A3(v); bo[0] = BUF3(A3(u)); bo[1] = BUF3(A3(w));
+  ps[AM] = P.aamc; ps[VV] = A3(v); bo[0] = BUF3(A3(u)); bo[1] = BUF3(A3(w));
 #pragma unroll
   for (int x = 0; x < NS; x++) bs[x] = BUF3(ps[x]);
   const RowShare<NS> S = rowshare_setup<NS>(P, r, j, j0w, i);
@@ -327,7 +327,7 @@
 #endif
     const pomgpu_ct am_c = cur.c[AM];
     const pomgpu_ct am_s = nb.s[AM], am_n = nb.n[AM], v_n = nb.n[VV];
-    const pomgpu_ct am_w = halo_w(am_c, [&] { return F3(aam, iw, jc, L); });
+    const pomgpu_ct am_w = halo_w(am_c, [&] { return G3(P.aamc, iw, jc, L); });
     pomgpu_ct w_c, ue_c = 0.;
     if constexpr (WF) {
       ue_c = halo_e(u_c, [&] { return uvm_ld<0>(P, ie, jc, L); });
@@ -353,8 +353,8 @@
         const pomgpu_ct xw = advq_face(cw, q_c, q_w, u_c, u_m, am_c, am_w, am_m, am_w_prv, qb_c, qb_w);
         xw_c = xw;
         xe_c = halo_e(xw, [&] {
-          return advq_face(coefq_x(P, ie, jc), G3(A.q[f], ie, jc, L), q_c, uvm_ld<0>(P, ie, jc, L), uvm_ld<0>(P, ie, jc, L - 1), F3(aam, ie, jc, L), am_c,
-                           F3(aam, ie, jc, L - 1), am_m, G3(A.qb[f], ie, jc, L), qb_c);
+          return advq_face(coefq_x(P, ie, jc), G3(A.q[f], ie, jc, L), q_c, uvm_ld<0>(P, ie, jc, L), uvm_ld<0>(P, ie, jc, L - 1), G3(P.aamc, ie, jc, L), am_c,
+                           G3(P.aamc, ie, jc, L - 1), am_m, G3(A.qb[f], ie, jc, L), qb_c);
         });
         ys_c = advq_face(cs, q_c, nb.s[f], v_c, v_m, am_c, am_s, am_m, ams_m, qb_c, nb.s[NF + f]);
         yn_c = advq_face(cn, nb.n[f], q_c, v_n, vn_m, am_n, am_c, amn_m, am_m, nb.n[NF + f], qb_c);
@@ -394,33 +394,33 @@
   }
 }
 
-__device__ double advct_xf_mem(const KP &P, int i, int j, int k) {
+__device__ double advct_xf_mem(const KP &P, const double *am, int i, int j, int k) {
   if (i < 2 || i > P.imm1) return 0.;
   double xf = .125 * (K2(DTSX, i + 1, j) * F3(u, i + 1, j, k) + K2(DTSX, i, j) * F3(u, i, j, k)) * (F3(u, i + 1, j, k) + F3(u, i, j, k));
-  xf = xf - F2(dt, i, j) * F3(aam, i, j, k) * 2. * (F3(ub, i + 1, j, k) - F3(ub, i, j, k)) / F2(dx, i, j);
+  xf = xf - F2(dt, i, j) * G3(am, i, j, k) * 2. * (F3(ub, i + 1, j, k) - F3(ub, i, j, k)) / F2(dx, i, j);
   return F2(dy, i, j) * xf;
 }
 __device__ double advct_curv_mem(const KP &P, int i, int j, int k) {
   if (i < 2 || i > P.imm1 || j < 2 || j > P.jmm1) return 0.;
   return .25 * ((F3(v, i, j + 1, k) + F3(v, i, j, k)) * K2(CVA, i, j) - (F3(u, i + 1, j, k) + F3(u, i, j, k)) * K2(CVB, i, j)) / F2(art, i, j);
 }
-__device__ double advct_xg_mem(const KP &P, int i, int j, int k) {
+__device__ double advct_xg_mem(const KP &P, const double *am, int i, int j, int k) {
   double xg = .125 * (K2(DTSX, i, j) * F3(u, i, j, k) + K2(DTSX, i, j - 1) * F3(u, i, j - 1, k)) * (F3(v, i, j, k) + F3(v, i - 1, j, k));
-  const double dtaam = .25 * K2(DT4, i, j) * (F3(aam, i, j, k) + F3(aam, i - 1, j, k) + F3(aam, i, j - 1, k) + F3(aam, i - 1, j - 1, k));
+  const double dtaam = .25 * K2(DT4, i, j) * (G3(am, i, j, k) + G3(am, i - 1, j, k) + G3(am, i, j - 1, k) + G3(am, i - 1, j - 1, k));
   const double dy4 = K2(DY4, i, j);
   xg = xg - dtaam * ((F3(ub, i, j, k) - F3(ub, i, j - 1, k)) / dy4 + (F3(vb, i, j, k) - F3(vb, i - 1, j, k)) / K2(DX4, i, j));
   return .25 * dy4 * xg;
 }
-__device__ double advct_yf_mem(const KP &P, int i, int j, int k) {
+__device__ double advct_yf_mem(const KP &P, const double *am, int i, int j, int k) {
   double yf = .125 * (K2(DTSY, i, j) * F3(v, i, j, k) + K2(DTSY, i - 1, j) * F3(v, i - 1, j, k)) * (F3(u, i, j, k) + F3(u, i, j - 1, k));
-  const double dtaam = .25 * K2(DT4, i, j) * (F3(aam, i, j, k) + F3(aam, i - 1, j, k) + F3(aam, i, j - 1, k) + F3(aam, i - 1, j - 1, k));
+  const double dtaam = .25 * K2(DT4, i, j) * (G3(am, i, j, k) + G3(am, i - 1, j, k) + G3(am, i, j - 1, k) + G3(am, i - 1, j - 1, k));
   const double dx4 = K2(DX4, i, j);
   yf = yf - dtaam * ((F3(ub, i, j, k) - F3(ub, i, j - 1, k)) / K2(DY4, i, j) + (F3(vb, i, j, k) - F3(vb, i - 1, j, k)) / dx4);
   return .25 * dx4 * yf;
 }
-__device__ double advct_yg_mem(const KP &P, int i, int j, int k) {
+__device__ double advct_yg_mem(const KP &P, const double *am, int i, int j, int k) {
   double yg = .125 * (K2(DTSY, i, j + 1) * F3(v, i, j + 1, k) + K2(DTSY, i, j) * F3(v, i, j, k)) * (F3(v, i, j + 1, k) + F3(v, i, j, k));
-  yg = yg - F2(dt, i, j) * F3(aam, i, j, k) * 2. * (F3(vb, i, j + 1, k) - F3(vb, i, j, k)) / F2(dy, i, j);
+  yg = yg - F2(dt, i, j) * G3(am, i, j, k) * 2. * (F3(vb, i, j + 1, k) - F3(vb, i, j, k)) / F2(dy, i, j);
   return F2(dx, i, j) * yg;
 }
 __global__ void k_advct_edge(KP P, double *to_e, double *to_n) {
@@ -429,12 +429,12 @@
   if (to_e && t <= P.jm) {
     const size_t o = (size_t)(k - 1) * P.jm + (size_t)(t - 1);
     to_e[o] = advct_curv_mem(P, P.imm1, t, k);
-    to_e[(size_t)P.kbm1 * P.jm + o] = t >= 2 ? advct_xf_mem(P, P.imm1, t, k) : 0.;
+    to_e[(size_t)P.kbm1 * P.jm + o] = t >= 2 ? advct_xf_mem(P, A3(aam), P.imm1, t, k) : 0.;
   }
   if (to_n && t <= P.im) {
     const size_t o = (size_t)(k - 1) * P.im + (size_t)(t - 1);
     to_n[o] = advct_curv_mem(P, t, P.jmm1, k);
-    to_n[(size_t)P.kbm1 * P.im + o] = t >= 2 ? advct_yg_mem(P, t, P.jmm1, k) : 0.;
+    to_n[(size_t)P.kbm1 * P.im + o] = t >= 2 ? advct_yg_mem(P, A3(aam), t, P.jmm1, k) : 0.;
   }
 }
 __global__ void k_advct_fix(KP P, const double *from_w, const double *from_s) {
@@ -444,7 +444,7 @@
     const int j = t;
     const size_t o = (size_t)(k - 1) * P.jm + (size_t)(j - 1);
     const double cv_w = from_w[o], xf_w = from_w[(size_t)P.kbm1 * P.jm + o];
-    const double xf = advct_xf_mem(P, 2, j, k), yf_n = advct_yf_mem(P, 2, j + 1, k), yf_c = advct_yf_mem(P, 2, j, k);
+    const double xf = advct_xf_mem(P, A3(aam), 2, j, k), yf_n = advct_yf_mem(P, A3(aam), 2, j + 1, k), yf_c = advct_yf_mem(P, A3(aam), 2, j, k);
     const double cv = advct_curv_mem(P, 2, j, k);
     const double ctx = cv * F2(dt, 2, j) * (F3(v, 2, j + 1, k) + F3(v, 2, j, k));
     const double ctx_w = cv_w * F2(dt, 1, j) * (F3(v, 1, j + 1, k) + F3(v, 1, j, k));
@@ -456,7 +456,7 @@
     const int i = t;
     const size_t o = (size_t)(k - 1) * P.im + (size_t)(i - 1);
     const double cv_s = from_s[o], yg_s = from_s[(size_t)P.kbm1 * P.im + o];
-    const double xg_e = advct_xg_mem(P, i + 1, 2, k), xg = advct_xg_mem(P, i, 2, k), yg_c = advct_yg_mem(P, i, 2, k);
+    const double xg_e = advct_xg_mem(P, A3(aam), i + 1, 2, k), xg = advct_xg_mem(P, A3(aam), i, 2, k), yg_c = advct_yg_mem(P, A3(aam), i, 2, k);
     const double cv = advct_curv_mem(P, i, 2, k);
     double ay = xg_e - xg + yg_c - yg_s;
     ay = ay + F2(arv, i, 2) * .25 * (cv * F2(dt, i, 2) * (F3(u, i + 1, 2, k) + F3(u, i, 2, k)) +
@@ -465,8 +465,8 @@
   }
 }
 template <int ROWS> struct LevCaT { pomgpu_ct c[5], h[(2 * 5 + ROWS - 1) / ROWS]; };
-template <int ROWS>
-__global__ void __launch_bounds__(64 * ROWS) k_advct_col(KP P, int sum2d) {
+template <int ROWS, bool AAM = false>
+__global__ void __launch_bounds__(64 * ROWS) k_advct_col(KP P, int sum2d, double *aam_w) {
   constexpr int NS = 5, NH = (2 * NS + ROWS - 1) / ROWS, U = 0, V = 1, UB = 2, VB = 3, AM = 4;
   typedef LevCaT<ROWS> LevCa;
   HALO_XCD_DECODE_R(ROWS)
@@ -491,6 +491,7 @@
 #if POMGPU_UVM_ONLOAD
   double su2 = 0., sv2 = 0.;
 #endif
+  double am2 = 0.;
   const pomgpu_ct dtsx_c = K2(DTSX, i, jc), dtsx_s = K2(DTSX, i, js);
   const pomgpu_ct dtsx_e = halo_e(dtsx_c, [&] { return K2(DTSX, ie, jc); });
   const pomgpu_ct dtsy_c = K2(DTSY, i, jc), dtsy_n = K2(DTSY, i, jn), dtsy_s = K2(DTSY, i, js);
@@ -509,15 +510,16 @@
   const bool srow = (jc - 1 >= 2);
   const bool curvx = (i0 >= (P.W ? 3 : 2)), curvy = (jc >= (P.S ? 3 : 2));
   BufA bs[NS], bh[NH];
-  const double *ps[NS] = {A3(u), A3(v), A3(ub), A3(vb), A3(aam)};
+  const double *ps[NS] = {A3(u), A3(v), A3(ub), A3(vb), AAM ? P.aamc : A3(aam)};
 #pragma unroll
   for (int x = 0; x < NS; x++) bs[x] = BUF3(ps[x]);
-  const BufA bax = BUF3(A3(advx)), bay = BUF3(A3(advy));
+  const BufA bax = BUF3(A3(advx)), bay = BUF3(A3(advy)), baw = BUF3(AAM ? aam_w : A3(advx));
   const RowShare<NS, ROWS> S = rowshare_setup<NS, ROWS>(P, r, j, j0w, i);
 #pragma unroll
   for (int q = 0; q < NH; q++) bh[q] = BUF3(rowshare_pick<NS>(ps, S.hop[q]));
   const unsigned oc = BOFF2(i, jc), lvb = LVB;
   const unsigned ost = (out && jrow) ? oc : BOFF_NONE;
+  const unsigned osta = out ? oc : BOFF_NONE;
 #ifndef POMGPU_EMU
   __shared__ pomgpu_ct slab[2][NS][ROWS + 3][64];
 #else
@@ -556,9 +558,9 @@
     const pomgpu_ct v_nw = halo_w(v_n, [&] { return F3(v, iw, jn, k); });
     const pomgpu_ct vb_w = halo_w(vb_c, [&] { return F3(vb, iw, jc, k); });
     const pomgpu_ct vb_nw = halo_w(vb_n, [&] { return F3(vb, iw, jn, k); });
-    const pomgpu_ct am_w = halo_w(am_c, [&] { return F3(aam, iw, jc, k); });
-    const pomgpu_ct am_sw = halo_w(am_s, [&] { return F3(aam, iw, js, k); });
-    const pomgpu_ct am_nw = halo_w(am_n, [&] { return F3(aam, iw, jn, k); });
+    const pomgpu_ct am_w = halo_w(am_c, [&] { return G3(ps[AM], iw, jc, k); });
+    const pomgpu_ct am_sw = halo_w(am_s, [&] { return G3(ps[AM], iw, js, k); });
+    const pomgpu_ct am_nw = halo_w(am_n, [&] { return G3(ps[AM], iw, jn, k); });
     pomgpu_ct xf = 0., cv = 0.;
     if (iin) {
       xf = CT(.125) * (dtsx_e * u_e + dtsx_c * u_c) * (u_e + u_c);
@@ -567,7 +569,7 @@
       cv = divi(CT(.25) * ((v_n + v_c) * cva_c - (u_e + u_c) * cvb_c), art_c);
     }
     const pomgpu_ct ctx = cv * dt_c * (v_n + v_c);
-    const pomgpu_ct xf_w = halo_w(xf, [&] { return advct_xf_mem(P, i - 1, jc, k); });
+    const pomgpu_ct xf_w = halo_w(xf, [&] { return advct_xf_mem(P, ps[AM], i - 1, jc, k); });
     const pomgpu_ct ctx_w = halo_w(ctx, [&] {
       return advct_curv_mem(P, i - 1, jc, k) * F2(dt, i - 1, jc) * (F3(v, i - 1, jc + 1, k) + F3(v, i - 1, jc, k));
     });
@@ -579,7 +581,7 @@
     pomgpu_ct xg = CT(.125) * (dtsx_c * u_c + dtsx_s * u_s) * (v_c + v_w);
     xg = xg - dtaam * br;
     xg = CT(.25) * dy4_c.b * xg;
-    const pomgpu_ct xg_e = halo_e(xg, [&] { return advct_xg_mem(P, i + 1, jc, k); });
+    const pomgpu_ct xg_e = halo_e(xg, [&] { return advct_xg_mem(P, ps[AM], i + 1, jc, k); });
     const pomgpu_ct dtaam_n = CT(.25) * dt4_n * (am_n + am_nw + am_c + am_w);
     pomgpu_ct yf_n = CT(.125) * (dtsy_n * v_n + dtsy_nw * v_nw) * (u_n + u_c);
     yf_n = yf_n - dtaam_n * (divi(ub_n - ub_c, dy4_n) + divi(vb_n - vb_nw, idx4_n));
@@ -611,6 +613,17 @@
     su2 = su2 + (double)u_c * dzk;
     sv2 = sv2 + (double)v_c * dzk;
 #endif
+#if POMGPU_AAM_FUSE
+    if constexpr (AAM) {
+      const double u_ne = halo_e(u_n, [&] { return F3(u, ie, jn, k); });
+      const double v_e = halo_e(v_c, [&] { return F3(v, ie, jc, k); });
+      const double v_ne = halo_e(v_n, [&] { return F3(v, ie, jn, k); });
+      double an = am_c;
+      if (in) an = aam_point_r(P, idx_c, idy_c, u_c, u_e, u_n, u_ne, u_s, u_se, v_c, v_n, v_e, v_ne, v_w, v_nw);
+      bstc(baw, osta, lv, an);
+      am2 = am2 + (double)(pomgpu_st)an * dzk;
+    }
+#endif
   };
   LevCa ra, rb;
 #ifdef POMGPU_EMU
@@ -629,6 +642,12 @@
     for (int k = 1; k <= kbm1; k++) { su2 = su2 + (double)F3(u, i, jc, k) * F1(dz, k); sv2 = sv2 + (double)F3(v, i, jc, k) * F1(dz, k); }
   }
 #endif
+  if (AAM && !jrow)
+    for (int k = 1; k <= kbm1; k++) {
+      const double an = bldc(bs[AM], oc, (unsigned)(k - 1) * lvb);
+      bstc(baw, osta, (unsigned)(k - 1) * lvb, an);
+      am2 = am2 + (double)(pomgpu_st)an * F1(dz, k);
+    }
 #endif
 #if POMGPU_UVM_ONLOAD
   if (out && (sum2d & 2)) { K2(USUM, i, jc) = su2; K2(VSUM, i, jc) = sv2; }
@@ -640,6 +659,7 @@
       for (int k = 1; k <= kb; k++) { F3(advx, i, jc, k) = 0.; F3(advy, i, jc, k) = 0.; }
     }
     if (sum2d & 1) { F2(adx2d, i, jc) = jrow ? ax2 : 0.; F2(ady2d, i, jc) = jrow ? ay2 : 0.; }
+    if (AAM) F2(aam2d, i, jc) = (i <= P.im && jc <= P.jm) ? am2 : 0.;
   }
 #ifdef POMGPU_WGTIME
   __syncthreads();
@@ -803,11 +823,21 @@
   LAUNCHN(c, "k_advq2_col", (k_advq_col<2, true>), grid1_halo_r(c->P, LDS_ROWS), blk_col_r(LDS_ROWS), c->P, A, zero_else);
 }
 #endif
-void launch_advct_col(pomgpu_ctx *c, int sum2d) {
+void launch_advct_col(pomgpu_ctx *c, int sum2d, double *aam_w) {
   const bool rows4 = SW(c, ADVCT_ROWS4) || (!SW(c, ADVCT_ROWS8) && c->P.jml <= 400 && c->exch);
   sum2d = (sum2d ? 1 : 0) | (POMGPU_UVM_ONLOAD && !c->exch && !c->tp.on && !c->wide.on && !(c->flags & POMGPU_CTX_2D) ? 2 : 0);
-  if (rows4) LAUNCHN(c, "k_advct_col", (k_advct_col<4>), grid1_halo_r(c->P, 4), blk_col_r(4), c->P, sum2d);
-  else LAUNCHN(c, "k_advct_col", (k_advct_col<LDS_ROWS>), grid1_halo_r(c->P, LDS_ROWS), blk_col_r(LDS_ROWS), c->P, sum2d);
+#if POMGPU_AAM_FUSE
+  if (aam_w) {
+    if (c->prof_on) {
+      const int s = pomgpu_prof_slot(c, "advct_aam_fused");
+      if (s >= 0) (c->parent ? c->parent : c)->prof[s].launches++;
+    }
+    LAUNCHN(c, "k_advct_col", (k_advct_col<LDS_ROWS, true>), grid1_halo_r(c->P, LDS_ROWS), blk_col_r(LDS_ROWS), c->P, sum2d, aam_w);
+    return;
+  }
+#endif
+  if (rows4) LAUNCHN(c, "k_advct_col", (k_advct_col<4>), grid1_halo_r(c->P, 4), blk_col_r(4), c->P, sum2d, (double *)NULL);
+  else LAUNCHN(c, "k_advct_col", (k_advct_col<LDS_ROWS>), grid1_halo_r(c->P, LDS_ROWS), blk_col_r(LDS_ROWS), c->P, sum2d, (double *)NULL);
 }
 __global__ void k_advct_fix2d(KP P, int west, int south) {
   const int t = TID_I;
diff --git a/extpom_amd/csrc/pomgpu_api.hip b/extpom_amd/csrc/pomgpu_api.hip
--- a/extpom_amd/csrc/pomgpu_api.hip
+++ b/extpom_amd/csrc/pomgpu_api.hip
@@ -251,6 +251,28 @@
   return (c->frc_on && (isrf < 1 || next % isrf == 0)) || (c->lat_on && (ibc < 1 || next % ibc == 0)) ||
          (c->wat_on && (iwater < 1 || (k.iint + 1) % iwater == 0));
 }
+static void aam_buffers(pomgpu_ctx *c) {
+  KP &P = c->P;
+  P.aamc = (c->aam_parity && c->aam_spare) ? c->aam_spare : (P.b3 ? P.b3 + (size_t)P3_aam * P.a3 : NULL);
+}
+static void aam_canonical(pomgpu_ctx *c) {
+  if (!c->aam_parity) return;
+  (void)hipSetDevice(c->device);
+  launch_aam_copy(c, SLOT3(c, P3_aam), c->aam_spare);
+  c->aam_parity = 0;
+  aam_buffers(c);
+}
+static bool aam_fused(pomgpu_ctx *c) {
+  if (!POMGPU_AAM_FUSE || c->exch || c->tp.on || c->wide.on || c->parent || (c->flags & POMGPU_CTX_2D) || c->wr_eager || c->P.mode == 2 ||
+      SW(c, AAM_NOFUSE) || c->aam_spare_failed)
+    return false;
+  if (!c->aam_spare) {
+    const size_t bytes = c->P.n3 * sizeof(pomgpu_st);
+    if (hipMalloc((void **)&c->aam_spare, bytes) != hipSuccess) { (void)hipGetLastError(); c->aam_spare = NULL; c->aam_spare_failed = 1; return false; }
+    (void)hipMemsetAsync(c->aam_spare, 0, bytes, c->stream);
+  }
+  return true;
+}
 static void uvf_materialize(pomgpu_ctx *c) {
   if (!c->uvf_pending) return;
   c->uvf_pending = 0;
@@ -262,6 +284,7 @@
   rho_materialize(c);
   pomgpu_wr_materialize(c);
   uvf_materialize(c);
+  aam_canonical(c);
   if (!c->rst_pending) return;
   c->rst_pending = 0;
   launch_restore_fields(c, c->rst_fold, c->rst_fnew);
@@ -379,6 +402,7 @@
   c->ext_parity = 0;
   c->rst_pending = 0;
   ext_buffers(c);
+  aam_buffers(c);
   (void)hipStreamSynchronize(c->stream);
   *out = c;
   return POMGPU_OK;
@@ -408,6 +432,7 @@
   for (int n = 0; n < POMGPU_NSCR2; n++) (void)hipFree(P.s2[n]);
   (void)hipFree(c->uvb_bot[0]); (void)hipFree(c->uvb_bot[1]);
   (void)hipFree(c->rt_words); (void)hipFree(c->rt_cols);
+  (void)hipFree(c->aam_spare);
   for (int n = 0; n < POMGPU_NCOEF2; n++) (void)hipFree(P.c2[n]);
   (void)hipFree(c->alt2[0]); (void)hipFree(c->alt3[0]);
   (void)hipFree(P.m8);
@@ -441,6 +466,7 @@
       pomgpu_ctx *two[2] = {c, c->wide.x};
       for (pomgpu_ctx *t : two)
         if (t) { t->sw.on[n] = value ? 1 : 0; t->sw.val[n] = value ? atol(value) : 0; }
+      if (n == SW_AAM_NOFUSE) aam_canonical(c);
       return POMGPU_OK;
     }
   return fail(c, POMGPU_EINVAL, "debug_switch: no switch named %s", name);
@@ -725,10 +751,10 @@
     launch_advave_m2b(c);
   }
 }
-static void seq_advct(pomgpu_ctx *c, int sum2d = 0, int defer_xch = 0) {
+static void seq_advct(pomgpu_ctx *c, int sum2d = 0, int defer_xch = 0, double *aam_w = NULL) {
   KP &P = c->P;
   if (!c->exch) {
-    launch_advct_col(c, sum2d);
+    launch_advct_col(c, sum2d, aam_w);
     c->uvm_valid = POMGPU_UVM_ONLOAD && !c->tp.on && !c->wide.on && !(c->flags & POMGPU_CTX_2D);
     return;
   }
@@ -1008,6 +1034,7 @@
   side_wait(c, SIDE_RTS);
   rho_materialize(c);
   KP &P = c->P;
+  c->aam2d_done = 0;
   if (P.mode != 2) {
     const bool lib_x = c->tp.on && c->exch && !SW(c, ADVCT_SPLIT);
     auto pressure_gradient = [&]() {
@@ -1021,9 +1048,12 @@
     const bool pg_first = c->side_ev[SIDE_R8].pending != 0;
     if (pg_first) pressure_gradient();
     side_wait(c, SIDE_R8);
-    seq_advct(c, sum2d, lib_x);
+    const bool fuse = sum2d && aam_fused(c);
+    if (!fuse) aam_canonical(c);
+    seq_advct(c, sum2d, lib_x, fuse ? (c->aam_parity ? SLOT3(c, P3_aam) : c->aam_spare) : NULL);
     if (!pg_first) pressure_gradient();
-    launch_aam(c);
+    if (fuse) { c->aam_parity ^= 1; aam_buffers(c); c->aam2d_done = 1; }
+    else launch_aam(c);
     if (lib_x && sum2d && rim_side(c)) {
       double *arr[3] = {D3(c, advx), D3(c, advy), D3(c, aam)};
       const int nz[3] = {P.kb, P.kb, P.kbm1};
@@ -1050,13 +1080,14 @@
 static int mode_interaction(pomgpu_ctx *c, int sums_done) {
   NEED_HOT(c);
   if (c->wide.on) {
-    if (c->P.mode != 2) launch_vint(c, sums_done, sums_done && c->side_ev[SIDE_R2].pending ? 1 : 0);
+    if (c->P.mode != 2) { aam_canonical(c); launch_vint(c, sums_done, sums_done && c->side_ev[SIDE_R2].pending ? 1 : 0); }
     return wide_begin(c);
   }
   if (c->P.mode != 2) {
-    launch_vint(c, sums_done);
+    if (!(sums_done && c->aam2d_done)) { aam_canonical(c); launch_vint(c, sums_done); }
     seq_advave(c);
   }
+  c->aam2d_done = 0;
   launch_modeint_tail(c);
   xch(c, 2, D2(c, utf), 1, D2(c, vtf), 1);
   return POMGPU_OK;
@@ -1579,6 +1610,7 @@
   side_wait(c, SIDE_R8);
   if ((k.iint != 1 || k.time0 != 0.) && k.mode != 2) {
     c->uvf_pending = 0;
+    if (!(k.nadv == 2 && P.nitera == 1) || (c->exch && SW(c, ADVQ_EXCHANGE))) aam_canonical(c);
     struct UvmScope { pomgpu_ctx *c; ~UvmScope() { c->P.uvm = 0; c->uvm_valid = 0; } } uvm_scope{c};
     P.uvm = uvm_onload(c) ? 1 : 0;
     if (!P.uvm) launch_int_uvmean(c);
@@ -2246,6 +2278,7 @@
     }
     return POMGPU_OK;
   };
+  aam_canonical(c);
   const TuneLay cur = {c->tune_front, c->P.a3};
   int rc = POMGPU_OK;
   if ((to.f >= cur.f && to.a >= cur.a) || (to.f <= cur.f && to.a <= cur.a)) rc = one_way(cur, to);
@@ -2260,6 +2293,7 @@
   P.a3 = to.a;
   P.b3 = c->tune_block + to.f;
   for (int n = 0; n < POMGPU_NSCR3; n++) P.s3[n] = P.b3 + (size_t)POM_NBLK3D * P.a3 + (size_t)n * P.n3;
+  aam_buffers(c);
   return POMGPU_OK;
 }
 extern "C" int pomgpu_tune_placement(pomgpu_ctx *c, int steps, int max_try, double *ms_out, long *front_mib_out, long *pad_mib_out, int *ntried, int *kept) {
@@ -2309,6 +2343,7 @@
     c->tune_amax = amax;
     P.b3 = blk;
     for (int n = 0; n < POMGPU_NSCR3; n++) P.s3[n] = blk + (size_t)POM_NBLK3D * a0 + (size_t)n * P.n3;
+    aam_buffers(c);
   }
   static const int KS[20][2] = {{0, 0}, {3, 0}, {10, 0}, {0, 1}, {3, 1}, {10, 1}, {5, 0}, {5, 1}, {2, 0}, {1, 0}, {7, 0}, {4, 0}, {7, 1}, {2, 1}, {15, 0}, {20, 0}, {25, 0}, {30, 0}, {15, 1}, {20, 1}};
   hipEvent_t e0 = NULL, e1 = NULL;
diff --git a/extpom_amd/csrc/pomgpu_internal.hpp b/extpom_amd/csrc/pomgpu_internal.hpp
--- a/extpom_amd/csrc/pomgpu_internal.hpp
+++ b/extpom_amd/csrc/pomgpu_internal.hpp
@@ -43,6 +43,7 @@
   double *g4[4];
   unsigned char *m8;
   int uvm;
+  const double *aamc;
 };
 enum pomgpu_x2 { X2_ua, X2_va, X2_d, X2_el, X2_elb, X2_uab, X2_vab };
 
@@ -70,6 +71,11 @@
 #define POMGPU_UVM_ONLOAD 0
 #else
 #define POMGPU_UVM_ONLOAD 1
+#endif
+#ifdef POMGPU_COMPUTE_F32
+#define POMGPU_AAM_FUSE 0
+#else
+#define POMGPU_AAM_FUSE 1
 #endif
 #ifdef POMGPU_STORE_F32
 struct Ref3 {
@@ -400,6 +406,12 @@
 static inline double divi(double a, const InvD &d) { return a / d.b; }
 static inline float divi(float a, const InvDT<float> &d) { return a / d.b; }
 #endif
+__device__ __forceinline__ double aam_point_r(const KP &P, const InvD &dx, const InvD &dy, double u_c, double u_e, double u_n, double u_ne, double u_s,
+                                              double u_se, double v_c, double v_n, double v_e, double v_ne, double v_w, double v_nw) {
+  return P.horcon * dx.b * dy.b *
+         sqrt(sq(divi(u_e - u_c, dx)) + sq(divi(v_n - v_c, dy)) +
+              .5 * sq(divi(.25 * (u_n + u_ne - u_s - u_se), dy) + divi(.25 * (v_e + v_ne - v_w - v_nw), dx)));
+}
 #define HALO_XCD_ORDER                                                                    \
   if (P.g_strip > 0) {                                                                    \
     const int st__ = P.g_strip, nfull__ = nbx__ / st__, wlast__ = nbx__ - nfull__ * st__; \
@@ -458,7 +470,7 @@
   X(PROFQ_NOPACE) X(COL_STRIP) X(BAND_BYTES) X(PAD3) X(IO_SYNC) X(ADVCT_SPLIT) X(ADVQ_EXCHANGE) X(PROD_FULL) X(QFILTER_SPLIT) \
   X(NO_OVERLAP) X(NO_SIDE_COMM) X(WR_MAIN) X(WIDE_W) X(WIDE_FULL) X(DEBUG_ALLOC) X(TEST_SPLIT_FAIL_RANK)  \
   X(WR_NODEFER) X(EXT_RING_FIRST) X(TUNE_FORCE) X(RIM_MAIN) X(RIM_RESULTS_MAIN) X(SUM2D_OFF) X(ADVCT_ROWS4) X(ADVCT_ROWS8) \
-  X(IO_CHUNK_KB) X(UV_NOFUSE) X(W_NOFUSE) X(UVMEAN_PASS) X(PROFT_TWIN) X(LD_EAGER) X(TR_NOPAIR) X(RT_LOAD)
+  X(IO_CHUNK_KB) X(UV_NOFUSE) X(W_NOFUSE) X(UVMEAN_PASS) X(PROFT_TWIN) X(LD_EAGER) X(TR_NOPAIR) X(RT_LOAD) X(AAM_NOFUSE)
 enum pomgpu_sw {
 #define POMGPU_SW_(name) SW_##name,
   POMGPU_SWITCHES(POMGPU_SW_)
@@ -577,6 +589,8 @@
   int wr_pending;
   int uvf_pending;
   int uvm_valid;
+  double *aam_spare;
+  int aam_parity, aam_spare_failed, aam2d_done;
   double *uvb_bot[2];
   int wr_eager;
   double *d_vel;
@@ -687,7 +701,7 @@
 void launch_advave_b(pomgpu_ctx *c);
 void launch_advave_c(pomgpu_ctx *c);
 void launch_advave_fused(pomgpu_ctx *c);
-void launch_advct_col(pomgpu_ctx *c, int sum2d);
+void launch_advct_col(pomgpu_ctx *c, int sum2d, double *aam_w = NULL);
 void launch_advct_edge(pomgpu_ctx *c, double *to_e, double *to_n);
 void launch_advct_fix(pomgpu_ctx *c, const double *from_w, const double *from_s);
 void launch_advct_fix2d(pomgpu_ctx *c, int west, int south);
@@ -741,6 +755,7 @@
 void launch_mask3(pomgpu_ctx *c, double *a, const double *m2);
 void launch_smol(pomgpu_ctx *c, const double *ff);
 void launch_copy3(pomgpu_ctx *c, double *dst, const double *src);
+void launch_aam_copy(pomgpu_ctx *c, double *dst, const double *src);
 void launch_advt2_diff(pomgpu_ctx *c, const double *fb, const double *fc, double *ff);
 void launch_ts_update(pomgpu_ctx *c, double fold, double fnew, int rt, int store_rst, int rt_flags = 0);
 void launch_restore_fields(pomgpu_ctx *c, double fold, double fnew);
```

Result: faster. 5.126 billion (median of 6 runs) (+3.2%).
